# ucsdarclab/diffco

Measured on AMD Instinct MI355X. Metric: million collision-score+grad evals/sec, 7-DoF FK-kernel, 2k supports, higher is better.
Workload: dtype f32

## Files before the change

### diffco_amd/csrc/dcx_api.hip

```cpp
#include <algorithm>
#include <atomic>
#include <cmath>
#include <cstdio>
#include <cstdlib>
#include <cstring>
#include <mutex>
#include <new>
#include <string>
#include <vector>

#include "dcx_internal.h"
#include "motion_cost_kernel.h"
#include "motion_kernel.h"
#include "motion_worst_kernel.h"
#include "pack_kernels.h"
#include "solve_kernels.h"
#include "traj_dense.h"

using namespace dcx;

struct dcx_model {
    int device = 0;
    dcx_fk_desc fk{};
    FkProg* fk_dev = nullptr;
    DhProg* dh_dev = nullptr;
    DhArgs dh{};
    int32_t fk_dwords = 0;
    float* rows_dev = nullptr;
    float* rows_p2_dev = nullptr;
    float* rows_xf_dev = nullptr;
    float* centre_dev = nullptr;
    int64_t S_in = 0;
    int32_t S_active = 0;
    int64_t cap = 0;
    float fold = 1.0f;
    int32_t* info_dev = nullptr;
    int32_t* info_host = nullptr;
    int32_t D = 0, Dt = 0, C = 0, RS = 0;
    int32_t Cc = 0;
    int32_t kind = 0, kf = 0;
    float kp0 = 0, kp1 = 0;
    float kp0_sweep = 0;
    int32_t xf_rq_ok = 0;
    int32_t frame_floats = 0;
    int32_t prog_floats = 0;
    launch_fn launch = nullptr;
    int32_t max_threads = 0;
    int32_t n_cu = 256;
    struct Scratch {
        hipStream_t stream;
        float* ptr;
        size_t rows_bytes;
        uint32_t epoch;
    };
    int32_t* giveup_host = nullptr;
    int32_t* giveup_dev = nullptr;
    mutable std::mutex mu;
    mutable std::vector<Scratch> scratch;
    struct TrajExch {
        hipStream_t stream;
        unsigned long long* ptr;
        size_t bytes;
        uint32_t epoch;
    };
    mutable std::vector<TrajExch> traj_exch;
    struct HessMom {
        hipStream_t stream;
        float* ptr;
        size_t bytes;
    };
    mutable std::vector<HessMom> hess_mom;
};

#ifdef DCX_TIMING
static unsigned long long* g_ts_dev = nullptr;
constexpr size_t kTsWords = 32 * 16 + 4096 * 4;
#endif

namespace {

thread_local std::string g_err;

int fail(int code, const std::string& msg) {
// ... 125 lines not shown
}

int set_device(int device) {
    int n = 0;
    hipError_t e = hipGetDeviceCount(&n);
    if (e != hipSuccess || n == 0) return fail(DCX_ERR_NO_DEVICE, "no HIP device visible (libdcx has no CPU path)");
    if (device < 0 || device >= n) return fail(DCX_ERR_INVALID, "device index out of range");
    DCX_HIP(hipSetDevice(device));
    return DCX_OK;
}

struct FkCacheEntry {
    int device;
    dcx_fk_desc host;
    FkProg* dev;
};
thread_local std::vector<FkCacheEntry> g_fk_cache;

int upload_fk_prog(const dcx_fk_desc& fk, FkProg** out) {
    FkProg prog;
    build_fk_prog(fk, prog);
    FkProg* d = nullptr;
    DCX_HIP(hipMalloc((void**)&d, sizeof(FkProg)));
    hipError_t e = hipMemcpy(d, &prog, sizeof(FkProg), hipMemcpyHostToDevice);
    if (e != hipSuccess) {
        (void)hipFree(d);
        return fail_hip(e, "upload of the FK program");
    }
    *out = d;
    return DCX_OK;
}

int fk_device_copy(int device, const dcx_fk_desc& fk, FkProg** out) {
    for (auto& e : g_fk_cache)
        if (e.device == device && std::memcmp(&e.host, &fk, sizeof(fk)) == 0) {
            *out = e.dev;
            return DCX_OK;
        }
    FkProg* d = nullptr;
    if (int rc = upload_fk_prog(fk, &d)) return rc;
    if (g_fk_cache.size() >= 64) {
        (void)hipFree(g_fk_cache.front().dev);
        g_fk_cache.erase(g_fk_cache.begin());
    }
    g_fk_cache.push_back({device, fk, d});
    *out = d;
    return DCX_OK;
}

struct Knobs {
    std::atomic<int64_t> ys{-1}, nw{-1}, min_rows{-1}, split_finish_kernel{-1}, inlaunch_tiles{-1}, jac_per_class{-1},
        traj_fused{-1}, xf{-1}, jac_one_sweep{-1}, train_grid{-1}, fkk{-1}, jt_waves{-1}, hess_ys{-1}, hess_form{-1},
        traj_ys{-1}, traj_across{-1}, owner_poll{-1}, solve_threads{-1}, qt{-1}, giveup_inject{-1}, skew{-1}, skew8{-1},
        motion_early_exit{-1};
    Knobs() {
        auto rd = [](const char* name, std::atomic<int64_t>& dst, bool flag) {
            if (const char* e = std::getenv(name)) dst = flag ? 1 : std::atoll(e);
        };
        rd("DCX_YS", ys, false);
        rd("DCX_NW", nw, false);
        rd("DCX_MIN_ROWS", min_rows, false);
        rd("DCX_SPLIT_FINISH_KERNEL", split_finish_kernel, true);
        rd("DCX_INLAUNCH_TILES", inlaunch_tiles, false);
        rd("DCX_JAC_PER_CLASS", jac_per_class, true);
        rd("DCX_TRAJ_FUSED", traj_fused, false);
        rd("DCX_XF", xf, false);
        rd("DCX_JAC_ONE_SWEEP", jac_one_sweep, false);
        rd("DCX_TRAIN_GRID", train_grid, false);
        rd("DCX_FKK", fkk, false);
        rd("DCX_JT_WAVES", jt_waves, false);
        rd("DCX_HESS_YS", hess_ys, false);
        rd("DCX_HESS_FORM", hess_form, false);
        rd("DCX_TRAJ_YS", traj_ys, false);
        rd("DCX_TRAJ_ACROSS", traj_across, false);
        rd("DCX_OWNER_POLL", owner_poll, false);
        rd("DCX_SOLVE_THREADS", solve_threads, false);
        rd("DCX_QT", qt, false);
        rd("DCX_SKEW", skew, false);
        rd("DCX_SKEW8", skew8, false);
    }
};
Knobs& knobs() {
    static Knobs k;
    return k;
}

struct Geometry {
    int nw, ys;
    int red_slots;
};
Geometry pick_geometry(const dcx_model* m, int64_t B, int acc_floats, bool allow_split) {
    const int cap = m->max_threads / 64;
    const int64_t tiles = (B + 63) / 64;
    Geometry g;
    g.ys = 1;
    if (allow_split && 2 * tiles <= m->n_cu) {
        const int64_t want = std::min<int64_t>((int64_t)m->n_cu / tiles, m->S_active / 250);
        while (2 * g.ys <= want && g.ys < 32) g.ys *= 2;
        g.nw = std::min(16, cap);
    } else if (allow_split && 3 * tiles <= 2 * (int64_t)m->n_cu && (int64_t)m->S_active * m->Dt >= 18000) {
        g.ys = 3;
        g.nw = std::min(16, cap);
    } else {
        g.nw = std::min((tiles <= 4 * (int64_t)m->n_cu) ? 16 : 8, cap);
    }
    const Knobs& kn = knobs();
    if (const int64_t v = kn.ys; v >= 1 && allow_split) g.ys = (int)std::min<int64_t>(v, 64);
    if (const int64_t v = kn.nw; v >= 1) g.nw = (int)std::min<int64_t>(v, cap);
    int min_rows = 15;
    if (const int64_t v = kn.min_rows; v >= 1) min_rows = (int)v;
    while (g.ys > 1 && m->S_active / (g.ys * g.nw) < min_rows) g.ys /= 2;
    while (g.nw > 1 && m->S_active / (g.ys * g.nw) < min_rows) g.nw /= 2;
    const int d_fk = m->fk.n_points * m->fk.point_dim;
    auto lds_bytes = [&](int nw, int slots) {
        return (size_t)(lds_plan(m->fk.dof, d_fk, m->frame_floats, nw > 1 ? slots : 0, acc_floats, true).total + m->prog_floats) * sizeof(float);
    };
    g.red_slots = g.nw;
    const size_t lds_cap = (g.ys > 1 ? 150 : 64) * 1024;
    if (lds_bytes(g.nw, g.nw) > lds_cap && g.nw >= 8 && lds_bytes(g.nw / 2, g.nw / 2) <= lds_cap && kn.nw < 1) {
        g.nw /= 2;
        g.red_slots = g.nw;
    }
    if (lds_bytes(g.nw, g.nw) > lds_cap) {
        const int wps = sweep_min_waves(m->Dt, m->Cc, m->kf);
        int best_nw = 1, best_waves = 0;
        for (int nw = g.nw; nw >= 1; nw /= 2) {
            const size_t lds = lds_bytes(nw, 1);
            if (lds > 64 * 1024) continue;
            const int by_lds = (int)((160 * 1024) / lds), by_regs = std::max(1, (4 * wps) / nw);
            const int waves = std::min(by_lds, by_regs) * nw;
            if (waves > best_waves) {
                best_waves = waves;
                best_nw = nw;
            }
        }
        g.nw = best_nw;
        g.red_slots = 1;
// ... 195 lines not shown
    a.upstream = upstream;
    a.score = score;
    a.grad = grad;
    a.B = B;
    a.S = m->S_active;
    a.ys = g.ys;
    a.s_super = (m->S_active + g.ys - 1) / g.ys;
    a.s_chunk = (a.s_super + g.nw - 1) / g.nw;
    const bool p2 = !qt && !xf_able && m->rows_p2_dev != nullptr && p2_applies(m->Dt, m->Cc, m->kf);
    if (p2) {
        a.rows = m->rows_p2_dev;
        a.s_super = (a.s_super + 1) & ~1;
        a.s_chunk = ((a.s_super + g.nw - 1) / g.nw + 1) & ~1;
    }
    const bool so = mode == MODE_SCORE && !hinge.traj_slices;
    a.s_skew = (g.nw == 16 && !qt && (a.s_chunk >= 24 || knobs().skew > 0)) ? skew_rule(m->Cc, so, hinge.traj_slices != 0) : (g.nw == 8 && !qt && (a.s_chunk >= 24 || knobs().skew8 > 0)) ? skew8_rule(so) : 0;
    a.red_slots = g.red_slots;
    a.dof = m->fk.dof;
    a.d_fk = d_fk;
    a.frame_floats = m->frame_floats;
    a.kind = m->kind;
    a.c_out = m->C;
    a.one_hot = one_hot;
    a.nz = nz;
    a.grad_stride = grad_stride;
    a.kp0 = m->kp0_sweep;
    a.kp1 = m->kp1;
    a.hinge = hinge.on;
    a.hinge_margin = hinge.margin;
    a.hinge_weight = hinge.weight;
    for (int c = 0; c < DCX_MAX_C; ++c) a.hinge_margin_c[c] = hinge.margin_c[c];
    a.xf = xf_able ? 1 : 0;
    if (qt) {
        a.xf = 0;
        a.qt = 1;
        a.qt_per = qt_per;
        for (int gq = 0; gq < 4; ++gq) a.qt_per_g[gq] = qt_per;
        if (g.nw == 16 && skew_rule() > 0) {
            const int32_t sk = skew_rule();
            const int w3[3] = {sk & 1023, (sk >> 10) & 1023, (sk >> 20) & 1023};
            int left = 4 * qt_per;
            for (int gq = 0; gq < 3; ++gq) {
                a.qt_per_g[gq] = std::min(left, (int)((int64_t)4 * qt_per * w3[gq] / 1000));
                left -= a.qt_per_g[gq];
            }
            a.qt_per_g[3] = left;
        }
        a.qt_off = (int32_t)((lds_plan(a.dof, d_fk, m->frame_floats, g.nw, acc, true).total + m->prog_floats + 3) & ~3);
        a.qt_scr = a.qt_off + QT_SLICES * g.nw * (qt_per * row_stride(m->Dt, m->Cc) + 4);
        const int64_t kq = knobs().qt;
        a.qt_front = (int32_t)((int64_t)QT_SLICES * g.nw * qt_per * (kq >= 100 ? std::min<int64_t>(kq - 100, 100) : 45) / 100);
        nblk = (B + 15) / 16;
    }
    if (a.xf) {
        a.rows = m->rows_xf_dev;
        a.centre = m->centre_dev;
    }
    a.jt_rows = (a.fkk == 2 && g.nw >= 2 * m->dh.n_chains && m->dh.n_chains <= 2 && m->dh.end0 <= kDhUnroll &&
                 m->dh.n_steps - m->dh.end0 <= kDhUnroll && knobs().jt_waves != 0) ? 1 : 0;
    a.jt_waves = (a.jt_rows && mode != MODE_SCORE && g.red_slots == g.nw && (g.nw - 1) * acc >= 12 * m->dh.n_pt + 1 &&
                  (g.ys == 1 || counters != nullptr)) ? 1 : 0;
#ifdef DCX_TIMING
    if (!g_ts_dev && hipMalloc((void**)&g_ts_dev, sizeof(unsigned long long) * kTsWords) == hipSuccess)
        (void)hipMemset(g_ts_dev, 0, sizeof(unsigned long long) * kTsWords);
    a.ts = g_ts_dev;
    a.ts_block = std::getenv("DCX_TS_BLOCK") ? (unsigned)std::atoi(std::getenv("DCX_TS_BLOCK")) : 0u;
#endif
    size_t lds = sizeof(float) * (lds_plan(a.dof, d_fk, m->frame_floats, g.nw > 1 ? g.red_slots : 0, acc, true).total + m->prog_floats);
    if (qt) lds = qt_lds;
    if (g.ys == 1) {
        hipError_t e = m->launch(m->kf, m->Cc, mode, g.nw, lds, nblk, a, st);
        if (e != hipSuccess) return fail_hip(e, "score kernel launch");
        return DCX_OK;
    }
    if (nz > 1 && counters == nullptr) return DCX_ERR_UNSUPPORTED;
    a.partial = part;
    a.tile_done = counters;
    if (counters != nullptr && g.red_slots == g.nw && g.nw > 1 && knobs().owner_poll != 0 && (acc <= 2 * g.nw || knobs().owner_poll > 0) &&
        nblk * nz * g.ys <= (int64_t)m->n_cu && 2 * nblk * nz <= (int64_t)m->n_cu && m->giveup_dev != nullptr &&
        (knobs().owner_poll > 0 || opoll_stream_ok(m->device, st))) {
        a.pwords = reinterpret_cast<unsigned long long*>(reinterpret_cast<char*>(part) + (size_t)2 * m->n_cu * (m->Dt + m->Cc) * 64 * sizeof(float));
        a.ptag = ptag;
        a.giveup = m->giveup_dev;
    }
    hipError_t e = m->launch(m->kf, m->Cc, mode, g.nw, lds, nblk, a, st);
    if (e == hipSuccess && counters == nullptr) {
        FinishArgs f{};
        f.partial = part;
        f.fk = m->fk_dev;
        f.q = q;
        f.upstream = (m->C == 1) ? upstream : nullptr;
        f.score = score;
        f.grad = grad;
        f.B = B;
        f.grad_stride = grad_stride;
        f.ys = g.ys;
        f.acc = acc;
        f.C = m->Cc;
        f.c_out = m->C;
        f.Dt = m->Dt;
        f.dof = m->fk.dof;
        f.d_fk = d_fk;
        f.frame_floats = m->frame_floats;
        f.want_grad = (mode != MODE_SCORE);
        f.hinge = hinge.on;
        f.hinge_margin = hinge.margin;
        f.hinge_weight = hinge.weight;
        e = launch_score_finish(f, nblk, sizeof(float) * (lds_plan(a.dof, d_fk, m->frame_floats, 0, 0).total + m->prog_floats), st);
    }
    if (e != hipSuccess) return fail_hip(e, "split score launch");
    return DCX_OK;
}

}

extern "C" {

#ifdef DCX_TIMING
int dcx_debug_ts_words(void) { return (int)kTsWords; }
int dcx_debug_read_ts(unsigned long long* out) {
    if (!g_ts_dev) return 1;
    (void)hipDeviceSynchronize();
    return hipMemcpy(out, g_ts_dev, sizeof(unsigned long long) * kTsWords, hipMemcpyDeviceToHost) == hipSuccess ? 0 : 3;
}
#endif

int dcx_version(void) { return DCX_VERSION; }

int dcx_debug_set(const char* name, int64_t value) {
    if (!name) return fail(DCX_ERR_INVALID, "knob name is NULL");
    Knobs& k = knobs();
    const std::string n(name);
    if (n == "mfma" || n == "xm")
        return value > 0 ? fail(DCX_ERR_UNSUPPORTED, "the matrix-core forms of the sweep were removed (measured slower, profiles/r03_mfma_ab.txt)")
                         : DCX_OK;
    std::atomic<int64_t>* dst = n == "ys" ? &k.ys : n == "nw" ? &k.nw : n == "min_rows" ? &k.min_rows
        : n == "split_finish_kernel" ? &k.split_finish_kernel : n == "inlaunch_tiles" ? &k.inlaunch_tiles
        : n == "jac_per_class" ? &k.jac_per_class : n == "traj_fused" ? &k.traj_fused : n == "xf" ? &k.xf : n == "jac_one_sweep" ? &k.jac_one_sweep : n == "train_grid" ? &k.train_grid : n == "fkk" ? &k.fkk : n == "jt_waves" ? &k.jt_waves : n == "hess_ys" ? &k.hess_ys : n == "hess_form" ? &k.hess_form : n == "traj_ys" ? &k.traj_ys : n == "traj_across" ? &k.traj_across : n == "owner_poll" ? &k.owner_poll : n == "solve_threads" ? &k.solve_threads : n == "qt" ? &k.qt : n == "giveup_inject" ? &k.giveup_inject : n == "skew" ? &k.skew : n == "skew8" ? &k.skew8 : n == "motion_early_exit" ? &k.motion_early_exit : nullptr;
    if (!dst) return fail(DCX_ERR_INVALID, "unknown knob: " + n);
    *dst = value;
    return DCX_OK;
}

const char* dcx_last_error(void) { return g_err.c_str(); }

int dcx_device_count(void) {
    int n = 0;
    if (hipGetDeviceCount(&n) != hipSuccess) return 0;
    return n;
}

static constexpr double kXfRqRule = 32.0;
static size_t rows_tail_floats(const dcx_model* m) { return 8 * (size_t)m->RS + 16; }

static void model_free_rows(dcx_model* m) {
    if (m->rows_dev) (void)hipFree(m->rows_dev);
    if (m->rows_xf_dev) (void)hipFree(m->rows_xf_dev);
    if (m->rows_p2_dev) (void)hipFree(m->rows_p2_dev);
    m->rows_dev = m->rows_xf_dev = m->rows_p2_dev = nullptr;
    m->cap = 0;
}

static int model_alloc_rows(dcx_model* m, int64_t cap) {
    if (cap < 1) cap = 1;
    if (cap <= m->cap && m->rows_dev) return DCX_OK;
    const size_t floats = (size_t)cap * m->RS + rows_tail_floats(m);
    float *rows = nullptr, *rows_xf = nullptr, *rows_p2 = nullptr;
    hipError_t e = hipMalloc((void**)&rows, floats * sizeof(float));
    if (e == hipSuccess) e = hipMalloc((void**)&rows_xf, floats * sizeof(float));
    if (e == hipSuccess && p2_applies(m->Dt, m->Cc, m->kf)) e = hipMalloc((void**)&rows_p2, (floats + m->RS) * sizeof(float));
    if (e == hipSuccess && !m->centre_dev) e = hipMalloc((void**)&m->centre_dev, (size_t)m->Dt * sizeof(float));
    if (e == hipSuccess && !m->info_dev) e = hipMalloc((void**)&m->info_dev, 16);
    if (e == hipSuccess && !m->info_host) e = hipHostMalloc((void**)&m->info_host, 16, hipHostMallocDefault);
    if (e == hipSuccess && !m->giveup_host) {
        e = hipHostMalloc((void**)&m->giveup_host, sizeof(int32_t), hipHostMallocMapped);
        if (e == hipSuccess) {
            *m->giveup_host = 0;
            e = hipHostGetDevicePointer((void**)&m->giveup_dev, m->giveup_host, 0);
        }
    }
    if (e != hipSuccess) {
        if (rows) (void)hipFree(rows);
        if (rows_xf) (void)hipFree(rows_xf);
        if (rows_p2) (void)hipFree(rows_p2);
        return fail_hip(e, "device allocation of the model");
    }
    model_free_rows(m);
    m->rows_dev = rows;
    m->rows_xf_dev = rows_xf;
    m->rows_p2_dev = rows_p2;
    m->cap = cap;
    return DCX_OK;
}

static int model_fill_device(dcx_model* m, const float* feat_dev, const float* w_dev, int64_t S, hipStream_t stream) {
    PackArgs a{};
    a.feat = feat_dev;
    a.w = w_dev;
    a.rows = m->rows_dev;
    a.rows_xf = m->rows_xf_dev;
    a.centre = m->centre_dev;
    a.info = m->info_dev;
    a.S = S;
    a.D = m->D;
    a.Dt = m->Dt;
    a.C = m->C;
    a.Cl = m->Cc;
    a.RS = m->RS;
    a.tail_floats = (int32_t)rows_tail_floats(m);
    a.centred = (m->fk.kind != DCX_FK_NONE) ? 1 : 0;
    a.rq2 = (m->kf == KF_RQ2) ? 1 : 0;
    a.fold = m->fold;
    a.seed = m->kp0_sweep;
    hipError_t e = launch_pack_rows(a, stream);
    if (e == hipSuccess) e = hipMemcpyAsync(m->info_host, m->info_dev, 16, hipMemcpyDeviceToHost, stream);
    if (e == hipSuccess) e = hipStreamSynchronize(stream);
    if (e != hipSuccess) return fail_hip(e, "packing of the support rows");
    double ss_max;
    std::memcpy(&ss_max, reinterpret_cast<const char*>(m->info_host) + 8, sizeof(double));
    m->S_in = S;
    m->S_active = m->info_host[0];
    m->xf_rq_ok = (m->kf == KF_RQ2 && m->fk.kind != DCX_FK_NONE && (double)m->kp0 * ss_max <= kXfRqRule) ? 1 : 0;
    return DCX_OK;
}

static int model_fill_host(dcx_model* m, const float* support_feat, const float* weights, int64_t S, hipStream_t stream) {
    const int32_t D = m->D, C = m->C, Cl = m->Cc;
    std::vector<float> feat((size_t)S * D), w((size_t)S * C);
    if (S > 0) {
        hipError_t e = hipStreamSynchronize(stream);
        if (e == hipSuccess) e = hipMemcpy(feat.data(), support_feat, feat.size() * sizeof(float), hipMemcpyDefault);
        if (e == hipSuccess) e = hipMemcpy(w.data(), weights, w.size() * sizeof(float), hipMemcpyDefault);
        if (e != hipSuccess) return fail_hip(e, "copy of supports/weights");
    }
    const float fold = m->fold;
    std::vector<float> rows;
    rows.reserve((size_t)S * m->RS + rows_tail_floats(m));
    int32_t kept = 0;
    for (int64_t j = 0; j < S; ++j) {
        bool any = false;
        for (int c = 0; c < C; ++c) any |= (w[j * C + c] != 0.0f);
        if (!any) continue;
        const size_t base = rows.size();
        rows.resize(base + m->RS, 0.0f);
        for (int k = 0; k < D; ++k) rows[base + k] = feat[j * D + k];
        float sum = 0.0f;
        for (int c = 0; c < C; ++c) {
            const float v = w[j * C + c] * fold;
            rows[base + m->Dt + c] = v;
            sum += v;
        }
        if (Cl > 1) rows[base + m->Dt + Cl] = sum;
        double ss = 0.0;
        for (int k = 0; k < D; ++k) ss += (double)feat[j * D + k] * (double)feat[j * D + k];
        rows[base + m->Dt + Cl + (Cl > 1 ? 1 : 0)] = (float)ss;
        ++kept;
    }
    m->S_in = S;
    m->S_active = kept;
    m->xf_rq_ok = 0;
    std::vector<float> centre(m->Dt, 0.0f), rows_xf(rows);
    const int ss_off = m->Dt + Cl + (Cl > 1 ? 1 : 0);
    if (m->fk.kind != DCX_FK_NONE && kept > 0) {
        for (int k = 0; k < D; ++k) {
            double acc = 0.0;
            for (int32_t j = 0; j < kept; ++j) acc += (double)rows[(size_t)j * m->RS + k];
            centre[k] = (float)(acc / (double)kept);
        }
    }
    double ss_max = 0.0;
    for (int32_t j = 0; j < kept; ++j) {
        float* cen = &rows_xf[(size_t)j * m->RS];
        double ss = 0.0;
        for (int k = 0; k < D; ++k) {
            cen[k] = cen[k] - centre[k];
            ss += (double)cen[k] * (double)cen[k];
        }
        ss_max = std::max(ss_max, ss);
        cen[ss_off] = (m->kf == KF_RQ2) ? (float)(ss + (double)m->kp0_sweep) : (float)ss;
    }
    m->xf_rq_ok = (m->kf == KF_RQ2 && m->fk.kind != DCX_FK_NONE && (double)m->kp0 * ss_max <= kXfRqRule) ? 1 : 0;
    rows.resize(rows.size() + rows_tail_floats(m), 0.0f);
    rows_xf.resize(rows.size(), 0.0f);
    hipError_t e = hipMemcpy(m->rows_dev, rows.data(), rows.size() * sizeof(float), hipMemcpyHostToDevice);
    if (e == hipSuccess) e = hipMemcpy(m->rows_xf_dev, rows_xf.data(), rows_xf.size() * sizeof(float), hipMemcpyHostToDevice);
    if (e == hipSuccess) e = hipMemcpy(m->centre_dev, centre.data(), centre.size() * sizeof(float), hipMemcpyHostToDevice);
    if (e != hipSuccess) return fail_hip(e, "upload of the model's rows");
    return DCX_OK;
}

static bool is_device_ptr(const void* p) {
    hipPointerAttribute_t at;
    if (hipPointerGetAttributes(&at, p) != hipSuccess) {
        (void)hipGetLastError();
        return false;
    }
    return at.type == hipMemoryTypeDevice;
}

static int refuse_capture(hipStream_t stream) {
    hipStreamCaptureStatus cap = hipStreamCaptureStatusNone;
    if (hipStreamIsCapturing(stream, &cap) != hipSuccess || cap != hipStreamCaptureStatusNone) {
        (void)hipGetLastError();
        return fail(DCX_ERR_UNSUPPORTED, "a model cannot be built or refilled on a stream that is being captured (the kept row count is read back)");
    }
    return DCX_OK;
}

static int model_fill(dcx_model* m, const float* support_feat, const float* weights, int64_t S, hipStream_t stream) {
    const bool on_device = S > 0 && is_device_ptr(support_feat) && is_device_ptr(weights);
    int rc = on_device ? model_fill_device(m, support_feat, weights, S, stream) : model_fill_host(m, support_feat, weights, S, stream);
    if (rc == DCX_OK && m->rows_p2_dev) {
        hipError_t e = launch_interleave_rows(m->rows_dev, m->rows_p2_dev, (int32_t)m->S_active, m->RS, (int32_t)rows_tail_floats(m), stream);
        if (e != hipSuccess) return fail_hip(e, "interleaving of the support rows");
    }
    return rc;
}

int dcx_model_create(dcx_model** out, int device, const dcx_fk_desc* fk, int kernel_kind, const float* kparams,
                     const float* support_feat, const float* weights, int64_t S, int32_t D, int32_t C) {
    return dcx_model_create_ex(out, device, fk, kernel_kind, kparams, support_feat, weights, S, D, C, 0, nullptr);
}

int dcx_model_create_ex(dcx_model** out, int device, const dcx_fk_desc* fk, int kernel_kind, const float* kparams,
                        const float* support_feat, const float* weights, int64_t S, int32_t D, int32_t C,
                        int64_t capacity, void* stream) {
    if (!out) return fail(DCX_ERR_INVALID, "out is NULL");
    *out = nullptr;
    if (S < 0 || S > 0x7fffffffLL) return fail(DCX_ERR_INVALID, "S out of range");
    if (S > 0 && (!support_feat || !weights)) return fail(DCX_ERR_INVALID, "support_feat / weights is NULL");
    if (D < 1 || D > DCX_MAX_D) return fail(DCX_ERR_UNSUPPORTED, "D must be in [1, DCX_MAX_D]");
    if (C < 1 || C > DCX_MAX_C) return fail(DCX_ERR_UNSUPPORTED, "C must be in [1, DCX_MAX_C]");
    if (int rc = check_kernel(kernel_kind, kparams)) return rc;
    dcx_fk_desc desc;
    std::memset(&desc, 0, sizeof(desc));
    if (fk && fk->kind != DCX_FK_NONE) {
        desc = *fk;
    } else {
// ... 41 lines not shown
        return rc;
    }
    {
        FkProg prog;
        build_fk_prog(m->fk, prog);
        m->fk_dwords = prog.n_dwords;
        DhProg dh;
        if (build_dh_prog(m->fk, dh)) {
            hipError_t de = hipMalloc((void**)&m->dh_dev, sizeof(DhProg));
            if (de == hipSuccess) de = hipMemcpy(m->dh_dev, &dh, sizeof(DhProg), hipMemcpyHostToDevice);
            if (de != hipSuccess) {
                dcx_model_destroy(m);
                return fail_hip(de, "upload of the DH step table");
            }
            m->dh = dh_args_of(dh, m->dh_dev);
        }
    }
    if (capacity > 0x7fffffffLL) capacity = 0x7fffffffLL;
    int rc = model_alloc_rows(m, std::max<int64_t>(S, capacity));
    if (rc == DCX_OK) rc = model_fill(m, support_feat, weights, S, (hipStream_t)stream);
    if (rc != DCX_OK) {
        const std::string msg = g_err;
        dcx_model_destroy(m);
        g_err = msg;
        return rc;
    }
    *out = m;
    return DCX_OK;
}

int dcx_model_update(dcx_model* m, const float* support_feat, const float* weights, int64_t S, void* stream) {
    if (!m) return fail(DCX_ERR_INVALID, "model is NULL");
    if (S < 0 || S > 0x7fffffffLL) return fail(DCX_ERR_INVALID, "S out of range");
    if (S > 0 && (!support_feat || !weights)) return fail(DCX_ERR_INVALID, "support_feat / weights is NULL");
    if (int rc = set_device(m->device)) return rc;
    if (int rc = refuse_capture((hipStream_t)stream)) return rc;
    std::lock_guard<std::mutex> lock(m->mu);
    if (S > m->cap) {
        hipError_t e = hipDeviceSynchronize();
        if (e != hipSuccess) return fail_hip(e, "dcx_model_update");
        if (int rc = model_alloc_rows(m, S)) return rc;
    }
    return model_fill(m, support_feat, weights, S, (hipStream_t)stream);
}

void dcx_model_destroy(dcx_model* m) {
    if (!m) return;
    (void)hipSetDevice(m->device);
    if (m->fk_dev) (void)hipFree(m->fk_dev);
    if (m->dh_dev) (void)hipFree(m->dh_dev);
    if (m->rows_dev) (void)hipFree(m->rows_dev);
    if (m->rows_xf_dev) (void)hipFree(m->rows_xf_dev);
    if (m->rows_p2_dev) (void)hipFree(m->rows_p2_dev);
    if (m->centre_dev) (void)hipFree(m->centre_dev);
    if (m->info_dev) (void)hipFree(m->info_dev);
    if (m->info_host) (void)hipHostFree(m->info_host);
    if (m->giveup_host) (void)hipHostFree(m->giveup_host);
    for (auto& sc : m->scratch)
        if (sc.ptr) (void)hipFree(sc.ptr);
    for (auto& hm : m->hess_mom)
        if (hm.ptr) (void)hipFree(hm.ptr);
    for (auto& ex : m->traj_exch)
        if (ex.ptr) (void)hipFree(ex.ptr);
    delete m;
}

int dcx_model_info(const dcx_model* m, int64_t* S_active, int32_t* D, int32_t* C, int32_t* dof, int32_t* device) {
    if (!m) return fail(DCX_ERR_INVALID, "model is NULL");
    if (S_active) *S_active = m->S_active;
    if (D) *D = m->D;
    if (C) *C = m->C;
    if (dof) *dof = m->fk.dof;
    if (device) *device = m->device;
    return DCX_OK;
}

int dcx_score(const dcx_model* m, const float* q, int64_t B, float* score, void* stream) {
    if (!m) return fail(DCX_ERR_INVALID, "model is NULL");
    if (B < 0 || (B > 0 && (!q || !score))) return fail(DCX_ERR_INVALID, "q / score is NULL or B < 0");
    if (int rc = set_device(m->device)) return rc;
    return run_score(m, q, B, nullptr, score, nullptr, MODE_SCORE, -1, m->fk.dof, (hipStream_t)stream);
}

int dcx_score_grad(const dcx_model* m, const float* q, int64_t B, const float* upstream, float* score, float* grad,
                   void* stream) {
    if (!m) return fail(DCX_ERR_INVALID, "model is NULL");
    if (B < 0 || (B > 0 && (!q || !grad))) return fail(DCX_ERR_INVALID, "q / grad is NULL or B < 0");
    if (int rc = set_device(m->device)) return rc;
    const int mode = (m->C > 1 && upstream) ? MODE_GRAD_UP : MODE_GRAD_ROW;
    return run_score(m, q, B, upstream, score, grad, mode, -1, m->fk.dof, (hipStream_t)stream);
}

static int run_hinge(const dcx_model* m, const float* q, int64_t B, const float* margin , float weight, float* score,
                     float* grad, hipStream_t st, bool traj_slices = false) {
    Hinge h;
    h.weight = weight;
    h.traj_slices = traj_slices ? 1 : 0;
    if (m->C == 1) {
        h.on = 1;
        h.margin = margin[0];
        return run_score(m, q, B, nullptr, score, grad, MODE_GRAD_ROW, -1, m->fk.dof, st, h);
    }
    h.on = 2;
    for (int c = 0; c < m->C; ++c) h.margin_c[c] = margin[c];
    Hinge hs;
    hs.traj_slices = traj_slices ? 1 : 0;
// ... 207 lines not shown
        const int d_fk = m->fk.n_points * m->fk.point_dim;
        int nw = std::min(16, m->max_threads / 64);
        if (const int64_t v = knobs().nw; v >= 1) nw = (int)std::min<int64_t>(v, m->max_threads / 64);
        int ys = 1;
        {
            int64_t want = std::min<int64_t>(8, (int64_t)m->n_cu / std::max(1, st->n_paths));
            if (const int64_t v = knobs().traj_ys; v >= 1) want = std::min<int64_t>(v, 32);
            while (2 * ys <= want) ys *= 2;
            int min_rows = 15;
            if (const int64_t v = knobs().min_rows; v >= 1) min_rows = (int)v;
            while (ys > 1 && (m->S_active / (ys * nw) < min_rows || (int64_t)ys * st->n_paths > m->n_cu)) ys /= 2;
        }
        while (nw > 1 && m->S_active / (ys * nw) < 15) nw /= 2;
        const bool dh_ok = m->fk.kind == DCX_FK_DH && m->dh_dev && knobs().fkk != 0 && knobs().fkk != 1 && knobs().jt_waves != 0 &&
                           m->dh.n_chains <= 2 && m->dh.end0 <= kDhUnroll && m->dh.n_steps - m->dh.end0 <= kDhUnroll;
        const int jt_min_waves = 2 + 2 * m->dh.n_chains;
        auto lds_of = [&](int w) {
            return sizeof(float) * (size_t)(traj_fused_plan(m->fk.dof, d_fk, m->frame_floats, w, m->Dt, (dh_ok && w >= jt_min_waves) ? m->dh.n_pt : 0, m->Cc).total + m->prog_floats);
        };
        while (nw > 1 && lds_of(nw) > 150 * 1024) nw /= 2;
        traj_fused_fn fn = traj_fused_for(m->Dt);
        bool fused_ok = fn && lds_of(nw) <= 150 * 1024;
        if (fused_ok) {
            TrajFusedArgs a{};
            for (int c = 0; c < DCX_MAX_C; ++c) a.margin_c[c] = margin[c];
            a.sc.rows = m->rows_dev;
            set_fk_walk(m, a.sc);
            a.sc.jt_rows = a.sc.jt_waves = (dh_ok && nw >= jt_min_waves && a.sc.fkk == 2) ? 1 : 0;
#ifdef DCX_TIMING
            if (!g_ts_dev && hipMalloc((void**)&g_ts_dev, sizeof(unsigned long long) * kTsWords) == hipSuccess)
                (void)hipMemset(g_ts_dev, 0, sizeof(unsigned long long) * kTsWords);
            a.sc.ts = g_ts_dev;
#endif
            a.sc.S = m->S_active;
            bool traj_p2 = false;
            auto slice = [&](int ys_) {
                a.s_super = (m->S_active + ys_ - 1) / ys_;
                a.sc.s_chunk = (a.s_super + nw - 1) / nw;
                if (traj_p2) {
                    a.s_super = (a.s_super + 1) & ~1;
                    a.sc.s_chunk = ((a.s_super + nw - 1) / nw + 1) & ~1;
                }
                a.sc.s_skew = (nw == 16 && (a.sc.s_chunk >= 24 || knobs().skew > 0)) ? skew_rule(m->Cc, false, true) : (nw == 8 && (a.sc.s_chunk >= 24 || knobs().skew8 > 0)) ? skew8_rule() : 0;
            };
            a.sc.dof = m->fk.dof;
            a.sc.d_fk = d_fk;
            a.sc.frame_floats = m->frame_floats;
            a.sc.kind = m->kind;
            a.sc.c_out = m->C;
            a.sc.kp0 = m->kp0_sweep;
            a.sc.kp1 = m->kp1;
            a.sc.xf = (knobs().xf != 0 && m->kf == KF_POLY1 && xf_applies(m->Dt, m->Cc, KF_POLY1) && m->rows_xf_dev) ? 1 : 0;
            if (a.sc.xf) {
                a.sc.rows = m->rows_xf_dev;
                a.sc.centre = m->centre_dev;
            } else if (m->rows_p2_dev && p2_applies(m->Dt, m->Cc, m->kf)) {
                a.sc.rows = m->rows_p2_dev;
                traj_p2 = true;
            }
            slice(ys);
            a.st = *st;
            a.opt = *opt;
            a.n_points = m->fk.n_points;
            a.point_dim = m->fk.point_dim;
            a.coord_major = (m->fk.kind == DCX_FK_TREE && m->fk.t_coord_major) ? 1 : 0;
            for (int done = 0; done < n_iters; done += kTrajFusedMaxIters) {
                a.n_iters = std::min(kTrajFusedMaxIters, n_iters - done);
                for (int i = 0; i < a.n_iters; ++i) {
                    const double t = (double)(first_step + done + i);
                    a.bias1[i] = (float)(1.0 - std::pow((double)opt->beta1, t));
                    a.bias2_sqrt[i] = (float)std::sqrt(1.0 - std::pow((double)opt->beta2, t));
                }
                a.ys = 1;
                if (ys > 1) {
                    a.exch = traj_exchange_rows(m, (hipStream_t)stream, (size_t)st->n_paths * 2 * ys * traj_exchange_words(m->Dt, m->Cc) * 64 * sizeof(unsigned long long),
                                                &a.tag_base);
                    if (a.exch) a.ys = ys;
                    a.cl_across = knobs().traj_across > 0 ? 1 : 0;
                }
                if (a.ys != ys) {
                    ys = 1;
                    slice(1);
                }
                hipError_t e = fn(m->kf, m->Cc, nw, lds_of(nw), st->n_paths, a, (hipStream_t)stream);
                if (e == hipErrorNotSupported && done == 0) {
                    (void)hipGetLastError();
                    fused_ok = false;
                    break;
                }
                if (e != hipSuccess && a.ys > 1) {
                    (void)hipGetLastError();
                    ys = a.ys = 1;
                    slice(1);
                    e = fn(m->kf, m->Cc, nw, lds_of(nw), st->n_paths, a, (hipStream_t)stream);
                }
                if (e != hipSuccess) return fail_hip(e, "fused trajectory launch");
            }
            if (fused_ok) return DCX_OK;
        }
    }
    for (int it = 0; it < n_iters; ++it) {
        int rc = run_hinge(m, st->path, B, margin, opt->w_collision, const_cast<float*>(st->col_score), const_cast<float*>(st->col_grad),
                           (hipStream_t)stream, true);
        if (rc) return rc;
        hipError_t e = launch_traj_adam_step(m->fk_dev, m->fk, *st, *opt, first_step + it, (hipStream_t)stream, m->C, margin);
        if (e != hipSuccess) return fail_hip(e, "trajectory step launch");
    }
    return DCX_OK;
// ... 113 lines not shown
    w.frac = up((size_t)(E + 1) * sizeof(int64_t));
    w.counters = w.frac + up((size_t)E * sizeof(float));
    w.partial = w.counters + (size_t)kMotionSplitTiles * kCounterStride * sizeof(unsigned int);
    w.total = w.partial + (size_t)kMotionSplitRows * DCX_MAX_C * 64 * sizeof(float);
    return w;
}
motion_fn motion_for(int Dt) {
    switch (Dt) {
#define DCX_CASE(D) case D: return launch_motion_D##D;
        DCX_CASE(2) DCX_CASE(4) DCX_CASE(6) DCX_CASE(8) DCX_CASE(12) DCX_CASE(16) DCX_CASE(18) DCX_CASE(21)
        DCX_CASE(24) DCX_CASE(27) DCX_CASE(30) DCX_CASE(32) DCX_CASE(36) DCX_CASE(42) DCX_CASE(48) DCX_CASE(54)
        DCX_CASE(60) DCX_CASE(64) DCX_CASE(72) DCX_CASE(84) DCX_CASE(96)
#undef DCX_CASE
    default: return nullptr;
    }
}
struct MotionSweepPlan {
    Geometry g;
    size_t lds;
};
MotionSweepPlan motion_sweep_plan(const dcx_model* m, int64_t tiles_max, char* base, const MotionWork& w, ScoreArgs& sa) {
    const int d_fk = m->fk.n_points * m->fk.point_dim;
    const int acc = m->Cc;
    Geometry g = pick_geometry(m, std::min<int64_t>(tiles_max, (int64_t)1 << 30) * 64, acc, true);
    if (g.ys > 1 && (tiles_max > kMotionSplitTiles || tiles_max * g.ys > kMotionSplitRows))
        g = pick_geometry(m, std::min<int64_t>(tiles_max, (int64_t)1 << 30) * 64, acc, false);
    sa.rows = m->rows_dev;
    set_fk_walk(m, sa);
    sa.B = 0;
    sa.S = m->S_active;
    sa.ys = g.ys;
    sa.s_super = (m->S_active + g.ys - 1) / g.ys;
    sa.s_chunk = (sa.s_super + g.nw - 1) / g.nw;
    const bool xf_able = knobs().xf != 0 && xf_applies(m->Dt, m->Cc, m->kf) && m->rows_xf_dev != nullptr &&
                         (m->kf != KF_RQ2 || m->xf_rq_ok || knobs().xf >= 2);
    if (!xf_able && m->rows_p2_dev != nullptr && p2_applies(m->Dt, m->Cc, m->kf)) {
        sa.rows = m->rows_p2_dev;
        sa.s_super = (sa.s_super + 1) & ~1;
        sa.s_chunk = ((sa.s_super + g.nw - 1) / g.nw + 1) & ~1;
    }
    sa.s_skew = (g.nw == 16 && (sa.s_chunk >= 24 || knobs().skew > 0)) ? skew_rule(m->Cc, true)
              : (g.nw == 8 && (sa.s_chunk >= 24 || knobs().skew8 > 0)) ? skew8_rule(true) : 0;
    sa.red_slots = g.red_slots;
    sa.dof = m->fk.dof;
    sa.d_fk = d_fk;
    sa.frame_floats = m->frame_floats;
    sa.kind = m->kind;
    sa.c_out = m->C;
    sa.one_hot = -1;
    sa.nz = 1;
    sa.kp0 = m->kp0_sweep;
    sa.kp1 = m->kp1;
    sa.xf = xf_able ? 1 : 0;
    if (sa.xf) {
        sa.rows = m->rows_xf_dev;
        sa.centre = m->centre_dev;
    }
    sa.jt_rows = (sa.fkk == 2 && g.nw >= 2 * m->dh.n_chains && m->dh.n_chains <= 2 && m->dh.end0 <= kDhUnroll &&
                  m->dh.n_steps - m->dh.end0 <= kDhUnroll && knobs().jt_waves != 0) ? 1 : 0;
    if (g.ys > 1) {
        sa.partial = (float*)(base + w.partial);
        sa.tile_done = (unsigned int*)(base + w.counters);
    }
    const size_t lds = sizeof(float) * (((size_t)lds_plan(sa.dof, d_fk, m->frame_floats, g.nw > 1 ? g.red_slots : 0, acc, true).total +
                                         m->prog_floats + 3) & ~(size_t)3) + sizeof(float) * kMotionLdsFloats;
    return MotionSweepPlan{g, lds};
}
}

size_t dcx_motion_work_bytes(const dcx_model* m, int64_t E) {
    if (!m || E < 0) return 0;
    return motion_work(E).total;
}

int dcx_check_motions(const dcx_model* m, const float* qa, const float* qb, int64_t E, const dcx_motion_opts* opt,
                      const float* margin, int32_t* first_hit, int32_t* n_samples, void* work, size_t work_bytes, void* stream) {
    return dcx_check_motions_ex(m, qa, qb, E, opt, margin, first_hit, n_samples, work, work_bytes, 0, stream);
}

int dcx_check_motions_ex(const dcx_model* m, const float* qa, const float* qb, int64_t E, const dcx_motion_opts* opt,
                         const float* margin, int32_t* first_hit, int32_t* n_samples, void* work, size_t work_bytes,
                         uint64_t wrap_mask, void* stream) {
    if (!m) return fail(DCX_ERR_INVALID, "model is NULL");
    if (!opt) return fail(DCX_ERR_INVALID, "motion options are NULL");
    if (E < 0) return fail(DCX_ERR_INVALID, "E < 0");
    if (E > 0 && (!qa || !qb || !first_hit || !work)) return fail(DCX_ERR_INVALID, "qa / qb / first_hit / work is NULL");
    const bool by_res = opt->res > 0, by_step = opt->max_step > 0.f;
    if (opt->res < 0 || !(opt->max_step >= 0.f) || by_res == by_step)
        return fail(DCX_ERR_INVALID, "motion check needs exactly one sampling rule: res > 0 or max_step > 0 (the other 0)");
    if (opt->max_samples < 1) return fail(DCX_ERR_INVALID, "motion check needs max_samples >= 1");
    if (wrap_mask != 0 && m->fk.dof < 64 && (wrap_mask >> m->fk.dof) != 0)
        return fail(DCX_ERR_INVALID, "motion check: wrap_mask has a bit at or above dof");
    const MotionWork w = motion_work(E);
    if (E > 0 && work_bytes < w.total) return fail(DCX_ERR_INVALID, "motion workspace is smaller than dcx_motion_work_bytes");
    if (E > INT32_MAX) return fail(DCX_ERR_UNSUPPORTED, "motion check: more than 2^31 - 1 edges");
    if (E == 0) return DCX_OK;
    const int64_t tiles_max = (E * (int64_t)opt->max_samples + 63) / 64;
    if (tiles_max > 0x7fffffffLL) return fail(DCX_ERR_UNSUPPORTED, "motion check: E * max_samples too large for one launch");
    if (int rc = set_device(m->device)) return rc;
    hipStream_t st = (hipStream_t)stream;
    char* base = (char*)work;
    MotionArgs a{};
    const MotionSweepPlan plan = motion_sweep_plan(m, tiles_max, base, w, a.sc);
    const Geometry& g = plan.g;
    MotionPrepArgs p{};
    p.qa = qa;
    p.qb = qb;
    p.E = E;
    p.dof = m->fk.dof;
    p.res = opt->res;
// ... 230 lines not shown
    const MotionCostWork w = motion_cost_work(m, E, opt->max_samples);
    char* base = (char*)work;
    const int d_fk = m->fk.n_points * m->fk.point_dim;
    const int acc = m->Dt + m->Cc;
    const int64_t b_max = std::min<int64_t>(tiles_max, (int64_t)1 << 30) * 64;
    Geometry g = pick_geometry(m, b_max, acc, true);
    if (g.ys > 1 && (tiles_max > kMotionSplitTiles || tiles_max * g.ys > kMotionSplitRows)) g = pick_geometry(m, b_max, acc, false);
    MotionPrepArgs p{};
    p.qa = qa;
    p.qb = qb;
    p.E = E;
    p.dof = m->fk.dof;
    p.res = opt->res;
    p.max_samples = opt->max_samples;
    p.max_step = opt->max_step;
    p.offs = (int64_t*)(base + w.offs);
    p.frac = (float*)(base + w.frac);
    p.first_hit = (int32_t*)(base + w.status);
    p.n_samples = n_samples;
    p.counters = g.ys > 1 ? (unsigned int*)(base + w.counters) : nullptr;
    p.n_counters = g.ys > 1 ? (int32_t)tiles_max : 0;
    p.open_end = opt->max_step > 0.f ? opt->open_end : 0;
    p.wrap_mask = wrap_mask;
    hipError_t e = launch_motion_prep(p, st);
    if (e != hipSuccess) return fail_hip(e, "motion cost prep launch");

    MotionCostArgs a{};
    ScoreArgs& sa = a.sc;
    sa.rows = m->rows_dev;
    set_fk_walk(m, sa);
    sa.B = 0;
    sa.S = m->S_active;
    sa.ys = g.ys;
    sa.s_super = (m->S_active + g.ys - 1) / g.ys;
    sa.s_chunk = (sa.s_super + g.nw - 1) / g.nw;
    const bool xf_able = knobs().xf != 0 && xf_applies(m->Dt, m->Cc, m->kf) && m->rows_xf_dev != nullptr &&
                         (m->kf != KF_RQ2 || m->xf_rq_ok || knobs().xf >= 2);
    if (!xf_able && m->rows_p2_dev != nullptr && p2_applies(m->Dt, m->Cc, m->kf)) {
        sa.rows = m->rows_p2_dev;
        sa.s_super = (sa.s_super + 1) & ~1;
        sa.s_chunk = ((sa.s_super + g.nw - 1) / g.nw + 1) & ~1;
    }
    sa.red_slots = g.red_slots;
    sa.dof = m->fk.dof;
    sa.d_fk = d_fk;
    sa.frame_floats = m->frame_floats;
    sa.kind = m->kind;
    sa.c_out = m->C;
    sa.one_hot = -1;
    sa.nz = 1;
    sa.kp0 = m->kp0_sweep;
    sa.kp1 = m->kp1;
    sa.xf = xf_able ? 1 : 0;
    if (sa.xf) {
        sa.rows = m->rows_xf_dev;
        sa.centre = m->centre_dev;
    }
    sa.jt_rows = (sa.fkk == 2 && g.nw >= 2 * m->dh.n_chains && m->dh.n_chains <= 2 && m->dh.end0 <= kDhUnroll &&
                  m->dh.n_steps - m->dh.end0 <= kDhUnroll && knobs().jt_waves != 0) ? 1 : 0;
    sa.jt_waves = 0;
    if (g.ys > 1) {
        sa.partial = (float*)(base + w.partial);
        sa.tile_done = (unsigned int*)(base + w.counters);
    }
    a.qa = qa;
    a.qb = qb;
    a.offs = p.offs;
    a.frac = p.frac;
    a.margin = margin;
    a.h = (float*)(base + w.h);
    a.dq = (float*)(base + w.dq);
    a.scores = m->C > 1 ? (float*)(base + w.scores) : nullptr;
    a.tile_on = m->C > 1 ? (int32_t*)(base + w.tile_on) : nullptr;
    a.E = E;
    a.weight = weight;
    a.res = opt->res;
    a.open_end = p.open_end;
    a.wrap_mask = wrap_mask;
    auto skew_for = [&](bool score_only) {
        return (g.nw == 16 && (sa.s_chunk >= 24 || knobs().skew > 0)) ? skew_rule(m->Cc, score_only)
             : (g.nw == 8 && (sa.s_chunk >= 24 || knobs().skew8 > 0)) ? skew8_rule(score_only) : 0;
    };
    auto lds_for = [&](int acc_floats) {
        return sizeof(float) * (((size_t)lds_plan(sa.dof, d_fk, m->frame_floats, g.nw > 1 ? g.red_slots : 0, acc_floats, true).total +
                                 m->prog_floats + 3) & ~(size_t)3) + sizeof(float) * kMotionCostLdsFloats;
    };
    if (m->C == 1) {
        sa.s_skew = skew_for(false);
        e = launch(m->kf, m->Cc, MODE_GRAD_ROW, g.nw, lds_for(acc), tiles_max, a, st);
    } else {
        sa.s_skew = skew_for(true);
        e = launch(m->kf, m->Cc, MODE_SCORE, g.nw, lds_for(m->Cc), tiles_max, a, st);
        if (e == hipSuccess) {
            sa.s_skew = skew_for(false);
            e = launch(m->kf, m->Cc, MODE_GRAD_UP, g.nw, lds_for(acc), tiles_max, a, st);
        }
    }
    if (e != hipSuccess) return fail_hip(e, "motion cost kernel launch");
    MotionReduceArgs r{};
    r.qa = qa;
    r.qb = qb;
    r.offs = p.offs;
    r.frac = p.frac;
    r.status = p.first_hit;
    r.h = a.h;
    r.dq = a.dq;
    r.cost = cost;
    r.grad_a = grad_a;
    r.grad_b = grad_b;
    r.E = E;
// ... 294 lines not shown
```

### diffco_amd/csrc/motion_cost_inst.hip

```cpp
#include "dcx_internal.h"
#include "motion_cost_kernel.h"

#ifndef DCX_INST_D
#error "compile with -DDCX_INST_D=<feature width>"
#endif

namespace dcx {
#define DCX_CAT_(a, b) a##b
#define DCX_CAT(a, b) DCX_CAT_(a, b)
#ifdef DCX_STUB
hipError_t DCX_CAT(launch_motion_cost_D, DCX_INST_D)(int, int, int, int, size_t, int64_t, const MotionCostArgs&, hipStream_t) {
    return hipErrorNotSupported;
}
#else
namespace {
constexpr int kD = DCX_INST_D;
constexpr int kMaxT = kD <= 16 ? 1024 : (kD <= 48 ? 512 : 256);

template <int KF, int CC, int MODE>
hipError_t go(int nw, size_t lds, int64_t nblk, const MotionCostArgs& a, hipStream_t st) {
    const dim3 grid((unsigned)nblk, (unsigned)(a.sc.ys > 1 ? a.sc.ys : 1));
    const int32_t mc_off = (int32_t)(lds / sizeof(float)) - kMotionCostLdsFloats;
    auto launch = [&](auto kern) {
        if (lds > 64 * 1024) {
            hipError_t e = hipFuncSetAttribute((const void*)kern, hipFuncAttributeMaxDynamicSharedMemorySize, (int)lds);
            if (e != hipSuccess) return e;
        }
        kern<<<grid, dim3(64 * nw), lds, st>>>(a, mc_off);
        return hipGetLastError();
    };
    if constexpr (xf_applies(kD, CC, KF)) {
        if (a.sc.xf) return launch(motion_cost_kernel<kD, KF, CC, MODE, kMaxT, true>);
    }
    return launch(motion_cost_kernel<kD, KF, CC, MODE, kMaxT>);
}

template <int KF, int CC>
hipError_t passes(int mode, int nw, size_t lds, int64_t nblk, const MotionCostArgs& a, hipStream_t st) {
    if (mode == MODE_SCORE) return go<KF, CC, MODE_SCORE>(nw, lds, nblk, a, st);
    if (mode == MODE_GRAD_UP) return go<KF, CC, MODE_GRAD_UP>(nw, lds, nblk, a, st);
    return hipErrorInvalidValue;
}

template <int KF>
hipError_t by_cc(int cc, int mode, int nw, size_t lds, int64_t nblk, const MotionCostArgs& a, hipStream_t st) {
    switch (cc) {
    case 1: return mode == MODE_GRAD_ROW ? go<KF, 1, MODE_GRAD_ROW>(nw, lds, nblk, a, st) : hipErrorInvalidValue;
    case 5: return passes<KF, 5>(mode, nw, lds, nblk, a, st);
#ifndef DCX_DEV_FAST
    case 4: return passes<KF, 4>(mode, nw, lds, nblk, a, st);
    case 8: return passes<KF, 8>(mode, nw, lds, nblk, a, st);
#endif
    default: return hipErrorInvalidValue;
    }
}
}

hipError_t DCX_CAT(launch_motion_cost_D, DCX_INST_D)(int kf, int cc, int mode, int nw, size_t lds, int64_t nblk,
                                                     const MotionCostArgs& a, hipStream_t st) {
    switch (kf) {
    case KF_RQ2: return by_cc<KF_RQ2>(cc, mode, nw, lds, nblk, a, st);
    case KF_POLY1: return by_cc<KF_POLY1>(cc, mode, nw, lds, nblk, a, st);
    case KF_GEN: return by_cc<KF_GEN>(cc, mode, nw, lds, nblk, a, st);
    default: return hipErrorInvalidValue;
    }
}
#endif
}
```

### diffco_amd/csrc/motion_cost_kernel.h

```cpp
#pragma once
#include <hip/hip_runtime.h>
#include <stdint.h>
#include "motion_kernel.h"

namespace dcx {

struct MotionCostArgs {
    ScoreArgs sc;
    const float* qa;
    const float* qb;
    const int64_t* offs;
    const float* frac;
    const float* margin;
    float* h;
    float* dq;
    float* scores;
    int32_t* tile_on;
    int64_t E;
    float weight;
    int32_t res;
    int32_t open_end;
    uint64_t wrap_mask;
};

// ... 20 lines not shown
    float* cost;
    float* grad_a;
    float* grad_b;
    int64_t E;
    int32_t dof, res, open_end;
    float weight;
    uint64_t wrap_mask;
};
hipError_t launch_motion_cost_reduce(const MotionReduceArgs& r, hipStream_t stream);

#ifdef __HIPCC__
constexpr int kMotionCostLdsFloats = kMotionLdsFloats;

__device__ __forceinline__ void motion_tile_lookup(const int64_t* offs, int64_t E, int64_t base, int nb, int64_t* sEnd,
                                                   int32_t* sEdge, int32_t* sK, int32_t* sN) {
    const int lane = threadIdx.x & 63;
    int64_t lo = 0, hi = E;
    while (hi - lo > 1) {
        const int64_t step = (hi - lo + 63) / 64;
        const int64_t idx = lo + (int64_t)lane * step;
        const bool le = idx < hi && offs[idx] <= base;
        const int p = __popcll(__builtin_amdgcn_ballot_w64(le));
        const int64_t nlo = lo + (int64_t)(p - 1) * step;
        hi = (lo + (int64_t)p * step < hi) ? lo + (int64_t)p * step : hi;
        lo = nlo;
    }
    const int64_t e0 = lo;
    sEnd[lane] = (e0 + 1 + lane <= E) ? offs[e0 + 1 + lane] : INT64_MAX;
    __builtin_amdgcn_wave_barrier();
    __builtin_amdgcn_fence(__ATOMIC_ACQ_REL, "workgroup");
    const int64_t s = base + (lane < nb ? lane : nb - 1);
    int64_t e, start;
    if (sEnd[63] > s) {
        int j = 0;
#pragma unroll
        for (int hh = 32; hh >= 1; hh >>= 1)
            if (sEnd[j + hh - 1] <= s) j += hh;
        e = e0 + j;
        start = j ? sEnd[j - 1] : offs[e0];
    } else {
        int64_t l2 = e0 + 64, h2 = E;
        while (h2 - l2 > 1) {
            const int64_t md = (l2 + h2) / 2;
            if (offs[md] <= s) l2 = md; else h2 = md;
        }
        e = l2;
        start = offs[l2];
    }
    sEdge[lane] = (int32_t)e;
    sK[lane] = (int32_t)(s - start);
    sN[lane] = (int32_t)(offs[e + 1] - start);
}

template <int D, int KF, int CC, int MODE, int MAXT, bool XF = false>
__global__ __launch_bounds__(MAXT, sweep_min_waves(D, CC, KF)) void motion_cost_kernel(const MotionCostArgs m, int32_t mc_off) {
    static_assert((CC == 1) == (MODE == MODE_GRAD_ROW), "one class: the hinge sweep; several: the score and gradient passes");
    extern __shared__ __attribute__((aligned(16))) float smem[];
    constexpr bool GRAD = MODE != MODE_SCORE;
    constexpr int ACC = (GRAD ? D : 0) + CC;
    const ScoreArgs& a = m.sc;
    const int wave = __builtin_amdgcn_readfirstlane(threadIdx.x >> 6);
    const int nw = blockDim.x >> 6;
    const int dof = a.dof;
    const LdsPlan lp = lds_plan(dof, a.d_fk, a.frame_floats, nw > 1 ? a.red_slots : 0, ACC, true);
    float* sQ = smem + lp.q;
    float* sX = smem + lp.x;
    float* sF = smem + lp.f;
    int64_t* sEnd = reinterpret_cast<int64_t*>(smem + mc_off);
    int32_t* sEdge = reinterpret_cast<int32_t*>(smem + mc_off + 128);
    int32_t* sK = sEdge + 64;
    int32_t* sN = sEdge + 128;

    const int64_t E = m.E;
    const int64_t total = m.offs[E];
    const int64_t tile = blockIdx.x;
    if (tile * 64 >= total) return;
    if constexpr (MODE == MODE_GRAD_UP) {
        if (m.tile_on[tile] == 0) return;
    }
    const FkWalk fw = fk_stage_sel(a.fkk, a.fk, a.fk_dwords, a.dh, smem + lp.fk, threadIdx.x, blockDim.x);
    const int64_t base = tile * 64;
    const int nb = (int)((total - base) < 64 ? (total - base) : 64);
    if (wave == 0) motion_tile_lookup(m.offs, E, base, nb, sEnd, sEdge, sK, sN);
    __syncthreads();
    for (int i = threadIdx.x; i < 64 * dof; i += blockDim.x) {
        const int l = i / dof, j = i - l * dof;
        const int64_t e = sEdge[l];
        const int k = sK[l];
        const float qa = m.qa[e * dof + j], qb = m.qb[e * dof + j];
        sQ[i] = motion_coord(qa, qb, k, m.res, !m.open_end && k == sN[l] - 1, m.frac + e, (m.wrap_mask >> j) & 1ull);
    }
    __syncthreads();
    {
        const int lane = threadIdx.x & 63;
        fk_trig_sel(fw, a.dh, sQ + lane * dof, sF + lane, wave, nw);
        __syncthreads();
        if (a.fkk == 2 && a.jt_rows) dh2_chain_rows_sel(fw.dh, a.dh, sX + lane, sF + lane, wave);
        else if (wave == 0) fk_chain_sel(fw, a.dh, sQ + lane * dof, sX + lane, sF + lane);
        __syncthreads();
    }
    const int lane0 = threadIdx.x & 63;
    float x[D];
    if (a.d_fk == D) {
#pragma unroll
        for (int k = 0; k < D; ++k) x[k] = sX[k * 64 + lane0];
    } else {
#pragma unroll
        for (int k = 0; k < D; ++k) x[k] = (k < a.d_fk) ? sX[k * 64 + lane0] : 0.0f;
    }
    if constexpr (XF) {
        cfloat_ptr cen = (cfloat_ptr)(uintptr_t)a.centre;
#pragma unroll
        for (int k = 0; k < D; ++k) x[k] -= cen[k];
    }
    if (nw > 1) __syncthreads();
    float up[CC];
#pragma unroll
    for (int c = 0; c < CC; ++c) up[c] = 0.0f;
    if constexpr (MODE == MODE_GRAD_UP) {
        const int64_t s = base + (lane0 < nb ? lane0 : nb - 1);
#pragma unroll
        for (int c = 0; c < CC; ++c)
            if (c < a.c_out) up[c] = (m.scores[s * a.c_out + c] - (m.margin ? m.margin[c] : 0.0f) > 0.0f) ? m.weight : 0.0f;
    }
    float sc[CC];
    float gx[D];
#pragma unroll
    for (int c = 0; c < CC; ++c) sc[c] = 0.0f;
#pragma unroll
    for (int k = 0; k < D; ++k) gx[k] = 0.0f;
    const int ybase = blockIdx.y * a.s_super;
    const int yend = (ybase + a.s_super < a.S) ? (ybase + a.s_super) : a.S;
    int j0, j1;
    wave_slice(wave, nw, a.s_chunk, a.s_skew, ybase, yend, j0, j1);
    sweep_rows<D, KF, CC, MODE, XF>(a, x, up, j0, j1, sc, gx);

    const auto& b = reload_kernargs<MotionCostArgs>();
    const int lane = fresh_lane();
    const LdsPlan lq = lds_plan(b.sc.dof, b.sc.d_fk, b.sc.frame_floats, nw > 1 ? b.sc.red_slots : 0, ACC, true);
    float* sRed = smem + lq.red;
    if (nw > 1 && b.sc.red_slots == nw) {
        float* mine = sRed + (size_t)wave * ACC * 64 + lane;
#pragma unroll
        for (int c = 0; c < CC; ++c) mine[c * 64] = sc[c];
        if constexpr (GRAD) {
#pragma unroll
            for (int k = 0; k < D; ++k) mine[(CC + k) * 64] = gx[k];
        }
        __syncthreads();
        fold_partial_rows<ACC>(sRed, wave, lane, nw);
        __syncthreads();
        if (wave != 0) return;
#pragma unroll
        for (int c = 0; c < CC; ++c) sc[c] = sRed[c * 64 + lane];
        if constexpr (GRAD) {
#pragma unroll
            for (int k = 0; k < D; ++k) gx[k] = sRed[(CC + k) * 64 + lane];
        }
    } else if (nw > 1) {
        for (int w = 1; w < nw; ++w) {
            if (wave == w) {
#pragma unroll
                for (int c = 0; c < CC; ++c) sRed[c * 64 + lane] = sc[c];
                if constexpr (GRAD) {
#pragma unroll
                    for (int k = 0; k < D; ++k) sRed[(CC + k) * 64 + lane] = gx[k];
                }
            }
            __syncthreads();
            if (wave == 0) {
#pragma unroll
                for (int c = 0; c < CC; ++c) sc[c] += sRed[c * 64 + lane];
                if constexpr (GRAD) {
#pragma unroll
                    for (int k = 0; k < D; ++k) gx[k] += sRed[(CC + k) * 64 + lane];
                }
            }
            __syncthreads();
        }
        if (wave != 0) return;
    }
    const int64_t t = blockIdx.x;
    if (b.sc.partial != nullptr) {
        float* out = b.sc.partial + (t * b.sc.ys + blockIdx.y) * ACC * 64 + lane;
#pragma unroll
        for (int c = 0; c < CC; ++c) __hip_atomic_store(out + c * 64, sc[c], __ATOMIC_RELAXED, __HIP_MEMORY_SCOPE_AGENT);
        if constexpr (GRAD) {
#pragma unroll
// ... 83 lines not shown
```

### diffco_amd/csrc/motion_inst.hip

```cpp
#include "dcx_internal.h"
#include "motion_kernel.h"

#ifndef DCX_INST_D
#error "compile with -DDCX_INST_D=<feature width>"
#endif

namespace dcx {
#define DCX_CAT_(a, b) a##b
#define DCX_CAT(a, b) DCX_CAT_(a, b)
#ifdef DCX_STUB
hipError_t DCX_CAT(launch_motion_D, DCX_INST_D)(int, int, int, size_t, int64_t, const MotionArgs&, hipStream_t) { return hipErrorNotSupported; }
#else
namespace {
constexpr int kD = DCX_INST_D;
constexpr int kMaxT = kD <= 16 ? 1024 : (kD <= 48 ? 512 : 256);

template <int KF, int CC>
hipError_t go(int nw, size_t lds, int64_t nblk, const MotionArgs& a, hipStream_t st) {
    const dim3 grid((unsigned)nblk, (unsigned)(a.sc.ys > 1 ? a.sc.ys : 1));
    const int32_t mo_off = (int32_t)(lds / sizeof(float)) - kMotionLdsFloats;
    auto launch = [&](auto kern) {
        if (lds > 64 * 1024) {
            hipError_t e = hipFuncSetAttribute((const void*)kern, hipFuncAttributeMaxDynamicSharedMemorySize, (int)lds);
            if (e != hipSuccess) return e;
        }
        kern<<<grid, dim3(64 * nw), lds, st>>>(a, mo_off);
        return hipGetLastError();
    };
    if constexpr (xf_applies(kD, CC, KF)) {
        if (a.sc.xf) return launch(motion_kernel<kD, KF, CC, kMaxT, true>);
    }
    return launch(motion_kernel<kD, KF, CC, kMaxT>);
}

template <int KF>
hipError_t by_cc(int cc, int nw, size_t lds, int64_t nblk, const MotionArgs& a, hipStream_t st) {
    switch (cc) {
    case 1: return go<KF, 1>(nw, lds, nblk, a, st);
    case 5: return go<KF, 5>(nw, lds, nblk, a, st);
#ifndef DCX_DEV_FAST
    case 4: return go<KF, 4>(nw, lds, nblk, a, st);
    case 8: return go<KF, 8>(nw, lds, nblk, a, st);
#endif
    default: return hipErrorInvalidValue;
    }
}
}

hipError_t DCX_CAT(launch_motion_D, DCX_INST_D)(int kf, int cc, int nw, size_t lds, int64_t nblk, const MotionArgs& a,
                                                hipStream_t st) {
    switch (kf) {
    case KF_RQ2: return by_cc<KF_RQ2>(cc, nw, lds, nblk, a, st);
    case KF_POLY1: return by_cc<KF_POLY1>(cc, nw, lds, nblk, a, st);
    case KF_GEN: return by_cc<KF_GEN>(cc, nw, lds, nblk, a, st);
    default: return hipErrorInvalidValue;
    }
}
#endif
}
```

### diffco_amd/csrc/motion_kernel.h

```cpp
#pragma once
#include <hip/hip_runtime.h>
#include <stdint.h>
#include "score_kernel.h"
#ifdef __HIPCC__
#include "wrap_device.h"
#endif

namespace dcx {

struct MotionArgs {
    ScoreArgs sc;
    const float* qa;
    const float* qb;
    const int64_t* offs;
    const float* frac;
    unsigned int* first_hit;
    const float* margin;
    int64_t E;
    int32_t res;
    int32_t early_exit;
    uint64_t wrap_mask;
};

constexpr int kMotionLdsFloats = 64 * 2 + 64 * 3 + 4;

struct MotionPrepArgs {
    const float* qa;
    const float* qb;
    int64_t E;
    int32_t dof, res, max_samples;
    float max_step;
    int64_t* offs;
    float* frac;
    int32_t* first_hit;
    int32_t* n_samples;
    unsigned int* counters;
    int32_t n_counters;
    int32_t open_end;
    uint64_t wrap_mask;
};
hipError_t launch_motion_prep(const MotionPrepArgs& p, hipStream_t stream);

typedef hipError_t (*motion_fn)(int kf, int cc, int nw, size_t lds, int64_t n_blocks, const MotionArgs& a, hipStream_t stream);
#define DCX_DECLARE_MOTION(D) hipError_t launch_motion_D##D(int, int, int, size_t, int64_t, const MotionArgs&, hipStream_t);
DCX_DECLARE_MOTION(2)  DCX_DECLARE_MOTION(4)  DCX_DECLARE_MOTION(6)  DCX_DECLARE_MOTION(8)
DCX_DECLARE_MOTION(12) DCX_DECLARE_MOTION(16) DCX_DECLARE_MOTION(18) DCX_DECLARE_MOTION(21)
DCX_DECLARE_MOTION(24) DCX_DECLARE_MOTION(27) DCX_DECLARE_MOTION(30) DCX_DECLARE_MOTION(32)
DCX_DECLARE_MOTION(36) DCX_DECLARE_MOTION(42) DCX_DECLARE_MOTION(48) DCX_DECLARE_MOTION(54)
DCX_DECLARE_MOTION(60) DCX_DECLARE_MOTION(64) DCX_DECLARE_MOTION(72) DCX_DECLARE_MOTION(84)
DCX_DECLARE_MOTION(96)
#undef DCX_DECLARE_MOTION

#ifdef __HIPCC__
__device__ __forceinline__ float motion_coord(float qa, float qb, int k, int res, bool target, const float* frac_e, bool masked) {
    if (masked) {
#pragma clang fp contract(off)
        const float d = wrap2pi_f32(__fsub_rn(qb, qa));
        if (res > 0) {
            const float p = d * __fdiv_rn((float)k, (float)res);
            return wrap2pi_f32(qa + p);
        }
        if (target) return qb;
        const float s = d * *frac_e;
        const float p = (float)k * s;
        return wrap2pi_f32(qa + p);
    }
    const float d = __fsub_rn(qb, qa);
    if (res > 0) return __fadd_rn(qa, __fmul_rn(d, __fdiv_rn((float)k, (float)res)));
    if (target) return qb;
    return __fadd_rn(qa, __fmul_rn((float)k, __fmul_rn(d, *frac_e)));
}

template <int D, int KF, int CC, int MAXT, bool XF = false>
__global__ __launch_bounds__(MAXT, sweep_min_waves(D, CC, KF)) void motion_kernel(const MotionArgs m, int32_t mo_off) {
    extern __shared__ __attribute__((aligned(16))) float smem[];
    const ScoreArgs& a = m.sc;
    constexpr int ACC = CC;
    const int wave = __builtin_amdgcn_readfirstlane(threadIdx.x >> 6);
    const int nw = blockDim.x >> 6;
    const int dof = a.dof;
    const LdsPlan lp = lds_plan(dof, a.d_fk, a.frame_floats, nw > 1 ? a.red_slots : 0, ACC, true);
    float* sQ = smem + lp.q;
    float* sX = smem + lp.x;
    float* sF = smem + lp.f;
    float* sRed = smem + lp.red;
    int64_t* sEnd = reinterpret_cast<int64_t*>(smem + mo_off);
    int32_t* sEdge = reinterpret_cast<int32_t*>(smem + mo_off + 128);
    int32_t* sK = sEdge + 64;
    int32_t* sN = sEdge + 128;
    int32_t* sFlag = sEdge + 192;

    const int64_t E = m.E;
    const int64_t total = m.offs[E];
    const int64_t tile = blockIdx.x;
    if (tile * 64 >= total) return;
    const FkWalk fw = fk_stage_sel(a.fkk, a.fk, a.fk_dwords, a.dh, smem + lp.fk, threadIdx.x, blockDim.x);
    const bool split = a.partial != nullptr;
    do {
        const int64_t base = tile * 64;
        const int nb = (int)((total - base) < 64 ? (total - base) : 64);
        if (wave == 0) {
            const int lane = threadIdx.x & 63;
            int64_t lo = 0, hi = E;
            while (hi - lo > 1) {
                const int64_t step = (hi - lo + 63) / 64;
                const int64_t idx = lo + (int64_t)lane * step;
                const bool le = idx < hi && m.offs[idx] <= base;
                const int p = __popcll(__builtin_amdgcn_ballot_w64(le));
                const int64_t nlo = lo + (int64_t)(p - 1) * step;
                hi = (lo + (int64_t)p * step < hi) ? lo + (int64_t)p * step : hi;
                lo = nlo;
            }
            const int64_t e0 = lo;
            sEnd[lane] = (e0 + 1 + lane <= E) ? m.offs[e0 + 1 + lane] : INT64_MAX;
            __builtin_amdgcn_wave_barrier();
            __builtin_amdgcn_fence(__ATOMIC_ACQ_REL, "workgroup");
            const int64_t s = base + (lane < nb ? lane : nb - 1);
            int64_t e, start;
            if (sEnd[63] > s) {
                int j = 0;
#pragma unroll
                for (int h = 32; h >= 1; h >>= 1)
                    if (sEnd[j + h - 1] <= s) j += h;
                e = e0 + j;
                start = j ? sEnd[j - 1] : m.offs[e0];
            } else {
                int64_t l2 = e0 + 64, h2 = E;
                while (h2 - l2 > 1) {
                    const int64_t md = (l2 + h2) / 2;
                    if (m.offs[md] <= s) l2 = md; else h2 = md;
                }
                e = l2;
                start = m.offs[l2];
            }
            const int k = (int)(s - start);
            sEdge[lane] = (int32_t)e;
            sK[lane] = k;
            sN[lane] = (int32_t)(m.offs[e + 1] - start);
            const unsigned int fh = m.early_exit ? __hip_atomic_load(m.first_hit + e, __ATOMIC_RELAXED, __HIP_MEMORY_SCOPE_AGENT) : 0xffffffffu;
            const bool any_live = __builtin_amdgcn_ballot_w64(lane < nb && (unsigned int)k < fh) != 0;
            if (lane == 0) *sFlag = any_live ? 1 : 0;
        }
        __syncthreads();
        const bool live = *sFlag != 0;
        if (!live && !split) continue;
        float sc[CC];
#pragma unroll
        for (int c = 0; c < CC; ++c) sc[c] = 0.0f;
        if (live) {
            for (int i = threadIdx.x; i < 64 * dof; i += blockDim.x) {
                const int l = i / dof, j = i - l * dof;
                const int64_t e = sEdge[l];
                const int k = sK[l];
                const float qa = m.qa[e * dof + j], qb = m.qb[e * dof + j];
                sQ[i] = motion_coord(qa, qb, k, m.res, k == sN[l] - 1, m.frac + e, (m.wrap_mask >> j) & 1ull);
            }
            __syncthreads();
            const int lane = threadIdx.x & 63;
            fk_trig_sel(fw, a.dh, sQ + lane * dof, sF + lane, wave, nw);
            __syncthreads();
            if (a.fkk == 2 && a.jt_rows) dh2_chain_rows_sel(fw.dh, a.dh, sX + lane, sF + lane, wave);
            else if (wave == 0) fk_chain_sel(fw, a.dh, sQ + lane * dof, sX + lane, sF + lane);
            __syncthreads();
            float x[D];
            if (a.d_fk == D) {
#pragma unroll
                for (int k = 0; k < D; ++k) x[k] = sX[k * 64 + lane];
            } else {
#pragma unroll
                for (int k = 0; k < D; ++k) x[k] = (k < a.d_fk) ? sX[k * 64 + lane] : 0.0f;
            }
            if constexpr (XF) {
                cfloat_ptr cen = (cfloat_ptr)(uintptr_t)a.centre;
#pragma unroll
                for (int k = 0; k < D; ++k) x[k] -= cen[k];
            }
            if (nw > 1) __syncthreads();
            const int ybase = blockIdx.y * a.s_super;
            const int yend = (ybase + a.s_super < a.S) ? (ybase + a.s_super) : a.S;
            int j0, j1;
            wave_slice(wave, nw, a.s_chunk, a.s_skew, ybase, yend, j0, j1);
            float up[CC];
            float gx[D];
#pragma unroll
            for (int c = 0; c < CC; ++c) up[c] = 0.0f;
            sweep_rows<D, KF, CC, MODE_SCORE, XF>(a, x, up, j0, j1, sc, gx);
        }
        const auto& b = reload_kernargs<MotionArgs>();
        const int lane = fresh_lane();
        if (nw > 1 && b.sc.red_slots == nw) {
            float* mine = sRed + (size_t)wave * ACC * 64 + lane;
#pragma unroll
            for (int c = 0; c < CC; ++c) mine[c * 64] = sc[c];
            __syncthreads();
            if (wave == 0) {
                for (int w = 1; w < nw; ++w)
#pragma unroll
                    for (int c = 0; c < CC; ++c) sc[c] += sRed[((size_t)w * ACC + c) * 64 + lane];
            }
        } else if (nw > 1) {
            for (int w = 1; w < nw; ++w) {
                if (wave == w) {
#pragma unroll
                    for (int c = 0; c < CC; ++c) sRed[c * 64 + lane] = sc[c];
                }
                __syncthreads();
                if (wave == 0) {
#pragma unroll
                    for (int c = 0; c < CC; ++c) sc[c] += sRed[c * 64 + lane];
                }
                __syncthreads();
            }
        }
        if (wave != 0) continue;
        if (split) {
            float* out = b.sc.partial + (tile * b.sc.ys + blockIdx.y) * ACC * 64 + lane;
#pragma unroll
            for (int c = 0; c < CC; ++c) __hip_atomic_store(out + c * 64, sc[c], __ATOMIC_RELAXED, __HIP_MEMORY_SCOPE_AGENT);
            asm volatile("s_waitcnt vmcnt(0)" ::: "memory");
            unsigned int arrived = 0;
            if (lane == 0) arrived = __hip_atomic_fetch_add(b.sc.tile_done + tile * kCounterStride, 1u, __ATOMIC_RELAXED, __HIP_MEMORY_SCOPE_AGENT);
            arrived = __builtin_amdgcn_readfirstlane(arrived);
            if (arrived != (unsigned int)b.sc.ys - 1u) continue;
            if (lane == 0) b.sc.tile_done[tile * kCounterStride] = 0u;
            asm volatile("" ::: "memory");
            const float* part = b.sc.partial + tile * b.sc.ys * ACC * 64 + lane;
#pragma unroll
            for (int c = 0; c < CC; ++c) sc[c] = 0.0f;
            for (int y = 0; y < b.sc.ys; ++y)
#pragma unroll
                for (int c = 0; c < CC; ++c) sc[c] += __hip_atomic_load(part + ((size_t)y * ACC + c) * 64, __ATOMIC_RELAXED, __HIP_MEMORY_SCOPE_AGENT);
        }
        bool hit = false;
#pragma unroll
        for (int c = 0; c < CC; ++c)
            if (c < b.sc.c_out) hit = hit || (sc[c] - (b.margin ? b.margin[c] : 0.0f) > 0.0f);
        hit = hit && lane < nb;
        const int k = sK[lane];
        const uint64_t hits = __builtin_amdgcn_ballot_w64(hit);
// ... 11 lines not shown
```

### diffco_amd/csrc/motion_worst_inst.hip

```cpp
#include "dcx_internal.h"
#include "motion_worst_kernel.h"

#ifndef DCX_INST_D
#error "compile with -DDCX_INST_D=<feature width>"
#endif

namespace dcx {
#define DCX_CAT_(a, b) a##b
#define DCX_CAT(a, b) DCX_CAT_(a, b)
#ifdef DCX_STUB
hipError_t DCX_CAT(launch_motion_worst_D, DCX_INST_D)(int, int, int, size_t, int64_t, const MotionWorstArgs&, hipStream_t) { return hipErrorNotSupported; }
#else
namespace {
constexpr int kD = DCX_INST_D;
constexpr int kMaxT = kD <= 16 ? 1024 : (kD <= 48 ? 512 : 256);

template <int KF, int CC>
hipError_t go(int nw, size_t lds, int64_t nblk, const MotionWorstArgs& a, hipStream_t st) {
    const dim3 grid((unsigned)nblk, (unsigned)(a.sc.ys > 1 ? a.sc.ys : 1));
    const int32_t mo_off = (int32_t)(lds / sizeof(float)) - kMotionLdsFloats;
    auto launch = [&](auto kern) {
        if (lds > 64 * 1024) {
            hipError_t e = hipFuncSetAttribute((const void*)kern, hipFuncAttributeMaxDynamicSharedMemorySize, (int)lds);
            if (e != hipSuccess) return e;
        }
        kern<<<grid, dim3(64 * nw), lds, st>>>(a, mo_off);
        return hipGetLastError();
    };
    if constexpr (xf_applies(kD, CC, KF)) {
        if (a.sc.xf) return launch(motion_worst_kernel<kD, KF, CC, kMaxT, true>);
    }
    return launch(motion_worst_kernel<kD, KF, CC, kMaxT>);
}

template <int KF>
hipError_t by_cc(int cc, int nw, size_t lds, int64_t nblk, const MotionWorstArgs& a, hipStream_t st) {
    switch (cc) {
    case 1: return go<KF, 1>(nw, lds, nblk, a, st);
    case 5: return go<KF, 5>(nw, lds, nblk, a, st);
#ifndef DCX_DEV_FAST
    case 4: return go<KF, 4>(nw, lds, nblk, a, st);
    case 8: return go<KF, 8>(nw, lds, nblk, a, st);
#endif
    default: return hipErrorInvalidValue;
    }
}
}

hipError_t DCX_CAT(launch_motion_worst_D, DCX_INST_D)(int kf, int cc, int nw, size_t lds, int64_t nblk, const MotionWorstArgs& a,
                                                hipStream_t st) {
    switch (kf) {
    case KF_RQ2: return by_cc<KF_RQ2>(cc, nw, lds, nblk, a, st);
    case KF_POLY1: return by_cc<KF_POLY1>(cc, nw, lds, nblk, a, st);
    case KF_GEN: return by_cc<KF_GEN>(cc, nw, lds, nblk, a, st);
    default: return hipErrorInvalidValue;
    }
}
#endif
}
```

### diffco_amd/csrc/motion_worst_kernel.h

```cpp
#pragma once
#include <hip/hip_runtime.h>
#include <stdint.h>
#include "motion_cost_kernel.h"

namespace dcx {

constexpr int kMotionWorstSampleLimit = (1 << 24) - 1;
static_assert(10000 <= kMotionWorstSampleLimit, "documentation only: the Python layer's default max_samples fits the sample field");
static_assert(DCX_MAX_C <= 256, "the key holds the class in 8 bits");

struct MotionWorstArgs {
    ScoreArgs sc;
    const float* qa;
    const float* qb;
    const int64_t* offs;
    const float* frac;
    unsigned long long* keys;
    const float* margin;
    int64_t E;
    int32_t res;
    uint64_t wrap_mask;
};

typedef hipError_t (*motion_worst_fn)(int kf, int cc, int nw, size_t lds, int64_t n_blocks, const MotionWorstArgs& a, hipStream_t stream);
#define DCX_DECLARE_MOTION_WORST(D) \
    hipError_t launch_motion_worst_D##D(int, int, int, size_t, int64_t, const MotionWorstArgs&, hipStream_t);
DCX_DECLARE_MOTION_WORST(2)  DCX_DECLARE_MOTION_WORST(4)  DCX_DECLARE_MOTION_WORST(6)  DCX_DECLARE_MOTION_WORST(8)
DCX_DECLARE_MOTION_WORST(12) DCX_DECLARE_MOTION_WORST(16) DCX_DECLARE_MOTION_WORST(18) DCX_DECLARE_MOTION_WORST(21)
DCX_DECLARE_MOTION_WORST(24) DCX_DECLARE_MOTION_WORST(27) DCX_DECLARE_MOTION_WORST(30) DCX_DECLARE_MOTION_WORST(32)
DCX_DECLARE_MOTION_WORST(36) DCX_DECLARE_MOTION_WORST(42) DCX_DECLARE_MOTION_WORST(48) DCX_DECLARE_MOTION_WORST(54)
DCX_DECLARE_MOTION_WORST(60) DCX_DECLARE_MOTION_WORST(64) DCX_DECLARE_MOTION_WORST(72) DCX_DECLARE_MOTION_WORST(84)
DCX_DECLARE_MOTION_WORST(96)
#undef DCX_DECLARE_MOTION_WORST

struct MotionWorstFinishArgs {
    const float* qa;
    const float* qb;
    const int64_t* offs;
    const float* frac;
    const int32_t* status;
    const unsigned long long* keys;
    float* worst;
    int32_t* worst_idx;
    int32_t* worst_class;
    float* xstar;
    float* up;
    const float* g;
    float* grad_a;
    float* grad_b;
    int64_t E;
    int32_t dof, res, C;
    uint64_t wrap_mask;
};
hipError_t launch_motion_worst_finish(const MotionWorstFinishArgs& f, hipStream_t stream);
hipError_t launch_motion_worst_chain(const MotionWorstFinishArgs& f, hipStream_t stream);

__host__ __device__ inline uint32_t motion_worst_orderable(uint32_t bits) { return (bits & 0x80000000u) ? ~bits : (bits | 0x80000000u); }
__host__ __device__ inline uint32_t motion_worst_unorder(uint32_t o) { return (o & 0x80000000u) ? (o & 0x7fffffffu) : ~o; }

#ifdef __HIPCC__
template <int D, int KF, int CC, int MAXT, bool XF = false>
__global__ __launch_bounds__(MAXT, sweep_min_waves(D, CC, KF)) void motion_worst_kernel(const MotionWorstArgs m, int32_t mo_off) {
    extern __shared__ __attribute__((aligned(16))) float smem[];
    const ScoreArgs& a = m.sc;
    constexpr int ACC = CC;
    const int wave = __builtin_amdgcn_readfirstlane(threadIdx.x >> 6);
    const int nw = blockDim.x >> 6;
    const int dof = a.dof;
    const LdsPlan lp = lds_plan(dof, a.d_fk, a.frame_floats, nw > 1 ? a.red_slots : 0, ACC, true);
    float* sQ = smem + lp.q;
    float* sX = smem + lp.x;
    float* sF = smem + lp.f;
    float* sRed = smem + lp.red;
    int64_t* sEnd = reinterpret_cast<int64_t*>(smem + mo_off);
    int32_t* sEdge = reinterpret_cast<int32_t*>(smem + mo_off + 128);
    int32_t* sK = sEdge + 64;
    int32_t* sN = sEdge + 128;

    const int64_t E = m.E;
    const int64_t total = m.offs[E];
    const int64_t tile = blockIdx.x;
    if (tile * 64 >= total) return;
    const FkWalk fw = fk_stage_sel(a.fkk, a.fk, a.fk_dwords, a.dh, smem + lp.fk, threadIdx.x, blockDim.x);
    const bool split = a.partial != nullptr;
    const int64_t base = tile * 64;
    const int nb = (int)((total - base) < 64 ? (total - base) : 64);
    if (wave == 0) motion_tile_lookup(m.offs, E, base, nb, sEnd, sEdge, sK, sN);
    __syncthreads();
    float sc[CC];
#pragma unroll
    for (int c = 0; c < CC; ++c) sc[c] = 0.0f;
    {
        for (int i = threadIdx.x; i < 64 * dof; i += blockDim.x) {
            const int l = i / dof, j = i - l * dof;
            const int64_t e = sEdge[l];
            const int k = sK[l];
            const float qa = m.qa[e * dof + j], qb = m.qb[e * dof + j];
            sQ[i] = motion_coord(qa, qb, k, m.res, k == sN[l] - 1, m.frac + e, (m.wrap_mask >> j) & 1ull);
        }
        __syncthreads();
        const int lane = threadIdx.x & 63;
        fk_trig_sel(fw, a.dh, sQ + lane * dof, sF + lane, wave, nw);
        __syncthreads();
        if (a.fkk == 2 && a.jt_rows) dh2_chain_rows_sel(fw.dh, a.dh, sX + lane, sF + lane, wave);
        else if (wave == 0) fk_chain_sel(fw, a.dh, sQ + lane * dof, sX + lane, sF + lane);
        __syncthreads();
        float x[D];
        if (a.d_fk == D) {
#pragma unroll
            for (int k = 0; k < D; ++k) x[k] = sX[k * 64 + lane];
        } else {
#pragma unroll
            for (int k = 0; k < D; ++k) x[k] = (k < a.d_fk) ? sX[k * 64 + lane] : 0.0f;
        }
        if constexpr (XF) {
            cfloat_ptr cen = (cfloat_ptr)(uintptr_t)a.centre;
#pragma unroll
            for (int k = 0; k < D; ++k) x[k] -= cen[k];
        }
        if (nw > 1) __syncthreads();
        const int ybase = blockIdx.y * a.s_super;
        const int yend = (ybase + a.s_super < a.S) ? (ybase + a.s_super) : a.S;
        int j0, j1;
        wave_slice(wave, nw, a.s_chunk, a.s_skew, ybase, yend, j0, j1);
        float up[CC];
        float gx[D];
#pragma unroll
        for (int c = 0; c < CC; ++c) up[c] = 0.0f;
        sweep_rows<D, KF, CC, MODE_SCORE, XF>(a, x, up, j0, j1, sc, gx);
    }
    const auto& b = reload_kernargs<MotionWorstArgs>();
    const int lane = fresh_lane();
    if (nw > 1 && b.sc.red_slots == nw) {
        float* mine = sRed + (size_t)wave * ACC * 64 + lane;
#pragma unroll
        for (int c = 0; c < CC; ++c) mine[c * 64] = sc[c];
        __syncthreads();
        if (wave == 0) {
            for (int w = 1; w < nw; ++w)
#pragma unroll
                for (int c = 0; c < CC; ++c) sc[c] += sRed[((size_t)w * ACC + c) * 64 + lane];
        }
    } else if (nw > 1) {
        for (int w = 1; w < nw; ++w) {
            if (wave == w) {
#pragma unroll
                for (int c = 0; c < CC; ++c) sRed[c * 64 + lane] = sc[c];
            }
            __syncthreads();
            if (wave == 0) {
#pragma unroll
                for (int c = 0; c < CC; ++c) sc[c] += sRed[c * 64 + lane];
            }
            __syncthreads();
        }
    }
    if (wave != 0) return;
    if (split) {
        float* out = b.sc.partial + (tile * b.sc.ys + blockIdx.y) * ACC * 64 + lane;
#pragma unroll
        for (int c = 0; c < CC; ++c) __hip_atomic_store(out + c * 64, sc[c], __ATOMIC_RELAXED, __HIP_MEMORY_SCOPE_AGENT);
        asm volatile("s_waitcnt vmcnt(0)" ::: "memory");
        unsigned int arrived = 0;
        if (lane == 0) arrived = __hip_atomic_fetch_add(b.sc.tile_done + tile * kCounterStride, 1u, __ATOMIC_RELAXED, __HIP_MEMORY_SCOPE_AGENT);
        arrived = __builtin_amdgcn_readfirstlane(arrived);
        if (arrived != (unsigned int)b.sc.ys - 1u) return;
        if (lane == 0) b.sc.tile_done[tile * kCounterStride] = 0u;
        asm volatile("" ::: "memory");
        const float* part = b.sc.partial + tile * b.sc.ys * ACC * 64 + lane;
#pragma unroll
        for (int c = 0; c < CC; ++c) sc[c] = 0.0f;
        for (int y = 0; y < b.sc.ys; ++y)
#pragma unroll
            for (int c = 0; c < CC; ++c) sc[c] += __hip_atomic_load(part + ((size_t)y * ACC + c) * 64, __ATOMIC_RELAXED, __HIP_MEMORY_SCOPE_AGENT);
    }
    float v = -__builtin_inff();
    int cbest = 0;
#pragma unroll
    for (int c = 0; c < CC; ++c) {
        const float d = sc[c] - (b.margin ? b.margin[c] : 0.0f);
        if (c < b.sc.c_out && d > v) {
            v = d;
// ... 25 lines not shown
```

### diffco_amd/csrc/pack_kernels.h

```cpp
#pragma once
#include <hip/hip_runtime.h>
#include <stdint.h>

namespace dcx {

struct PackArgs {
    const float* feat;
    const float* w;
    float* rows;
    float* rows_xf;
    float* centre;
    int32_t* info;
    int64_t S;
    int32_t D, Dt, C, RS;
    int32_t Cl;
    int32_t tail_floats;
    int32_t centred;
    int32_t rq2;
    float fold, seed;
};
hipError_t launch_pack_rows(const PackArgs& a, hipStream_t stream);
hipError_t launch_interleave_rows(const float* rows, float* rows_il, int32_t kept, int32_t RS, int32_t tail, hipStream_t stream);

}
```

### diffco_amd/csrc/pack_kernels.hip

```cpp
#include <algorithm>

#include "pack_kernels.h"

namespace dcx {
namespace {

constexpr int kPackThreads = 1024;

__global__ __launch_bounds__(kPackThreads) void pack_rows_kernel(const PackArgs a) {
    __shared__ int s_wave_cnt[kPackThreads / 64];
    __shared__ int s_base;
    __shared__ double s_max[kPackThreads / 64];
    const int tid = threadIdx.x, lane = tid & 63, wave = tid >> 6;
    const int ss_off = a.Dt + a.Cl + (a.Cl > 1 ? 1 : 0);
    if (tid == 0) s_base = 0;
    __syncthreads();
    for (int64_t j0 = 0; j0 < a.S; j0 += kPackThreads) {
        const int64_t j = j0 + tid;
        bool keep = false;
        if (j < a.S)
            for (int c = 0; c < a.C; ++c) keep |= (a.w[j * a.C + c] != 0.0f);
        const unsigned long long m = __builtin_amdgcn_ballot_w64(keep);
        if (lane == 0) s_wave_cnt[wave] = __builtin_popcountll(m);
        __syncthreads();
        int before = s_base;
        for (int w = 0; w < wave; ++w) before += s_wave_cnt[w];
        const int dst = before + __builtin_popcountll(m & ((1ull << lane) - 1ull));
        if (keep) {
            float* r = a.rows + (size_t)dst * a.RS;
            const float* f = a.feat + j * a.D;
            double ss = 0.0;
            for (int k = 0; k < a.D; ++k) {
                const float v = f[k];
                r[k] = v;
                ss += (double)v * (double)v;
            }
            for (int k = a.D; k < a.RS; ++k) r[k] = 0.0f;
            float sum = 0.0f;
            for (int c = 0; c < a.C; ++c) {
                const float v = a.w[j * a.C + c] * a.fold;
                r[a.Dt + c] = v;
                sum += v;
            }
            if (a.Cl > 1) r[a.Dt + a.Cl] = sum;
            r[ss_off] = (float)ss;
        }
        __syncthreads();
        if (tid == 0) {
            int tot = 0;
            for (int w = 0; w < kPackThreads / 64; ++w) tot += s_wave_cnt[w];
            s_base += tot;
        }
        __syncthreads();
    }
    const int kept = s_base;
    for (int i = tid; i < a.tail_floats; i += kPackThreads) {
        a.rows[(size_t)kept * a.RS + i] = 0.0f;
        a.rows_xf[(size_t)kept * a.RS + i] = 0.0f;
    }
    __syncthreads();
    if (tid < a.Dt) {
        float c = 0.0f;
        if (a.centred && tid < a.D && kept > 0) {
            double acc = 0.0;
            const float* col = a.rows + tid;
            int j = 0;
            for (; j + 32 <= kept; j += 32) {
                float v[32];
#pragma unroll
                for (int u = 0; u < 32; ++u) v[u] = col[(size_t)(j + u) * a.RS];
#pragma unroll
                for (int u = 0; u < 32; ++u) acc += (double)v[u];
            }
            for (; j < kept; ++j) acc += (double)col[(size_t)j * a.RS];
            c = (float)(acc / (double)kept);
        }
        a.centre[tid] = c;
    }
    __syncthreads();
    double mx = 0.0;
    for (int j = tid; j < kept; j += kPackThreads) {
        const float* r = a.rows + (size_t)j * a.RS;
        float* x = a.rows_xf + (size_t)j * a.RS;
        double ss = 0.0;
        for (int k = 0; k < a.D; ++k) {
            const float v = r[k] - a.centre[k];
            x[k] = v;
            ss += (double)v * (double)v;
        }
        for (int k = a.D; k < a.RS; ++k) x[k] = r[k];
        x[ss_off] = a.rq2 ? (float)(ss + (double)a.seed) : (float)ss;
        mx = ss > mx ? ss : mx;
    }
#pragma unroll
    for (int o = 32; o > 0; o >>= 1) {
        const double other = __shfl_xor(mx, o, 64);
        mx = other > mx ? other : mx;
    }
    if (lane == 0) s_max[wave] = mx;
    __syncthreads();
    if (tid == 0) {
        double t = 0.0;
        for (int w = 0; w < kPackThreads / 64; ++w) t = s_max[w] > t ? s_max[w] : t;
        a.info[0] = kept;
        a.info[1] = 0;
        reinterpret_cast<double*>(a.info)[1] = t;
    }
}

__global__ __launch_bounds__(256) void interleave_rows_kernel(const float* rows, float* il, int32_t kept, int32_t RS, int32_t tail) {
    const int32_t even = (kept + 1) & ~1;
    const int64_t n = (int64_t)even * RS + tail;
    for (int64_t i = (int64_t)blockIdx.x * blockDim.x + threadIdx.x; i < n; i += (int64_t)gridDim.x * blockDim.x) {
        if (i >= (int64_t)even * RS) {
            il[i] = 0.0f;
            continue;
        }
        const int32_t j = (int32_t)(i / RS), e = (int32_t)(i % RS);
        il[(size_t)(j >> 1) * 2 * RS + 2 * e + (j & 1)] = j < kept ? rows[i] : 0.0f;
    }
}

}

hipError_t launch_interleave_rows(const float* rows, float* rows_il, int32_t kept, int32_t RS, int32_t tail, hipStream_t stream) {
    const int64_t n = (int64_t)((kept + 1) & ~1) * RS + tail;
    const unsigned blocks = (unsigned)std::min<int64_t>((n + 255) / 256, 1024);
    interleave_rows_kernel<<<dim3(blocks ? blocks : 1), 256, 0, stream>>>(rows, rows_il, kept, RS, tail);
    return hipGetLastError();
}

hipError_t launch_pack_rows(const PackArgs& a, hipStream_t stream) {
    pack_rows_kernel<<<dim3(1), dim3(kPackThreads), 0, stream>>>(a);
    return hipGetLastError();
}

}
```

### diffco_amd/csrc/score_inst.hip

```cpp
#include "dcx_internal.h"
#include "traj_fused.h"
#include "jac_kernel.h"

#ifndef DCX_INST_D
#error "compile with -DDCX_INST_D=<feature width>"
#endif

#if (defined(DCX_STUB) && DCX_INST_PART != 0) || (DCX_INST_PART == 2 && DCX_INST_D > 24)
#elif defined(DCX_STUB)
namespace dcx {
#define DCX_CAT_(a, b) a##b
#define DCX_CAT(a, b) DCX_CAT_(a, b)
hipError_t DCX_CAT(launch_score_D, DCX_INST_D)(int, int, int, int, size_t, int64_t, const ScoreArgs&, hipStream_t) { return hipErrorNotSupported; }
hipError_t DCX_CAT(launch_jac_D, DCX_INST_D)(int, int, int, size_t, int64_t, const ScoreArgs&, hipStream_t) { return hipErrorNotSupported; }
hipError_t DCX_CAT(launch_traj_fused_D, DCX_INST_D)(int, int, int, size_t, int, const TrajFusedArgs&, hipStream_t) { return hipErrorNotSupported; }
}
#else
namespace dcx {
namespace {

constexpr int kD = DCX_INST_D;
constexpr int kMaxT = kD <= 16 ? 1024 : (kD <= 48 ? 512 : 256);


template <int KF, int CC, int MODE>
hipError_t go(int nw, size_t lds, int64_t nblk, const ScoreArgs& a, hipStream_t st) {
    const dim3 grid((unsigned)nblk, (unsigned)(a.ys > 1 ? a.ys : 1), (unsigned)(a.nz > 1 ? a.nz : 1));
    auto launch = [&](auto kern) {
        if (lds > 64 * 1024) {
            hipError_t e = hipFuncSetAttribute((const void*)kern, hipFuncAttributeMaxDynamicSharedMemorySize, (int)lds);
            if (e != hipSuccess) return e;
        }
        kern<<<grid, dim3(64 * nw), lds, st>>>(a);
        return hipGetLastError();
    };
    if constexpr (qt_applies(kD, CC, KF, MODE)) {
        if (a.qt) return launch(score_kernel<kD, KF, CC, MODE, kMaxT, false, true>);
    }
    if constexpr (xf_applies(kD, CC, KF)) {
        if (a.xf) return launch(score_kernel<kD, KF, CC, MODE, kMaxT, true>);
    }
    return launch(score_kernel<kD, KF, CC, MODE, kMaxT>);
}

template <int KF, int CC>
hipError_t by_mode(int mode, int nw, size_t lds, int64_t nblk, const ScoreArgs& a, hipStream_t st) {
    switch (mode) {
    case MODE_SCORE: return go<KF, CC, MODE_SCORE>(nw, lds, nblk, a, st);
    case MODE_GRAD_ROW: return go<KF, CC, MODE_GRAD_ROW>(nw, lds, nblk, a, st);
    case MODE_GRAD_UP:
        if constexpr (CC > 1) return go<KF, CC, MODE_GRAD_UP>(nw, lds, nblk, a, st);
    default: return hipErrorInvalidValue;
    }
}

template <int KF>
hipError_t by_cc(int cc, int mode, int nw, size_t lds, int64_t nblk, const ScoreArgs& a, hipStream_t st) {
    switch (cc) {
    case 1: return by_mode<KF, 1>(mode, nw, lds, nblk, a, st);
    case 5: return by_mode<KF, 5>(mode, nw, lds, nblk, a, st);
#ifndef DCX_DEV_FAST
    case 4: return by_mode<KF, 4>(mode, nw, lds, nblk, a, st);
    case 8: return by_mode<KF, 8>(mode, nw, lds, nblk, a, st);
#endif
    default: return hipErrorInvalidValue;
    }
}

}

#define DCX_CAT_(a, b) a##b
#define DCX_CAT(a, b) DCX_CAT_(a, b)
#ifndef DCX_INST_PART
#error "compile with -DDCX_INST_PART=0, 1 and (D <= 24) 2"
#endif
hipError_t DCX_CAT(launch_score_gen_D, DCX_INST_D)(int cc, int mode, int nw, size_t lds, int64_t nblk, const ScoreArgs& a, hipStream_t st);
namespace {
template <class K>
hipError_t traj_go(K kern, int nw, size_t lds, int n_paths, const TrajFusedArgs& a, hipStream_t st) {
    if (lds > 64 * 1024) {
        hipError_t e = hipFuncSetAttribute((const void*)kern, hipFuncAttributeMaxDynamicSharedMemorySize, (int)lds);
        if (e != hipSuccess) return e;
    }
    if (a.ys > 1) {
        TrajFusedArgs copy = a;
        void* params[] = {&copy};
        const dim3 grid = a.cl_across ? dim3((unsigned)a.ys, (unsigned)n_paths) : dim3((unsigned)n_paths, (unsigned)a.ys);
        return hipLaunchCooperativeKernel((const void*)kern, grid, dim3(64 * nw), params, (unsigned int)lds, st);
    }
    kern<<<dim3((unsigned)n_paths), dim3(64 * nw), lds, st>>>(a);
    return hipGetLastError();
// ... 18 lines not shown
namespace {
template <int KF, int CC>
hipError_t jac_go(int nw, size_t lds, int64_t nblk, const ScoreArgs& a, hipStream_t st) {
    if constexpr (jac_applies(kD, CC)) {
        auto kern = score_jac_kernel<kD, KF, CC, kMaxT>;
        if (lds > 64 * 1024) {
            hipError_t e = hipFuncSetAttribute((const void*)kern, hipFuncAttributeMaxDynamicSharedMemorySize, (int)lds);
            if (e != hipSuccess) return e;
        }
        kern<<<dim3((unsigned)nblk), dim3(64 * nw), lds, st>>>(a);
        return hipGetLastError();
    } else {
        return hipErrorNotSupported;
    }
}
template <int KF>
hipError_t jac_by_cc(int cc, int nw, size_t lds, int64_t nblk, const ScoreArgs& a, hipStream_t st) {
    switch (cc) {
    case 5: return jac_go<KF, 5>(nw, lds, nblk, a, st);
#ifndef DCX_DEV_FAST
    case 4: return jac_go<KF, 4>(nw, lds, nblk, a, st);
    case 8: return jac_go<KF, 8>(nw, lds, nblk, a, st);
#endif
    default: return hipErrorNotSupported;
    }
}
}

hipError_t DCX_CAT(launch_jac_D, DCX_INST_D)(int kf, int cc, int nw, size_t lds, int64_t nblk, const ScoreArgs& a,
                                             hipStream_t st) {
    switch (kf) {
    case KF_RQ2: return jac_by_cc<KF_RQ2>(cc, nw, lds, nblk, a, st);
    case KF_POLY1: return jac_by_cc<KF_POLY1>(cc, nw, lds, nblk, a, st);
    case KF_GEN: return jac_by_cc<KF_GEN>(cc, nw, lds, nblk, a, st);
    default: return hipErrorInvalidValue;
    }
}

#if DCX_INST_PART == 1
#if DCX_INST_D <= 24
hipError_t DCX_CAT(launch_traj_fused_mc_D, DCX_INST_D)(int kf, int cc, int nw, size_t lds, int n_paths, const TrajFusedArgs& a, hipStream_t st);
#endif
hipError_t DCX_CAT(launch_traj_fused_D, DCX_INST_D)(int kf, int cc, int nw, size_t lds, int n_paths, const TrajFusedArgs& a,
                                                    hipStream_t st) {
    if (cc > 1) {
#if DCX_INST_D <= 24
        return DCX_CAT(launch_traj_fused_mc_D, DCX_INST_D)(kf, cc, nw, lds, n_paths, a, st);
#else
        return hipErrorNotSupported;
#endif
    }
    auto go_t = [&](auto kern) { return traj_go(kern, nw, lds, n_paths, a, st); };
    if (a.ys > 1) {
        if constexpr (xf_applies(kD, 1, KF_POLY1)) {
            if (kf == KF_POLY1 && a.sc.xf) return go_t(traj_fused_kernel<kD, KF_POLY1, kMaxT, true, true>);
        }
        switch (kf) {
        case KF_RQ2: return go_t(traj_fused_kernel<kD, KF_RQ2, kMaxT, false, true>);
        case KF_POLY1: return go_t(traj_fused_kernel<kD, KF_POLY1, kMaxT, false, true>);
        case KF_GEN: return go_t(traj_fused_kernel<kD, KF_GEN, kMaxT, false, true>);
        default: return hipErrorInvalidValue;
        }
    }
    if constexpr (xf_applies(kD, 1, KF_POLY1)) {
        if (kf == KF_POLY1 && a.sc.xf) return go_t(traj_fused_kernel<kD, KF_POLY1, kMaxT, true>);
    }
    switch (kf) {
    case KF_RQ2: return go_t(traj_fused_kernel<kD, KF_RQ2, kMaxT>);
    case KF_POLY1: return go_t(traj_fused_kernel<kD, KF_POLY1, kMaxT>);
    case KF_GEN: return go_t(traj_fused_kernel<kD, KF_GEN, kMaxT>);
    default: return hipErrorInvalidValue;
    }
}
#endif

#else
namespace {
template <int CC>
hipError_t traj_mc(int kf, int nw, size_t lds, int n_paths, const TrajFusedArgs& a, hipStream_t st) {
    auto go_t = [&](auto kern) { return traj_go(kern, nw, lds, n_paths, a, st); };
    if (a.ys > 1) {
        if constexpr (xf_applies(kD, CC, KF_POLY1)) {
            if (kf == KF_POLY1 && a.sc.xf) return go_t(traj_fused_kernel<kD, KF_POLY1, kMaxT, true, true, CC>);
        }
        switch (kf) {
        case KF_RQ2: return go_t(traj_fused_kernel<kD, KF_RQ2, kMaxT, false, true, CC>);
        case KF_POLY1: return go_t(traj_fused_kernel<kD, KF_POLY1, kMaxT, false, true, CC>);
        default: return hipErrorNotSupported;
        }
    }
    if constexpr (xf_applies(kD, CC, KF_POLY1)) {
        if (kf == KF_POLY1 && a.sc.xf) return go_t(traj_fused_kernel<kD, KF_POLY1, kMaxT, true, false, CC>);
    }
    switch (kf) {
    case KF_RQ2: return go_t(traj_fused_kernel<kD, KF_RQ2, kMaxT, false, false, CC>);
    case KF_POLY1: return go_t(traj_fused_kernel<kD, KF_POLY1, kMaxT, false, false, CC>);
    default: return hipErrorNotSupported;
    }
}
}
hipError_t DCX_CAT(launch_traj_fused_mc_D, DCX_INST_D)(int kf, int cc, int nw, size_t lds, int n_paths, const TrajFusedArgs& a, hipStream_t st) {
    switch (cc) {
    case 5: return traj_mc<5>(kf, nw, lds, n_paths, a, st);
#ifndef DCX_DEV_FAST
    case 4: return traj_mc<4>(kf, nw, lds, n_paths, a, st);
    case 8: return traj_mc<8>(kf, nw, lds, n_paths, a, st);
#endif
    default: return hipErrorNotSupported;
    }
}
#endif
}
#endif
```

### diffco_amd/csrc/score_kernel.h

```cpp
#pragma once
#include <hip/hip_runtime.h>
#include <type_traits>
#include <stdint.h>
#include "fk_device.h"

namespace dcx {

enum { KF_RQ2 = 0,
       KF_POLY1 = 1,
       KF_GEN = 2 };

enum { MODE_SCORE = 0,
       MODE_GRAD_ROW = 1,
       MODE_GRAD_UP = 2 };

struct ScoreArgs {
    const float* rows;
    const float* centre;
    const FkProg* fk;
    const float* q;
    const float* upstream;
    float* score;
    float* grad;
    int64_t B;
    int32_t S;
    int32_t s_chunk;
    int32_t dof;
    int32_t d_fk;
    int32_t frame_floats;
    int32_t kind;
    int32_t c_out;
    int32_t one_hot;
    int32_t nz;
    int64_t grad_stride;
    float* partial;
    unsigned int* tile_done;
    unsigned long long* pwords;
    uint32_t ptag;
    int32_t* giveup;
    int32_t ys;
    int32_t s_super;
    int32_t red_slots;
#ifdef DCX_TIMING
    unsigned long long* ts;
    unsigned int ts_block;
#endif
    float kp0, kp1;
    int32_t xf;
    int32_t fkk;
    int32_t fk_dwords;
    DhArgs dh;
    int32_t jt_rows;
    int32_t jt_waves;
    int32_t hinge;
    float hinge_margin, hinge_weight;
    float hinge_margin_c[8];
    int32_t s_skew;
    int32_t qt;
    int32_t qt_off;
    int32_t qt_per;
    int32_t qt_per_g[4];
    int32_t qt_scr;
    int32_t qt_front;
};

#ifndef DCX_ROW_ALIGN_MULTI
#define DCX_ROW_ALIGN_MULTI 4
#endif
template <int D, int CC>
struct RowLayout {
    static constexpr int W_OFF = D;
    static constexpr int WSUM_OFF = D + CC;
    static constexpr int SS_OFF = D + CC + (CC > 1 ? 1 : 0);
    static constexpr int AL = CC > 1 ? DCX_ROW_ALIGN_MULTI : 4;
    static constexpr int RS = (SS_OFF + 1 + AL - 1) / AL * AL;
};

__device__ __forceinline__ void wave_slice(int wave, int nw, int s_chunk, int skew, int ybase, int yend, int& j0, int& j1) {
    int start = wave * s_chunk, len = s_chunk;
    if (skew > 0 && nw == 16) {
        const int w0 = skew & 1023, w1 = (skew >> 10) & 1023, w2 = (skew >> 20) & 1023;
        const int l0 = (s_chunk * w0 / 250) & ~1, l1 = (s_chunk * w1 / 250) & ~1, l2 = (s_chunk * w2 / 250) & ~1;
        int l3 = 4 * s_chunk - l0 - l1 - l2;
        l3 = l3 > 0 ? l3 : 0;
        const int g = wave >> 2, q = wave & 3;
        len = (g == 0) ? l0 : (g == 1) ? l1 : (g == 2) ? l2 : l3;
        start = 4 * ((g > 0 ? l0 : 0) + (g > 1 ? l1 : 0) + (g > 2 ? l2 : 0)) + q * len;
    } else if (skew < 0 && nw == 8) {
        int l0 = (s_chunk * (-skew) / 500) & ~1;
        l0 = l0 < 2 * s_chunk ? l0 : 2 * s_chunk;
        const int g = wave >> 2, q = wave & 3;
        len = g ? 2 * s_chunk - l0 : l0;
        start = (g ? 4 * l0 : 0) + q * len;
    }
    j0 = (ybase + start < yend) ? ybase + start : yend;
    j1 = (j0 + len < yend) ? j0 + len : yend;
}

constexpr int kCounterStride = 32;

typedef const __attribute__((address_space(4))) float* cfloat_ptr;
// ... 131 lines not shown
    return p;
}

#ifndef DCX_MINW_SLACK
#define DCX_MINW_SLACK 0
#endif
constexpr int sweep_min_waves(int D, int CC, int KF, bool QT = false) {
    if (QT) return 4;
    const int need = 3 * D + 2 * CC + 16 + DCX_MINW_SLACK + (KF == 2 ? 40 : 0);
    return need <= 64 ? 8 : need <= 72 ? 7 : need <= 80 ? 6 : need <= 96 ? 5 : need <= 128 ? 4 : need <= 168 ? 3 : need <= 256 ? 2 : 1;
}

__device__ __forceinline__ int fresh_lane() {
    int l = (int)__builtin_amdgcn_mbcnt_hi(~0u, __builtin_amdgcn_mbcnt_lo(~0u, 0u));
    asm volatile("" : "+v"(l));
    return l;
}

template <class Args>
__device__ __forceinline__ const __attribute__((address_space(4))) Args& reload_kernargs() {
    auto p = (const __attribute__((address_space(4))) Args*)__builtin_amdgcn_kernarg_segment_ptr();
    asm volatile("" : "+s"(p));
    return *p;
}
__device__ __forceinline__ const __attribute__((address_space(4))) ScoreArgs& reload_args() { return reload_kernargs<ScoreArgs>(); }
#define DCX_COPY_DH(dst, src)          \
    do {                               \
        (dst).prog = (src).prog;       \
        (dst).n_dwords = (src).n_dwords; \
        (dst).n_steps = (src).n_steps; \
        (dst).end0 = (src).end0;       \
        (dst).n_chains = (src).n_chains; \
        (dst).pt = (src).pt;           \
        (dst).bare = (src).bare;       \
        (dst).real = (src).real;       \
        (dst).n_pt = (src).n_pt;       \
        (dst).shared_q = (src).shared_q; \
    } while (0)

__device__ __forceinline__ void row_opaque(float& u, float& v) { asm volatile("" : "+v"(u), "+v"(v)); }

#ifndef DCX_XF_TAU
#define DCX_XF_TAU 0.01f
#endif
#ifndef DCX_XF_FLUSH
#define DCX_XF_FLUSH 64
#endif

constexpr bool xf_applies(int D, int CC, int KF) {
    const int used = D + CC + (CC > 1 ? 1 : 0);
    const int parts = (4 * used <= (CC > 1 ? DCX_P0_MAX_MULTI : DCX_P0_MAX_SINGLE)) ? 0 : (used + 37) / 38;
    return (KF == KF_POLY1 || KF == KF_RQ2) && used + 1 <= 38 && parts <= 1;
}
constexpr bool p2_applies(int D, int CC, int KF) {
    return DCX_PAIR2 && DCX_PAIR2_LOADS && CC == 1 && (D % 2) == 0 && D <= DCX_PAIR2_MAX_D && 4 * (D + 1) <= DCX_P0_MAX_SINGLE &&
           (KF == KF_RQ2 || KF == KF_POLY1);
}

template <int D, int KF, int CC, int MODE, bool XF = false, int NACC = 0, bool NS = false>
__device__ __forceinline__ void sweep_rows(const ScoreArgs& a, const float (&x)[D], const float (&up)[CC], int j0, int j1,
                                           float (&sc)[CC], float (&gx)[D]) {
    static_assert(!NS || (CC > 1 && MODE == MODE_GRAD_UP), "NS: the gradient sweep of a multi-class model");
    using L = RowLayout<D, CC>;
    constexpr bool GRAD = (MODE != MODE_SCORE);
    v2f gx2[D / 2 + 1];
#pragma unroll
    for (int k = 0; k < D / 2 + 1; ++k) gx2[k] = v2f{0.0f, 0.0f};
    cfloat_ptr rows = (cfloat_ptr)(uintptr_t)a.rows;
    constexpr int USED_DIRECT = D + CC + (CC > 1 ? 1 : 0);
    constexpr bool XFA = XF && xf_applies(D, CC, KF);
    constexpr int USED = USED_DIRECT + (XFA ? 1 : 0);
    constexpr int RSTRIDE = L::RS;
    constexpr int PARTS = (4 * USED <= (CC > 1 ? DCX_P0_MAX_MULTI : DCX_P0_MAX_SINGLE)) ? 0 : (USED + 37) / 38;
    constexpr bool SC2 = (CC > 1 && PARTS == 1);
    v2f sc2[CC / 2 + 1];
#pragma unroll
    for (int i = 0; i < CC / 2 + 1; ++i) sc2[i] = v2f{0.0f, 0.0f};
    auto add_scores = [&](auto weight_of, float val) __attribute__((always_inline)) {
        if constexpr (NS) {
            (void)val;
        } else if constexpr (SC2) {
            const v2f v2 = {val, val};
#pragma unroll
            for (int c = 0; c + 1 < CC; c += 2) sc2[c / 2] = __builtin_elementwise_fma(v2f{weight_of(c), weight_of(c + 1)}, v2, sc2[c / 2]);
            if constexpr (CC & 1) sc[CC - 1] = fmaf(weight_of(CC - 1), val, sc[CC - 1]);
#pragma unroll
            for (int c = 0; c + 1 < CC; c += 2) asm volatile("" : "+v"(sc2[c / 2]));
            if constexpr (CC & 1) asm volatile("" : "+v"(sc[CC - 1]));
        } else {
#pragma unroll
            for (int c = 0; c < CC; ++c) sc[c] = fmaf(weight_of(c), val, sc[c]);
        }
    };

    v2f xm[D / 2 + 1], ga[D / 2 + 1];
    float xm_tail = 0.0f, ga_tail = 0.0f, xx = 0.0f, thr = 1e-30f, asum = 0.0f;
    if constexpr (XFA) {
#pragma unroll
        for (int k = 0; k < D; ++k) xx = fmaf(x[k], x[k], xx);
        thr = fmaxf(DCX_XF_TAU * xx, 1e-30f);
#pragma unroll
        for (int k = 0; k + 1 < D; k += 2) {
            xm[k / 2] = v2f{-2.0f * x[k], -2.0f * x[k + 1]};
            ga[k / 2] = v2f{0.0f, 0.0f};
        }
        if constexpr (D & 1) xm_tail = -2.0f * x[D - 1];
    }
    auto d2_x = [&](const auto& r) __attribute__((always_inline)) -> float {
        constexpr int NA = NACC > 0 ? NACC : DCX_D2_ACCS(D);
        v2f acc[NA];
        acc[0] = v2f{xx + r[L::SS_OFF], 0.0f};
#pragma unroll
        for (int i = 1; i < NA; ++i) acc[i] = v2f{0.0f, 0.0f};
#pragma unroll
        for (int k = 0; k + 1 < D; k += 2) {
            const v2f rv = {r[k], r[k + 1]};
            acc[(k / 2) % NA] = __builtin_elementwise_fma(xm[k / 2], rv, acc[(k / 2) % NA]);
        }
#pragma unroll
        for (int i = 1; i < NA; ++i) acc[0] += acc[i];
        float d2 = acc[0].x + acc[0].y;
        if constexpr (D & 1) d2 = fmaf(xm_tail, r[D - 1], d2);
        if constexpr (KF == KF_POLY1) return fmaxf(d2, thr);
        else return d2;
    };
    auto coef_of = [&](const auto& r, float g) __attribute__((always_inline)) -> float {
        if constexpr (MODE == MODE_GRAD_ROW) {
            return g * r[CC > 1 ? L::WSUM_OFF : L::W_OFF];
        } else {
            float wb = 0.0f;
#pragma unroll
            for (int c = 0; c < CC; ++c) wb = fmaf(up[c], r[L::W_OFF + c], wb);
            return g * wb;
        }
    };
    auto apply_x = [&](const auto& r, float d2c, auto sign, bool keep) __attribute__((always_inline)) {
        constexpr int SIGN = decltype(sign)::value;
        float val, g;
        sweep_eval<KF, true>(d2c, a, val, g);
        if constexpr (PARTS == 1) row_opaque(val, g);
        constexpr bool SCORE_BY_COEF = (KF == KF_POLY1 && CC == 1 && MODE == MODE_GRAD_ROW);
        if constexpr (!SCORE_BY_COEF) {
            if constexpr (SIGN < 0) val = keep ? -val : 0.0f;
            add_scores([&](int c) __attribute__((always_inline)) { return r[L::W_OFF + c]; }, val);
        }
        if constexpr (GRAD) {
            float coef = coef_of(r, g);
            if constexpr (PARTS == 1) asm volatile("" : "+v"(coef));
            if constexpr (SIGN < 0) coef = keep ? -coef : 0.0f;
            if constexpr (SCORE_BY_COEF) sc[0] = fmaf(coef, d2c, sc[0]);
            const v2f c2 = {coef, coef};
#pragma unroll
            for (int k = 0; k + 1 < D; k += 2) {
                const v2f rv = {r[k], r[k + 1]};
                ga[k / 2] = __builtin_elementwise_fma(c2, rv, ga[k / 2]);
            }
            if constexpr (D & 1) ga_tail = fmaf(coef, r[D - 1], ga_tail);
            asum += coef;
        }
    };
    auto pair_x = [&](const auto& r) __attribute__((always_inline)) -> float {
        const float d2 = d2_x(r);
        apply_x(r, d2, std::integral_constant<int, 1>{}, true);
        return d2;
    };
    auto fix_near = [&](const auto& r, float d2c) __attribute__((always_inline)) {
        const bool nr = d2c <= thr;
        apply_x(r, d2c, std::integral_constant<int, -1>{}, nr);
        const v2f mh = {-0.5f, -0.5f};
        v2f dacc = {0.0f, 0.0f};
#pragma unroll
        for (int k = 0; k + 1 < D; k += 2) {
            const v2f rv = {r[k], r[k + 1]};
            const v2f dk = xm[k / 2] * mh - rv;
            dacc = __builtin_elementwise_fma(dk, dk, dacc);
        }
        float d2d = dacc.x + dacc.y;
        if constexpr (D & 1) {
            const float dl_tail = -0.5f * xm_tail - r[D - 1];
            d2d = fmaf(dl_tail, dl_tail, d2d);
        }
        float val, g;
        kernel_eval<KF>(d2d, a, val, g);
        val = nr ? val : 0.0f;
        if constexpr (!NS) {
#pragma unroll
            for (int c = 0; c < CC; ++c) sc[c] = fmaf(r[L::W_OFF + c], val, sc[c]);
        }
        if constexpr (GRAD) {
            const float cd = nr ? -coef_of(r, g) : 0.0f;
            const v2f cd2 = {cd, cd};
#pragma unroll
            for (int k = 0; k + 1 < D; k += 2) {
                const v2f rv = {r[k], r[k + 1]};
                ga[k / 2] = __builtin_elementwise_fma(cd2, xm[k / 2] * mh - rv, ga[k / 2]);
            }
            if constexpr (D & 1) ga_tail = fmaf(cd, -0.5f * xm_tail - r[D - 1], ga_tail);
        }
    };
    auto stage_x = [&](const auto& r0, const auto& r1) __attribute__((always_inline)) {
        if constexpr (KF != KF_POLY1) {
            (void)pair_x(r0);
            (void)pair_x(r1);
            return;
        }
        const auto m0 = __builtin_amdgcn_ballot_w64(pair_x(r0) <= thr);
        const auto m1 = __builtin_amdgcn_ballot_w64(pair_x(r1) <= thr);
        if (__builtin_expect((m0 | m1) != 0, 0)) {
            fix_near(r0, d2_x(r0));
            fix_near(r1, d2_x(r1));
        }
    };
    auto single_x = [&](const auto& r0) __attribute__((always_inline)) {
        if constexpr (KF != KF_POLY1) {
            (void)pair_x(r0);
            return;
        }
        if (__builtin_expect(__builtin_amdgcn_ballot_w64(pair_x(r0) <= thr) != 0, 0)) fix_near(r0, d2_x(r0));
    };
    auto flush_x = [&]() __attribute__((always_inline)) {
        if constexpr (XFA && GRAD) {
            const v2f ah = {0.5f * asum, 0.5f * asum};
#pragma unroll
            for (int k = 0; k + 1 < D; k += 2) ga[k / 2] = __builtin_elementwise_fma(xm[k / 2], ah, ga[k / 2]);
            if constexpr (D & 1) ga_tail = fmaf(xm_tail, 0.5f * asum, ga_tail);
            asum = 0.0f;
        }
    };
    auto pair = [&](const float (&r)[L::RS]) __attribute__((always_inline)) {
        float dl[D];
        float d2;
        v2f dp[D / 2 + 1];
        {
            constexpr int NA = DCX_D2_ACCS(D);
            v2f acc[NA];
            acc[0] = v2f{d2_seed<KF>(a), 0.0f};
#pragma unroll
            for (int i = 1; i < NA; ++i) acc[i] = v2f{0.0f, 0.0f};
#pragma unroll
            for (int k = 0; k + 1 < D; k += 2) {
                const v2f xv = {x[k], x[k + 1]};
                const v2f rv = {r[k], r[k + 1]};
                dp[k / 2] = xv - rv;
                acc[(k / 2) % NA] = __builtin_elementwise_fma(dp[k / 2], dp[k / 2], acc[(k / 2) % NA]);
            }
#pragma unroll
            for (int i = 1; i < NA; ++i) acc[0] += acc[i];
            d2 = acc[0].x + acc[0].y;
            if constexpr (D & 1) {
                dl[D - 1] = x[D - 1] - r[D - 1];
                d2 = fmaf(dl[D - 1], dl[D - 1], d2);
            }
        }
        float val, g;
        sweep_eval<KF>(d2, a, val, g);
        if constexpr (!NS) {
#pragma unroll
            for (int c = 0; c < CC; ++c) sc[c] = fmaf(r[L::W_OFF + c], val, sc[c]);
        }
        if constexpr (GRAD) {
            float coef;
            if constexpr (MODE == MODE_GRAD_ROW) {
                coef = g * r[CC > 1 ? L::WSUM_OFF : L::W_OFF];
            } else {
                float wb = 0.0f;
#pragma unroll
                for (int c = 0; c < CC; ++c) wb = fmaf(up[c], r[L::W_OFF + c], wb);
                coef = g * wb;
            }
            const v2f c2 = {coef, coef};
#pragma unroll
            for (int k = 0; k + 1 < D; k += 2) gx2[k / 2] = __builtin_elementwise_fma(c2, dp[k / 2], gx2[k / 2]);
            if constexpr (D & 1) gx[D - 1] = fmaf(coef, dl[D - 1], gx[D - 1]);
        }
    };
    constexpr bool P2 = !XF && p2_applies(D, CC, KF);
    static_assert(!P2 || PARTS == 0, "pair2: whole rows in the four-row budget");
    v2f gp[P2 ? D : 1];
    v2f scp = {0.0f, 0.0f};
    if constexpr (P2) {
#pragma unroll
        for (int k = 0; k < D; ++k) gp[k] = v2f{0.0f, 0.0f};
    }
    auto pair2 = [&](const float (&b)[2 * L::RS]) __attribute__((always_inline)) {
        v2f dk[D];
        v2f acc = {d2_seed<KF>(a), d2_seed<KF>(a)};
#pragma unroll
        for (int k = 0; k < D; ++k) {
            const v2f xv = {x[k], x[k]};
            const v2f rv = {b[2 * k], b[2 * k + 1]};
            dk[k] = xv - rv;
            acc = __builtin_elementwise_fma(dk[k], dk[k], acc);
        }
        v2f val, g;
        if constexpr (KF == KF_RQ2) {
            const v2f u = {__builtin_amdgcn_rcpf(acc.x), __builtin_amdgcn_rcpf(acc.y)};
            val = u * u;
            g = val * u;
        } else {
            const v2f d2c = {fmaxf(acc.x, 1e-30f), fmaxf(acc.y, 1e-30f)};
            g = v2f{__builtin_amdgcn_rsqf(d2c.x), __builtin_amdgcn_rsqf(d2c.y)};
            val = d2c * g;
        }
        const v2f w2 = {b[2 * L::W_OFF], b[2 * L::W_OFF + 1]};
        scp = __builtin_elementwise_fma(w2, val, scp);
        if constexpr (GRAD) {
            v2f coef = g * w2;
            if constexpr (MODE != MODE_GRAD_ROW) coef = coef * v2f{up[0], up[0]};
#pragma unroll
            for (int k = 0; k < D; ++k) gp[k] = __builtin_elementwise_fma(coef, dk[k], gp[k]);
        }
    };
    constexpr int USED4 = (USED + 3) / 4 * 4;
    static_assert(USED4 <= L::RS, "the row stride covers whole groups of four");
    constexpr int NLOAD = DCX_LOAD_GROUPS ? USED4 : USED;
#ifdef DCX_EXP_NO_LOADS
    int exp_real_loads = 4;
#endif
    auto load_row = [&](float (&dst)[L::RS], int j) __attribute__((always_inline)) {
        cfloat_ptr r = rows + (size_t)j * RSTRIDE;
#ifdef DCX_EXP_NO_LOADS
        if (exp_real_loads <= 0) {
#pragma unroll
            for (int e = 0; e < NLOAD; ++e) asm volatile("" : "+s"(dst[e]));
            return;
        }
        --exp_real_loads;
#endif
#pragma unroll
        for (int e = 0; e < NLOAD; ++e) dst[e] = r[e];
    };

    static_assert(!XFA || PARTS <= 1, "expanded form: whole rows only");
    if constexpr (P2 && DCX_PAIR2_LOADS) {
    if (j0 < j1) {
        constexpr int R2 = 2 * L::RS;
        float ab[R2], cd[R2];
        auto load2 = [&](float (&dst)[R2], int j) __attribute__((always_inline)) {
            cfloat_ptr r = rows + (size_t)j * RSTRIDE;
#pragma unroll
            for (int e = 0; e < R2; ++e) dst[e] = r[e];
        };
        auto body2 = [&](const float (&b)[R2]) __attribute__((always_inline)) {
#pragma unroll
            for (int e = 2 * USED; e < R2; ++e) asm volatile("" ::"s"(b[e]));
            pair2(b);
        };
        const int j1e = (j1 + 1) & ~1;
        const int jl = j1e - 2;
        load2(ab, j0);
        int j = j0;
        for (; j + 3 < j1e; j += 4) {
            __builtin_amdgcn_s_waitcnt(0xC07F);
            __builtin_amdgcn_sched_barrier(0);
            load2(cd, j + 2);
            __builtin_amdgcn_sched_barrier(0);
            body2(ab);
            __builtin_amdgcn_sched_barrier(0);
            __builtin_amdgcn_s_waitcnt(0xC07F);
            __builtin_amdgcn_sched_barrier(0);
            load2(ab, (j + 4 < j1e) ? j + 4 : jl);
            __builtin_amdgcn_sched_barrier(0);
            body2(cd);
            __builtin_amdgcn_sched_barrier(0);
        }
        if (j < j1e) body2(ab);
    }
    } else if constexpr (PARTS == 0) {
    if (j0 < j1) {
        float rowA[L::RS], rowB[L::RS], rowC[L::RS], rowD[L::RS];
        const int jl = j1 - 1;
        load_row(rowA, j0);
        load_row(rowB, (j0 + 1 < j1) ? j0 + 1 : jl);
        int j = j0;
        for (; j + 3 < j1; j += 4) {
            __builtin_amdgcn_s_waitcnt(0xC07F);
            __builtin_amdgcn_sched_barrier(0);
            load_row(rowC, j + 2);
            load_row(rowD, j + 3);
            __builtin_amdgcn_sched_barrier(0);
            if constexpr (XFA) {
                stage_x(rowA, rowB);
            } else {
// ... 143 lines not shown
                    consume(bufA, P0c{});
                    __builtin_amdgcn_sched_barrier(0);
                    __builtin_amdgcn_s_waitcnt(0xC07F);
                    __builtin_amdgcn_sched_barrier(0);
                    load_part(bufA, (j + 1 < j1) ? j + 1 : jl, P0c{});
                    __builtin_amdgcn_sched_barrier(0);
                    consume(bufB, P1c{});
                    __builtin_amdgcn_sched_barrier(0);
                }
            } else {
                auto step = [&](auto self, auto uc, int j) __attribute__((always_inline)) -> void {
                    constexpr int U = decltype(uc)::value;
                    constexpr int NU = U + 1;
                    __builtin_amdgcn_s_waitcnt(0xC07F);
                    __builtin_amdgcn_sched_barrier(0);
                    {
                        const int jr = j + NU / PARTS;
                        const int row = jr < j1 ? jr : jl;
                        if constexpr (NU % 2 == 0) load_part(bufA, row, std::integral_constant<int, NU % PARTS>{});
                        else load_part(bufB, row, std::integral_constant<int, NU % PARTS>{});
                    }
                    __builtin_amdgcn_sched_barrier(0);
                    if constexpr (U % 2 == 0) consume(bufA, std::integral_constant<int, U % PARTS>{});
                    else consume(bufB, std::integral_constant<int, U % PARTS>{});
                    __builtin_amdgcn_sched_barrier(0);
                    if constexpr (U + 1 < 2 * PARTS) self(self, std::integral_constant<int, U + 1>{}, j);
                };
                load_part(bufA, j0, P0c{});
                int j = j0;
                for (; j + 1 < j1; j += 2) step(step, P0c{}, j);
                if (j < j1) {
                    auto tail = [&](auto self, auto pc) __attribute__((always_inline)) -> void {
                        constexpr int P = decltype(pc)::value;
                        __builtin_amdgcn_s_waitcnt(0xC07F);
                        __builtin_amdgcn_sched_barrier(0);
                        if constexpr (P + 1 < PARTS) {
                            if constexpr ((P + 1) % 2 == 0) load_part(bufA, j, std::integral_constant<int, P + 1>{});
                            else load_part(bufB, j, std::integral_constant<int, P + 1>{});
                        }
                        __builtin_amdgcn_sched_barrier(0);
                        if constexpr (P % 2 == 0) consume(bufA, pc);
                        else consume(bufB, pc);
                        __builtin_amdgcn_sched_barrier(0);
                        if constexpr (P + 1 < PARTS) self(self, std::integral_constant<int, P + 1>{});
                    };
                    tail(tail, P0c{});
                }
            }
        }
    }

    if constexpr (XFA && GRAD) {
        flush_x();
#pragma unroll
        for (int k = 0; k + 1 < D; k += 2) {
            gx[k] -= ga[k / 2].x;
            gx[k + 1] -= ga[k / 2].y;
        }
        if constexpr (D & 1) gx[D - 1] -= ga_tail;
    } else {
#pragma unroll
        for (int k = 0; k + 1 < D; k += 2) {
            gx[k] += gx2[k / 2].x;
            gx[k + 1] += gx2[k / 2].y;
        }
        if constexpr (P2) {
            sc[0] += scp.x + scp.y;
            if constexpr (GRAD) {
#pragma unroll
                for (int k = 0; k < D; ++k) gx[k] += gp[k].x + gp[k].y;
            }
        }
    }
    if constexpr (SC2) {
#pragma unroll
        for (int c = 0; c + 1 < CC; c += 2) {
            sc[c] += sc2[c / 2].x;
            sc[c + 1] += sc2[c / 2].y;
        }
    }
    if constexpr (GRAD && kGradScale<KF> != 1.0f) {
#pragma unroll
        for (int k = 0; k < D; ++k) gx[k] *= kGradScale<KF>;
    }
}

constexpr int kQtSlices = 4;
constexpr bool qt_applies(int D, int CC, int KF, int MODE) {
    return (D == 12 || D == 24) && CC == 1 && (MODE == 1  || MODE == 0 ) && KF != 2 ;
}
template <int D, int KF, bool GRAD>
__device__ __forceinline__ void sweep_rows_lds(const ScoreArgs& a, const float (&x)[D], const float* slice, int per, float& sc0,
                                               float (&gx)[D]) {
    static_assert(D % 4 == 0, "rows are read as whole float4s");
    using L = RowLayout<D, 1>;
    v2f g2[D / 2];
#pragma unroll
    for (int k = 0; k < D / 2; ++k) g2[k] = v2f{0.0f, 0.0f};
    typedef float v4f_t __attribute__((ext_vector_type(4)));
    auto load_row = [&](float (&r)[D + 1], int jj) __attribute__((always_inline)) {
        const float* p = slice + (size_t)jj * L::RS;
#pragma unroll
        for (int q = 0; q < D / 4; ++q) {
            const v4f_t v = *reinterpret_cast<const v4f_t*>(p + 4 * q);
            r[4 * q] = v.x; r[4 * q + 1] = v.y; r[4 * q + 2] = v.z; r[4 * q + 3] = v.w;
        }
        r[D] = p[L::W_OFF];
    };
    auto pair = [&](const float (&r)[D + 1]) __attribute__((always_inline)) {
        v2f dp[D / 2];
        constexpr int NA = DCX_D2_ACCS(D);
        v2f acc[NA];
// ... 17 lines not shown
            const float coef = g * r[D];
            const v2f c2 = {coef, coef};
#pragma unroll
            for (int k = 0; k + 1 < D; k += 2) g2[k / 2] = __builtin_elementwise_fma(c2, dp[k / 2], g2[k / 2]);
        }
    };
    float ra[D + 1], rb[D + 1];
    load_row(ra, 0);
    int jj = 0;
    for (; jj + 2 <= per; jj += 2) {
        load_row(rb, jj + 1);
        pair(ra);
        load_row(ra, jj + 2 < per ? jj + 2 : jj + 1);
        pair(rb);
    }
    if (jj < per) pair(ra);
    if constexpr (GRAD) {
#pragma unroll
        for (int k = 0; k + 1 < D; k += 2) {
            gx[k] += g2[k / 2].x * kGradScale<KF>;
            gx[k + 1] += g2[k / 2].y * kGradScale<KF>;
        }
    }
}

template <int ACC, int E0 = 0, int E1 = ACC>
__device__ __forceinline__ void fold_partial_rows(float* sRed, int wave, int lane, int nw) {
    auto fold_rows = [&](auto nwc) __attribute__((always_inline)) {
        constexpr int NWC = decltype(nwc)::value;
        for (int e = E0 + wave; e < E1; e += NWC) {
            float r[NWC];
#pragma unroll
            for (int w = 0; w < NWC; ++w) r[w] = sRed[((size_t)w * ACC + e) * 64 + lane];
            float v = r[0];
#pragma unroll
            for (int w = 1; w < NWC; ++w) v += r[w];
            sRed[e * 64 + lane] = v;
        }
    };
    if (nw == 16) fold_rows(std::integral_constant<int, 16>{});
    else if (nw == 8) fold_rows(std::integral_constant<int, 8>{});
    else if (nw == 4) fold_rows(std::integral_constant<int, 4>{});
    else if (nw == 2) fold_rows(std::integral_constant<int, 2>{});
    else {
        for (int e = E0 + wave; e < E1; e += nw) {
            float v = sRed[e * 64 + lane];
            for (int w = 1; w < nw; ++w) v += sRed[((size_t)w * ACC + e) * 64 + lane];
            sRed[e * 64 + lane] = v;
        }
    }
}


template <int D, int KF, int CC, int MODE, int MAXT, bool XF = false, bool QT = false>
__global__ __launch_bounds__(MAXT, sweep_min_waves(D, CC, KF, QT)) void score_kernel(const ScoreArgs a) {
    extern __shared__ __attribute__((aligned(16))) float smem[];
    constexpr bool GRAD = (MODE != MODE_SCORE);
    constexpr int ACC = (GRAD ? D : 0) + CC;
    constexpr int TILE = QT ? 16 : 64;
    static_assert(!QT || (!XF && qt_applies(D, CC, KF, MODE)), "the quarter tile: direct form, one class, row weights");

    int lane = threadIdx.x & 63;
    const int wave = __builtin_amdgcn_readfirstlane(threadIdx.x >> 6);
    const int nw = blockDim.x >> 6;
    const int64_t b0 = (int64_t)blockIdx.x * TILE;
    const int nb = (int)((a.B - b0) < TILE ? (a.B - b0) : TILE);
    const int dof = a.dof;
    const LdsPlan lp = lds_plan(dof, a.d_fk, a.frame_floats, nw > 1 ? a.red_slots : 0, ACC, true);
    float* sQ = smem + lp.q;
    float* sX = smem + lp.x;
    float* sF = smem + lp.f;

    auto stage_rows = [&](int first_wave, int row0, int row1) __attribute__((always_inline)) {
        if constexpr (QT) {
            constexpr int RS4 = RowLayout<D, CC>::RS / 4;
            typedef float v4f_t __attribute__((ext_vector_type(4)));
            const v4f_t* src = reinterpret_cast<const v4f_t*>(a.rows);
            constexpr int RSQ = RowLayout<D, CC>::RS;
            const int p0 = a.qt_per_g[0], p1 = a.qt_per_g[1], p2 = a.qt_per_g[2], p3 = a.qt_per_g[3];
            const int r1 = 16 * p0, r2 = r1 + 16 * p1, r3 = r2 + 16 * p2;
            const int b1 = 16 * (p0 * RSQ + 4), b2 = b1 + 16 * (p1 * RSQ + 4), b3 = b2 + 16 * (p2 * RSQ + 4);
            float* dst = smem + a.qt_off;
            for (int e = row0 * RS4 + (int)threadIdx.x - 64 * first_wave; e < row1 * RS4; e += (int)blockDim.x - 64 * first_wave) {
                const int row = e / RS4, q4 = e - row * RS4;
                const int g = (row >= r3) ? 3 : (row >= r2) ? 2 : (row >= r1) ? 1 : 0;
                const int per = (g == 3) ? p3 : (g == 2) ? p2 : (g == 1) ? p1 : p0;
                const int rr = row - ((g == 3) ? r3 : (g == 2) ? r2 : (g == 1) ? r1 : 0);
                const int base = (g == 3) ? b3 : (g == 2) ? b2 : (g == 1) ? b1 : 0;
                const int sl = per > 0 ? rr / per : 0, jj = rr - sl * per;
                v4f_t v = {0.0f, 0.0f, 0.0f, 0.0f};
                if (row < a.S) v = src[(size_t)row * RS4 + q4];
                if (per > 0 && sl < 16) *reinterpret_cast<v4f_t*>(dst + base + sl * (per * RSQ + 4) + jj * RSQ + 4 * q4) = v;
            }
        }
    };
    DCX_TS(0);
    DCX_TSB(0);
    const FkWalk fw = fk_stage_sel(a.fkk, a.fk, a.fk_dwords, a.dh, smem + lp.fk, threadIdx.x, blockDim.x);
#ifdef DCX_TIMING
    if (threadIdx.x == 0) dcx_fk_ts = (a.ts && blockIdx.x == a.ts_block && blockIdx.y == 0) ? a.ts : nullptr;
#endif
    {
        const float* qsrc = a.q + b0 * dof;
        const int n = nb * dof;
        if constexpr (QT) {
            for (int i = threadIdx.x; i < 64 * dof; i += blockDim.x) {
                const int c = (i / dof) & 15;
                sQ[i] = qsrc[(c < nb ? c : nb - 1) * dof + (i % dof)];
// ... 17 lines not shown
        stage_rows(1, a.qt_front, kQtSlices * nw * a.qt_per);
    }
    __syncthreads();

    DCX_TS(2);
    float x[D];
    if (a.d_fk == D) {
#pragma unroll
        for (int k = 0; k < D; ++k) x[k] = sX[k * 64 + lane];
    } else {
#pragma unroll
        for (int k = 0; k < D; ++k) x[k] = (k < a.d_fk) ? sX[k * 64 + lane] : 0.0f;
    }
    if constexpr (XF) {
        cfloat_ptr cen = (cfloat_ptr)(uintptr_t)a.centre;
#pragma unroll
        for (int k = 0; k < D; ++k) x[k] -= cen[k];
    }
    if (nw > 1) __syncthreads();

    float up[CC];
    if constexpr (MODE == MODE_GRAD_UP) {
        const int64_t bl = b0 + (lane < nb ? lane : nb - 1);
        const int hot = (a.nz > 1) ? (int)blockIdx.z : a.one_hot;
#pragma unroll
        for (int c = 0; c < CC; ++c) up[c] = (hot >= 0) ? (c == hot ? 1.0f : 0.0f) : (c < a.c_out ? a.upstream[bl * a.c_out + c] : 0.0f);
        if (a.hinge == 2) {
#pragma unroll
            for (int c = 0; c < CC; ++c) up[c] = (c < a.c_out && up[c] - a.hinge_margin_c[c < 8 ? c : 7] > 0.0f) ? a.hinge_weight : 0.0f;
        }
    }

    float sc[CC];
    float gx[D];
#pragma unroll
    for (int c = 0; c < CC; ++c) sc[c] = 0.0f;
#pragma unroll
    for (int k = 0; k < D; ++k) gx[k] = 0.0f;
    const int ybase = blockIdx.y * a.s_super;
    const int yend = (ybase + a.s_super < a.S) ? (ybase + a.s_super) : a.S;
    int j0, j1;
    wave_slice(wave, nw, a.s_chunk, a.s_skew, ybase, yend, j0, j1);

    DCX_TSB(1);
    if constexpr (QT) {
        constexpr int RSQ = RowLayout<D, CC>::RS;
        const int g = wave >> 2;
        const int per = a.qt_per_g[g];
        int base = 0;
        for (int h = 0; h < g; ++h) base += 16 * (a.qt_per_g[h] * RSQ + 4);
        const float* slice = smem + a.qt_off + base + ((wave & 3) * kQtSlices + (lane >> 4)) * (per * RSQ + 4);
        sweep_rows_lds<D, KF, GRAD>(a, x, slice, per, sc[0], gx);
    } else {
        sweep_rows<D, KF, CC, MODE, XF>(a, x, up, j0, j1, sc, gx);
    }
    DCX_TS(3);
    {
    const auto& b = reload_args();
    int lane = fresh_lane();
    const int wave = __builtin_amdgcn_readfirstlane(threadIdx.x >> 6);
    const int nw = blockDim.x >> 6;
    const int64_t b0 = (int64_t)blockIdx.x * TILE;
    const size_t tile = (size_t)blockIdx.x * gridDim.z + blockIdx.z;
    const int nb = (int)((b.B - b0) < TILE ? (b.B - b0) : TILE);
    const int dof = b.dof;
    const LdsPlan lp = lds_plan(dof, b.d_fk, b.frame_floats, nw > 1 ? b.red_slots : 0, ACC, true);
    float* sQ = smem + lp.q;
    float* sG = smem + lp.g;
    float* sF = smem + lp.f;
    float* sRed = smem + lp.red;
    DhArgs dhb;
    DCX_COPY_DH(dhb, b.dh);
    FkWalk fw;
    fw.fkk = b.fkk;
    fw.g = b.fk;
    fw.fk = (fk_cptr)(uintptr_t)(uint32_t)(uintptr_t)(smem + lp.fk);
    fw.dh = (dh_cptr)(uintptr_t)(uint32_t)(uintptr_t)(smem + lp.fk);
    const bool split = b.partial != nullptr;
    const bool par_tail = nw > 1 && b.red_slots != 1 && (!split || b.tile_done != nullptr);
    bool r1_done = false;
    if constexpr (QT && GRAD) {
        if (b.jt_waves && b.qt_scr > 0) {
            r1_done = true;
            dh2_vjp_r1_sel(fw.dh, dhb, sF + lane, smem + b.qt_scr + lane, wave);
        }
    }
    if (par_tail) {
        float* mine = sRed + (size_t)wave * ACC * 64 + lane;
#pragma unroll
        for (int c = 0; c < CC; ++c) mine[c * 64] = sc[c];
        if constexpr (GRAD) {
#pragma unroll
            for (int k = 0; k < D; ++k) mine[(CC + k) * 64] = gx[k];
        }
        __syncthreads();
        DCX_TS(16);
        const bool opoll = split && b.pwords != nullptr;
        const bool publisher = opoll && blockIdx.y != 0;
        unsigned long long* wout = opoll ? b.pwords + ((tile * b.ys + blockIdx.y) * ACC) * 64 + lane : nullptr;
        float* out = (split && !opoll) ? b.partial + (tile * b.ys + blockIdx.y) * ACC * 64 + lane : nullptr;
        auto fold_mine = [&](auto nwc) __attribute__((always_inline)) {
            constexpr int NWC = decltype(nwc)::value;
            const int nwr = NWC > 0 ? NWC : nw;
            for (int e = wave; e < ACC; e += nwr) {
                float v;
                if constexpr (NWC > 0) {
                    float r[NWC];
// ... 246 lines not shown
                }
            }
#pragma unroll
            for (int u = 0; u < 4; ++u)
                if (e0 + u < ACC) sRed[(e0 + u) * 64 + lane] = tot[u];
        }
#pragma unroll
        for (int c = 0; c < CC; ++c) sc[c] = sRed[c * 64 + lane];
        if constexpr (GRAD) {
#pragma unroll
            for (int k = 0; k < D; ++k) gx[k] = sRed[(CC + k) * 64 + lane];
        }
    }

    if (b.score != nullptr && lane < nb && blockIdx.z == 0) {
#pragma unroll
        for (int c = 0; c < CC; ++c)
            if (c < b.c_out) b.score[(b0 + lane) * b.c_out + c] = sc[c];
    }
    }

    if constexpr (GRAD) {
        float scale = 1.0f;
        if constexpr (CC == 1 && MODE == MODE_GRAD_ROW) {
            if (b.upstream != nullptr) scale = b.upstream[b0 + (lane < nb ? lane : nb - 1)];
            if (b.hinge) scale = (sc[0] - b.hinge_margin > 0.0f) ? b.hinge_weight : 0.0f;
        }
        if (b.d_fk == D) {
#pragma unroll
            for (int k = 0; k < D; ++k) sG[k * 64 + lane] = gx[k] * scale;
        } else {
#pragma unroll
            for (int k = 0; k < D; ++k)
                if (k < b.d_fk) sG[k * 64 + lane] = gx[k] * scale;
        }
        DCX_FK_TS(12, 2);
        float* gq = smem + lp.q;
        fk_vjp_sel(fw, dhb, sQ + lane * dof, sF + lane, sG + lane, gq + lane * dof, dof);
        DCX_TS(5);
        __builtin_amdgcn_fence(__ATOMIC_ACQ_REL, "workgroup");
        __builtin_amdgcn_wave_barrier();
        float* gdst = b.grad + b0 * b.grad_stride + (b.nz > 1 ? (size_t)blockIdx.z * dof : 0);
        const int n = nb * dof;
        if (b.grad_stride == dof) {
            for (int i = lane; i < n; i += 64) gdst[i] = gq[i];
        } else {
            for (int i = lane; i < n; i += 64) gdst[(int64_t)(i / dof) * b.grad_stride + (i % dof)] = gq[i];
        }
        DCX_TSB(3);
    }
    }
}

struct FinishArgs {
    const float* partial;
    const FkProg* fk;
    const float* q;
    const float* upstream;
    float* score;
    float* grad;
    int64_t B;
    int64_t grad_stride;
    int32_t ys, acc, C, Dt, dof, d_fk, frame_floats, want_grad;
    int32_t c_out;
    int32_t hinge;
    float hinge_margin, hinge_weight;
};

}
```

### diffco_amd/csrc/traj_fused.h

```cpp
#pragma once
#include "score_kernel.h"

#ifndef DCX_TRAJ_NACC
#define DCX_TRAJ_NACC 0
#endif

namespace dcx {

#ifdef DCX_TIMING
#define DCX_TTS(slot)                                                                             \
    do {                                                                                          \
        if (a.sc.ts && blockIdx.x == 0 && blockIdx.y == 0 && it == 2 && (threadIdx.x & 63) == 0 && (threadIdx.x >> 6) < 16) \
            a.sc.ts[(slot) * 16 + (threadIdx.x >> 6)] = __builtin_readcyclecounter();             \
    } while (0)
#else
#define DCX_TTS(slot) do { } while (0)
#endif

__device__ __forceinline__ float traj_excess(float n2, float max_speed) {
#pragma clang fp contract(off)
    return n2 - max_speed * max_speed;
}
__device__ __forceinline__ float traj_path_grad(float cp, float dp, float cn, float dn) {
#pragma clang fp contract(off)
// ... 131 lines not shown
            }
            __builtin_amdgcn_s_sleep(2);
        }
        sRed[e * 64 + lane] = tot;
    }
    return ok;
}

template <typename A>
__device__ __forceinline__ void traj_path_terms(const A& b, const TrajLds& L, int lane) {
    const int w = lane;
    const int W = b.st.n_waypoints, pd = b.point_dim, n_points = b.n_points;
    const bool live = w < W;
    float obj = 0.f, mmv = 0.f;
        const float ms = b.opt.max_speed;
        const float w_diff = b.opt.w_diff, w_mm = b.opt.w_max_move;
        const bool has_n = live && w + 1 < W, has_p = live && w >= 1;
        const int wn = has_n ? w + 1 : w, wp = has_p ? w - 1 : w;
        auto one = [&](int kx, int ky, int kz, int npd) __attribute__((always_inline)) {
            const int kk[3] = {kx, ky, kz};
            float dn[3] = {0.f, 0.f, 0.f}, dp[3] = {0.f, 0.f, 0.f};
            float n2n = 0.f, n2p = 0.f;
#pragma unroll
            for (int c = 0; c < 3; ++c) {
                if (c < npd) {
                    const float xc = live ? L.sX[kk[c] * 64 + w] : 0.f;
                    if (has_n) { dn[c] = L.sX[kk[c] * 64 + wn] - xc; n2n = fmaf(dn[c], dn[c], n2n); }
                    if (has_p) { dp[c] = xc - L.sX[kk[c] * 64 + wp]; n2p = fmaf(dp[c], dp[c], n2p); }
                }
            }
            const float mn = traj_excess(n2n, ms), mp = traj_excess(n2p, ms);
            if (has_n) {
                obj += n2n;
                if (mn > 0.f) mmv += mn;
            }
            const float cn = 2.f * (w_diff + (mn > 0.f ? w_mm : 0.f));
            const float cp = 2.f * (w_diff + (mp > 0.f ? w_mm : 0.f));
#pragma unroll
            for (int c = 0; c < 3; ++c)
                if (c < npd) L.sGp[kk[c] * 64 + lane] = traj_path_grad(cp, dp[c], cn, dn[c]);
        };
        if (pd == 3 && !b.coord_major) {
            for (int p = 0; p < n_points; ++p) one(3 * p, 3 * p + 1, 3 * p + 2, 3);
        } else {
            for (int p = 0; p < n_points; ++p) {
                const int k0 = b.coord_major ? p : p * pd, st = b.coord_major ? n_points : 1;
                one(k0, k0 + st, k0 + 2 * st, pd);
            }
        }
        const float so = traj_wave_sum(obj), sm = traj_wave_sum(mmv);
        if (lane == 0) { L.sR[0] = so; L.sR[16] = sm; }
}

template <int D, int KF, int MAXT, bool XF = false, bool CL = false, int CC = 1>
__global__ __launch_bounds__(MAXT, (MAXT / 256 > 0 ? MAXT / 256 : 1)) void traj_fused_kernel(const TrajFusedArgs a) {
    extern __shared__ __attribute__((aligned(16))) float smem[];
    constexpr int ACC = D + CC;
    constexpr int XS = CC > 1 ? CC + 2 * D : ACC;
    const int r = (CL && a.cl_across) ? blockIdx.y : blockIdx.x;
    const int ycl = CL ? (a.cl_across ? (int)blockIdx.x : (int)blockIdx.y) : 0;
    if (a.st.done[r]) return;
    const int tid = threadIdx.x, lane = tid & 63;
    const int wave = __builtin_amdgcn_readfirstlane(tid >> 6);
    const int nw = blockDim.x >> 6;
    {
        const int W = a.st.n_waypoints, dof = a.sc.dof;
        const TrajLds L = traj_lds<D, CC>(smem, a, nw);
        (void)fk_stage_sel(a.sc.fkk, a.sc.fk, a.sc.fk_dwords, a.sc.dh, L.sFk, tid, blockDim.x);
        const size_t base = (size_t)r * W * dof;
        const int n = W * dof;
        for (int i = tid; i < 64 * dof; i += blockDim.x) {
            const int ii = i < n ? i : (i % dof) + (W - 1) * dof;
            L.sQ[i] = a.st.path[base + ii];
            L.sM[i] = i < n ? a.st.adam_m[base + i] : 0.f;
            L.sV[i] = i < n ? a.st.adam_v[base + i] : 0.f;
        }
        if (tid < 2 * dof) L.sR[kTrajLim + tid] = a.st.limits[tid];
        if (tid == 0) {
            L.sR[kTrajLowest] = a.st.lowest_loss[r];
            L.sR[kTrajBestValid] = a.st.best_valid_obj[r];
            L.sR[kTrajLowestObj] = a.st.lowest_obj[r];
            L.sR[kTrajSteps] = __int_as_float(a.st.steps[r]);
            L.sR[kTrajAbort] = 0.0f;
        }
        if (tid < 8) L.sR[kTrajStats + tid] = a.st.stats[(size_t)r * 8 + tid];
    }
    __syncthreads();

    const int w = lane;
    float up_prev[CC];
    bool spec = false;
#pragma unroll
    for (int c = 0; c < CC; ++c) up_prev[c] = 0.0f;
    int it = 0, n_iters;
    {
        const auto& b = reload_kernargs<TrajFusedArgs>();
        n_iters = b.n_iters;
    }
    for (; it < n_iters; ++it) {
        float x[D];
        int j0, j1;
        ScoreArgs sa;
        {
            const auto& b = reload_kernargs<TrajFusedArgs>();
            const TrajLds L = traj_lds<D, CC>(smem, b, nw);
            const int dof = b.sc.dof, d_fk = b.sc.d_fk;
            DhArgs dh;
            DCX_COPY_DH(dh, b.sc.dh);
            FkWalk fw;
            fw.fkk = b.sc.fkk;
            fw.g = b.sc.fk;
            fw.fk = (fk_cptr)(uintptr_t)(uint32_t)(uintptr_t)L.sFk;
            fw.dh = (dh_cptr)(uintptr_t)(uint32_t)(uintptr_t)L.sFk;
            DCX_TTS(0);
            fk_trig_sel(fw, dh, L.sQ + lane * dof, L.sF + lane, wave, nw);
            __syncthreads();
            DCX_TTS(1);
            if (b.sc.jt_waves) dh2_chain_rows_sel(fw.dh, dh, L.sX + lane, L.sF + lane, wave);
            else if (wave == 0) fk_chain_sel(fw, dh, L.sQ + lane * dof, L.sX + lane, L.sF + lane);
            __syncthreads();
            DCX_TTS(2);
            if (b.sc.jt_waves && nw > 1) {
                if (wave == 1) traj_path_terms(b, L, lane);
                else if (wave >= 2) dh2_vjp_r1_sel(fw.dh, dh, L.sF + lane, L.sJ + lane, wave - 2, 15);
            }
            if (d_fk == D) {
#pragma unroll
                for (int k = 0; k < D; ++k) x[k] = L.sX[k * 64 + lane];
            } else {
#pragma unroll
                for (int k = 0; k < D; ++k) x[k] = (k < d_fk) ? L.sX[k * 64 + lane] : 0.0f;
            }
            if constexpr (CL) {
                const int ybase = ycl * b.s_super;
                const int yend = (ybase + b.s_super < b.sc.S) ? ybase + b.s_super : b.sc.S;
                wave_slice(wave, nw, b.sc.s_chunk, b.sc.s_skew, ybase, yend, j0, j1);
            } else {
                wave_slice(wave, nw, b.sc.s_chunk, b.sc.s_skew, 0, b.sc.S, j0, j1);
            }
            if constexpr (XF) {
                cfloat_ptr cen = (cfloat_ptr)(uintptr_t)b.sc.centre;
#pragma unroll
                for (int k = 0; k < D; ++k) x[k] -= cen[k];
            }
            sa.rows = b.sc.rows;
            sa.kind = b.sc.kind;
            sa.kp0 = b.sc.kp0;
            sa.kp1 = b.sc.kp1;
        }
        float sc[CC];
        float gx[D];
        bool grad_folded = false, regrad = false, grad_zero = false;
#pragma unroll
        for (int k = 0; k < D; ++k) gx[k] = 0.0f;
#pragma unroll
        for (int c = 0; c < CC; ++c) sc[c] = 0.0f;
        if constexpr (CC == 1) {
            const float up[1] = {1.0f};
            sweep_rows<D, KF, 1, MODE_GRAD_ROW, XF, DCX_TRAJ_NACC>(sa, x, up, j0, j1, sc, gx);
        } else {
            float up[CC];
            bool resweep = true;
            bool moved = false;
            auto totals_to_upstream = [&](const auto& b, const TrajLds& L) __attribute__((always_inline)) {
#pragma unroll
                for (int c = 0; c < CC; ++c) {
                    const float t = L.sRed[c * 64 + lane];
                    up[c] = (c < b.sc.c_out && t - b.margin_c[c < 8 ? c : 7] > 0.0f) ? b.opt.w_collision : 0.0f;
                }
            };
            bool prev_nonzero = false;
#pragma unroll
            for (int c = 0; c < CC; ++c) prev_nonzero = prev_nonzero || (up_prev[c] != 0.0f);
            const bool spec_full = spec && __builtin_amdgcn_ballot_w64(prev_nonzero) != 0;
            if (spec_full) {
#pragma unroll
                for (int c = 0; c < CC; ++c) up[c] = up_prev[c];
                sweep_rows<D, KF, CC, MODE_GRAD_UP, XF, DCX_TRAJ_NACC>(sa, x, up, j0, j1, sc, gx);
                const auto& b = reload_kernargs<TrajFusedArgs>();
                const TrajLds L = traj_lds<D, CC>(smem, b, nw);
                float* mine = L.sRed + (size_t)wave * ACC * 64 + lane;
#pragma unroll
                for (int c = 0; c < CC; ++c) mine[c * 64] = sc[c];
#pragma unroll
                for (int k = 0; k < D; ++k) mine[(CC + k) * 64] = gx[k];
                __syncthreads();
                if constexpr (CL) {
                    unsigned long long* slot = b.exch + ((size_t)(r * 2 + (it & 1)) * b.ys) * XS * 64 + lane;
                    const uint32_t tag = b.tag_base + (uint32_t)it + 1u;
                    traj_exchange_publish<ACC, 0, ACC, XS, 0>(L.sRed, slot, tag, ycl, wave, lane, nw);
                    if (!traj_exchange_collect<ACC, 0, ACC, XS, 0>(L.sRed, slot, tag, b.ys, wave, lane, nw)) L.sR[kTrajAbort] = 1.0f;
                } else {
                    fold_partial_rows<ACC, 0, ACC>(L.sRed, wave, lane, nw);
                }
                __syncthreads();
                totals_to_upstream(b, L);
                bool differs = false;
#pragma unroll
                for (int c = 0; c < CC; ++c) differs = differs || (up[c] != up_prev[c]);
                resweep = __builtin_amdgcn_ballot_w64(differs) != 0;
                moved = resweep;
            } else {
#pragma unroll
                for (int c = 0; c < CC; ++c) up[c] = 0.0f;
                sweep_rows<D, KF, CC, MODE_SCORE, XF, DCX_TRAJ_NACC>(sa, x, up, j0, j1, sc, gx);
                const auto& b = reload_kernargs<TrajFusedArgs>();
                const TrajLds L = traj_lds<D, CC>(smem, b, nw);
                float* mine = L.sRed + (size_t)wave * ACC * 64 + lane;
#pragma unroll
                for (int c = 0; c < CC; ++c) mine[c * 64] = sc[c];
                __syncthreads();
                if constexpr (CL) {
                    unsigned long long* slot = b.exch + ((size_t)(r * 2 + (it & 1)) * b.ys) * XS * 64 + lane;
                    const uint32_t tag = b.tag_base + (uint32_t)it + 1u;
                    traj_exchange_publish<ACC, 0, CC, XS, 0>(L.sRed, slot, tag, ycl, wave, lane, nw);
                    if (!traj_exchange_collect<ACC, 0, CC, XS, 0>(L.sRed, slot, tag, b.ys, wave, lane, nw)) L.sR[kTrajAbort] = 1.0f;
                } else {
                    fold_partial_rows<ACC, 0, CC>(L.sRed, wave, lane, nw);
                }
                __syncthreads();
                totals_to_upstream(b, L);
                bool differs = false;
#pragma unroll
                for (int c = 0; c < CC; ++c) differs = differs || (up[c] != up_prev[c]);
                moved = __builtin_amdgcn_ballot_w64(differs) != 0;
                bool nonzero = false;
#pragma unroll
                for (int c = 0; c < CC; ++c) nonzero = nonzero || (up[c] != 0.0f);
                resweep = __builtin_amdgcn_ballot_w64(nonzero) != 0;
                grad_zero = !resweep;
            }
            if (resweep) {
#pragma unroll
                for (int c = 0; c < CC; ++c) sc[c] = 0.0f;
#pragma unroll
                for (int k = 0; k < D; ++k) gx[k] = 0.0f;
                sweep_rows<D, KF, CC, MODE_GRAD_UP, XF, DCX_TRAJ_NACC, true>(sa, x, up, j0, j1, sc, gx);
            }
            grad_folded = !resweep;
            regrad = spec_full && resweep;
#pragma unroll
            for (int c = 0; c < CC; ++c) up_prev[c] = up[c];
            spec = !moved;
        }
        DCX_TTS(3);
        {
            const auto& b = reload_kernargs<TrajFusedArgs>();
            const TrajLds L = traj_lds<D, CC>(smem, b, nw);
            const int W = b.st.n_waypoints, dof = b.sc.dof, d_fk = b.sc.d_fk;
            const bool live = w < W;
            const bool jt = b.sc.jt_waves != 0;
            DhArgs dh;
            DCX_COPY_DH(dh, b.sc.dh);
            FkWalk fw;
            fw.fkk = b.sc.fkk;
            fw.g = b.sc.fk;
            fw.fk = (fk_cptr)(uintptr_t)(uint32_t)(uintptr_t)L.sFk;
            fw.dh = (dh_cptr)(uintptr_t)(uint32_t)(uintptr_t)L.sFk;
            const bool tree = fk_is_tree(fw);
            float col = 0.f;
            const int pwave = (nw > 1 && !tree) ? 1 : 0;
            auto path_terms = [&]() __attribute__((always_inline)) { traj_path_terms(b, L, lane); };
            constexpr int E0 = CC > 1 ? CC : 0;
            if (CC > 1 && grad_zero) {
                for (int e = wave; e < D; e += nw) L.sRed[(CC + e) * 64 + lane] = 0.0f;
                __syncthreads();
            }
            if ((CL || nw > 1 || CC > 1) && !grad_folded) {
                float* mine = L.sRed + (size_t)wave * ACC * 64 + lane;
                if constexpr (CC == 1) mine[0] = sc[0];
#pragma unroll
                for (int k = 0; k < D; ++k) mine[(CC + k) * 64] = gx[k];
                __syncthreads();
                DCX_TTS(4);
                if constexpr (CL) {
                    unsigned long long* slot = b.exch + ((size_t)(r * 2 + (it & 1)) * b.ys) * XS * 64 + lane;
                    const uint32_t tag = b.tag_base + (uint32_t)it + 1u;
                    if (CC > 1 && regrad) {
                        traj_exchange_publish<ACC, E0, ACC, XS, D>(L.sRed, slot, tag, ycl, wave, lane, nw);
                        if (!traj_exchange_collect<ACC, E0, ACC, XS, D>(L.sRed, slot, tag, b.ys, wave, lane, nw)) L.sR[kTrajAbort] = 1.0f;
                    } else {
                        traj_exchange_publish<ACC, E0, ACC, XS, 0>(L.sRed, slot, tag, ycl, wave, lane, nw);
                        if (!traj_exchange_collect<ACC, E0, ACC, XS, 0>(L.sRed, slot, tag, b.ys, wave, lane, nw)) L.sR[kTrajAbort] = 1.0f;
                    }
                } else {
                fold_partial_rows<ACC, E0, ACC>(L.sRed, wave, lane, nw);
                }
                DCX_TTS(5);
                DCX_TTS(6);
                __syncthreads();
// ... 193 lines not shown
```

Baseline: 783.1.

## Reuse a constant input column as spare slot for squared-norm term in sweep

Detects at pack time a configuration column whose value is the same across all support rows (or an FK-output column) and builds an alternate row buffer that moves the last coordinate into that column and puts the row's squared-norm offset in the freed slot. Sweep kernels gain an SP template path that folds the norm into the vector FMA instead of a separate add, and drops the scalar coefficient accumulation in the gradient, with a fix-up at flush time. The aim is fewer per-row scalar ops and loads in the hot distance/gradient loop, at the cost of an extra device row buffer, more kernel instantiations, and more complex gradient bookkeeping.

```diff
diff --git a/diffco_amd/csrc/dcx_api.hip b/diffco_amd/csrc/dcx_api.hip
--- a/diffco_amd/csrc/dcx_api.hip
+++ b/diffco_amd/csrc/dcx_api.hip
@@ -29,6 +29,8 @@
     float* rows_dev = nullptr;
     float* rows_p2_dev = nullptr;
     float* rows_xf_dev = nullptr;
+    float* rows_sp_dev = nullptr;
+    int32_t spare_col = -1;
     float* centre_dev = nullptr;
     int64_t S_in = 0;
     int32_t S_active = 0;
@@ -260,7 +262,7 @@
     std::atomic<int64_t> ys{-1}, nw{-1}, min_rows{-1}, split_finish_kernel{-1}, inlaunch_tiles{-1}, jac_per_class{-1},
         traj_fused{-1}, xf{-1}, jac_one_sweep{-1}, train_grid{-1}, fkk{-1}, jt_waves{-1}, hess_ys{-1}, hess_form{-1},
         traj_ys{-1}, traj_across{-1}, owner_poll{-1}, solve_threads{-1}, qt{-1}, giveup_inject{-1}, skew{-1}, skew8{-1},
-        motion_early_exit{-1};
+        motion_early_exit{-1}, spare{-1};
     Knobs() {
         auto rd = [](const char* name, std::atomic<int64_t>& dst, bool flag) {
             if (const char* e = std::getenv(name)) dst = flag ? 1 : std::atoll(e);
@@ -273,6 +275,7 @@
         rd("DCX_JAC_PER_CLASS", jac_per_class, true);
         rd("DCX_TRAJ_FUSED", traj_fused, false);
         rd("DCX_XF", xf, false);
+        rd("DCX_SPARE", spare, false);
         rd("DCX_JAC_ONE_SWEEP", jac_one_sweep, false);
         rd("DCX_TRAIN_GRID", train_grid, false);
         rd("DCX_FKK", fkk, false);
@@ -291,6 +294,16 @@
 Knobs& knobs() {
     static Knobs k;
     return k;
+}
+
+bool spare_on(const dcx_model* m) {
+    return knobs().spare != 0 && m->spare_col >= 0 && m->rows_sp_dev != nullptr && spare_applies(m->Dt, m->Cc, m->kf);
+}
+void xf_rows(const dcx_model* m, ScoreArgs& a) {
+    const bool sp = spare_on(m);
+    a.rows = sp ? m->rows_sp_dev : m->rows_xf_dev;
+    a.centre = m->centre_dev;
+    a.spare = sp ? m->spare_col + 1 : 0;
 }
 
 struct Geometry {
@@ -592,10 +605,7 @@
         a.qt_front = (int32_t)((int64_t)QT_SLICES * g.nw * qt_per * (kq >= 100 ? std::min<int64_t>(kq - 100, 100) : 45) / 100);
         nblk = (B + 15) / 16;
     }
-    if (a.xf) {
-        a.rows = m->rows_xf_dev;
-        a.centre = m->centre_dev;
-    }
+    if (a.xf) xf_rows(m, a);
     a.jt_rows = (a.fkk == 2 && g.nw >= 2 * m->dh.n_chains && m->dh.n_chains <= 2 && m->dh.end0 <= kDhUnroll &&
                  m->dh.n_steps - m->dh.end0 <= kDhUnroll && knobs().jt_waves != 0) ? 1 : 0;
     a.jt_waves = (a.jt_rows && mode != MODE_SCORE && g.red_slots == g.nw && (g.nw - 1) * acc >= 12 * m->dh.n_pt + 1 &&
@@ -676,7 +686,7 @@
                          : DCX_OK;
     std::atomic<int64_t>* dst = n == "ys" ? &k.ys : n == "nw" ? &k.nw : n == "min_rows" ? &k.min_rows
         : n == "split_finish_kernel" ? &k.split_finish_kernel : n == "inlaunch_tiles" ? &k.inlaunch_tiles
-        : n == "jac_per_class" ? &k.jac_per_class : n == "traj_fused" ? &k.traj_fused : n == "xf" ? &k.xf : n == "jac_one_sweep" ? &k.jac_one_sweep : n == "train_grid" ? &k.train_grid : n == "fkk" ? &k.fkk : n == "jt_waves" ? &k.jt_waves : n == "hess_ys" ? &k.hess_ys : n == "hess_form" ? &k.hess_form : n == "traj_ys" ? &k.traj_ys : n == "traj_across" ? &k.traj_across : n == "owner_poll" ? &k.owner_poll : n == "solve_threads" ? &k.solve_threads : n == "qt" ? &k.qt : n == "giveup_inject" ? &k.giveup_inject : n == "skew" ? &k.skew : n == "skew8" ? &k.skew8 : n == "motion_early_exit" ? &k.motion_early_exit : nullptr;
+        : n == "jac_per_class" ? &k.jac_per_class : n == "traj_fused" ? &k.traj_fused : n == "xf" ? &k.xf : n == "spare" ? &k.spare : n == "jac_one_sweep" ? &k.jac_one_sweep : n == "train_grid" ? &k.train_grid : n == "fkk" ? &k.fkk : n == "jt_waves" ? &k.jt_waves : n == "hess_ys" ? &k.hess_ys : n == "hess_form" ? &k.hess_form : n == "traj_ys" ? &k.traj_ys : n == "traj_across" ? &k.traj_across : n == "owner_poll" ? &k.owner_poll : n == "solve_threads" ? &k.solve_threads : n == "qt" ? &k.qt : n == "giveup_inject" ? &k.giveup_inject : n == "skew" ? &k.skew : n == "skew8" ? &k.skew8 : n == "motion_early_exit" ? &k.motion_early_exit : nullptr;
     if (!dst) return fail(DCX_ERR_INVALID, "unknown knob: " + n);
     *dst = value;
     return DCX_OK;
@@ -697,7 +707,9 @@
     if (m->rows_dev) (void)hipFree(m->rows_dev);
     if (m->rows_xf_dev) (void)hipFree(m->rows_xf_dev);
     if (m->rows_p2_dev) (void)hipFree(m->rows_p2_dev);
-    m->rows_dev = m->rows_xf_dev = m->rows_p2_dev = nullptr;
+    if (m->rows_sp_dev) (void)hipFree(m->rows_sp_dev);
+    m->rows_dev = m->rows_xf_dev = m->rows_p2_dev = m->rows_sp_dev = nullptr;
+    m->spare_col = -1;
     m->cap = 0;
 }
 
@@ -705,9 +717,10 @@
     if (cap < 1) cap = 1;
     if (cap <= m->cap && m->rows_dev) return DCX_OK;
     const size_t floats = (size_t)cap * m->RS + rows_tail_floats(m);
-    float *rows = nullptr, *rows_xf = nullptr, *rows_p2 = nullptr;
+    float *rows = nullptr, *rows_xf = nullptr, *rows_p2 = nullptr, *rows_sp = nullptr;
     hipError_t e = hipMalloc((void**)&rows, floats * sizeof(float));
     if (e == hipSuccess) e = hipMalloc((void**)&rows_xf, floats * sizeof(float));
+    if (e == hipSuccess && spare_applies(m->Dt, m->Cc, m->kf)) e = hipMalloc((void**)&rows_sp, floats * sizeof(float));
     if (e == hipSuccess && p2_applies(m->Dt, m->Cc, m->kf)) e = hipMalloc((void**)&rows_p2, (floats + m->RS) * sizeof(float));
     if (e == hipSuccess && !m->centre_dev) e = hipMalloc((void**)&m->centre_dev, (size_t)m->Dt * sizeof(float));
     if (e == hipSuccess && !m->info_dev) e = hipMalloc((void**)&m->info_dev, 16);
@@ -723,12 +736,14 @@
         if (rows) (void)hipFree(rows);
         if (rows_xf) (void)hipFree(rows_xf);
         if (rows_p2) (void)hipFree(rows_p2);
+        if (rows_sp) (void)hipFree(rows_sp);
         return fail_hip(e, "device allocation of the model");
     }
     model_free_rows(m);
     m->rows_dev = rows;
     m->rows_xf_dev = rows_xf;
     m->rows_p2_dev = rows_p2;
+    m->rows_sp_dev = rows_sp;
     m->cap = cap;
     return DCX_OK;
 }
@@ -739,6 +754,7 @@
     a.w = w_dev;
     a.rows = m->rows_dev;
     a.rows_xf = m->rows_xf_dev;
+    a.rows_sp = m->rows_sp_dev;
     a.centre = m->centre_dev;
     a.info = m->info_dev;
     a.S = S;
@@ -760,6 +776,7 @@
     std::memcpy(&ss_max, reinterpret_cast<const char*>(m->info_host) + 8, sizeof(double));
     m->S_in = S;
     m->S_active = m->info_host[0];
+    m->spare_col = m->info_host[1] - 1;
     m->xf_rq_ok = (m->kf == KF_RQ2 && m->fk.kind != DCX_FK_NONE && (double)m->kp0 * ss_max <= kXfRqRule) ? 1 : 0;
     return DCX_OK;
 }
@@ -808,6 +825,23 @@
             centre[k] = (float)(acc / (double)kept);
         }
     }
+    int sp = -1;
+    if (m->rows_sp_dev && kept > 0) {
+        for (int k = m->Dt - 1; k >= 0; --k) {
+            bool same = (k >= D || m->fk.kind != DCX_FK_NONE);
+            if (same && k < D) {
+                uint32_t first, v;
+                std::memcpy(&first, &rows[k], 4);
+                for (int32_t j = 0; j < kept && same; ++j) {
+                    std::memcpy(&v, &rows[(size_t)j * m->RS + k], 4);
+                    same = (v == first);
+                }
+                if (same) centre[k] = rows[k];
+            }
+            if (same && sp < 0) sp = k;
+        }
+    }
+    m->spare_col = sp;
     double ss_max = 0.0;
     for (int32_t j = 0; j < kept; ++j) {
         float* cen = &rows_xf[(size_t)j * m->RS];
@@ -824,6 +858,18 @@
     rows_xf.resize(rows.size(), 0.0f);
     hipError_t e = hipMemcpy(m->rows_dev, rows.data(), rows.size() * sizeof(float), hipMemcpyHostToDevice);
     if (e == hipSuccess) e = hipMemcpy(m->rows_xf_dev, rows_xf.data(), rows_xf.size() * sizeof(float), hipMemcpyHostToDevice);
+    if (e == hipSuccess && sp >= 0) {
+        std::vector<float> rows_sp(rows_xf);
+        for (int32_t j = 0; j < kept; ++j) {
+            const float* x = &rows_xf[(size_t)j * m->RS];
+            float* y = &rows_sp[(size_t)j * m->RS];
+            y[sp] = x[m->Dt - 1];
+            y[m->Dt - 1] = x[ss_off];
+            y[m->Dt + 2] = y[m->Dt - 2];
+            y[m->Dt + 3] = 1.0f;
+        }
+        e = hipMemcpy(m->rows_sp_dev, rows_sp.data(), rows_sp.size() * sizeof(float), hipMemcpyHostToDevice);
+    }
     if (e == hipSuccess) e = hipMemcpy(m->centre_dev, centre.data(), centre.size() * sizeof(float), hipMemcpyHostToDevice);
     if (e != hipSuccess) return fail_hip(e, "upload of the model's rows");
     return DCX_OK;
@@ -971,6 +1017,7 @@
     if (m->rows_dev) (void)hipFree(m->rows_dev);
     if (m->rows_xf_dev) (void)hipFree(m->rows_xf_dev);
     if (m->rows_p2_dev) (void)hipFree(m->rows_p2_dev);
+    if (m->rows_sp_dev) (void)hipFree(m->rows_sp_dev);
     if (m->centre_dev) (void)hipFree(m->centre_dev);
     if (m->info_dev) (void)hipFree(m->info_dev);
     if (m->info_host) (void)hipHostFree(m->info_host);
@@ -1284,8 +1331,7 @@
             a.sc.kp1 = m->kp1;
             a.sc.xf = (knobs().xf != 0 && m->kf == KF_POLY1 && xf_applies(m->Dt, m->Cc, KF_POLY1) && m->rows_xf_dev) ? 1 : 0;
             if (a.sc.xf) {
-                a.sc.rows = m->rows_xf_dev;
-                a.sc.centre = m->centre_dev;
+                xf_rows(m, a.sc);
             } else if (m->rows_p2_dev && p2_applies(m->Dt, m->Cc, m->kf)) {
                 a.sc.rows = m->rows_p2_dev;
                 traj_p2 = true;
@@ -1505,10 +1551,7 @@
     sa.kp0 = m->kp0_sweep;
     sa.kp1 = m->kp1;
     sa.xf = xf_able ? 1 : 0;
-    if (sa.xf) {
-        sa.rows = m->rows_xf_dev;
-        sa.centre = m->centre_dev;
-    }
+    if (sa.xf) xf_rows(m, sa);
     sa.jt_rows = (sa.fkk == 2 && g.nw >= 2 * m->dh.n_chains && m->dh.n_chains <= 2 && m->dh.end0 <= kDhUnroll &&
                   m->dh.n_steps - m->dh.end0 <= kDhUnroll && knobs().jt_waves != 0) ? 1 : 0;
     if (g.ys > 1) {
@@ -1845,10 +1888,7 @@
     sa.kp0 = m->kp0_sweep;
     sa.kp1 = m->kp1;
     sa.xf = xf_able ? 1 : 0;
-    if (sa.xf) {
-        sa.rows = m->rows_xf_dev;
-        sa.centre = m->centre_dev;
-    }
+    if (sa.xf) xf_rows(m, sa);
     sa.jt_rows = (sa.fkk == 2 && g.nw >= 2 * m->dh.n_chains && m->dh.n_chains <= 2 && m->dh.end0 <= kDhUnroll &&
                   m->dh.n_steps - m->dh.end0 <= kDhUnroll && knobs().jt_waves != 0) ? 1 : 0;
     sa.jt_waves = 0;
diff --git a/diffco_amd/csrc/motion_cost_inst.hip b/diffco_amd/csrc/motion_cost_inst.hip
--- a/diffco_amd/csrc/motion_cost_inst.hip
+++ b/diffco_amd/csrc/motion_cost_inst.hip
@@ -29,8 +29,11 @@
         kern<<<grid, dim3(64 * nw), lds, st>>>(a, mc_off);
         return hipGetLastError();
     };
+    if constexpr (spare_applies(kD, CC, KF)) {
+        if (a.sc.xf && a.sc.spare > 0) return launch(motion_cost_kernel<kD, KF, CC, MODE, kMaxT, 2>);
+    }
     if constexpr (xf_applies(kD, CC, KF)) {
-        if (a.sc.xf) return launch(motion_cost_kernel<kD, KF, CC, MODE, kMaxT, true>);
+        if (a.sc.xf) return launch(motion_cost_kernel<kD, KF, CC, MODE, kMaxT, 1>);
     }
     return launch(motion_cost_kernel<kD, KF, CC, MODE, kMaxT>);
 }
diff --git a/diffco_amd/csrc/motion_cost_kernel.h b/diffco_amd/csrc/motion_cost_kernel.h
--- a/diffco_amd/csrc/motion_cost_kernel.h
+++ b/diffco_amd/csrc/motion_cost_kernel.h
@@ -96,7 +96,7 @@
     sN[lane] = (int32_t)(offs[e + 1] - start);
 }
 
-template <int D, int KF, int CC, int MODE, int MAXT, bool XF = false>
+template <int D, int KF, int CC, int MODE, int MAXT, int XF = 0 >
 __global__ __launch_bounds__(MAXT, sweep_min_waves(D, CC, KF)) void motion_cost_kernel(const MotionCostArgs m, int32_t mc_off) {
     static_assert((CC == 1) == (MODE == MODE_GRAD_ROW), "one class: the hinge sweep; several: the score and gradient passes");
     extern __shared__ __attribute__((aligned(16))) float smem[];
@@ -152,7 +152,7 @@
 #pragma unroll
         for (int k = 0; k < D; ++k) x[k] = (k < a.d_fk) ? sX[k * 64 + lane0] : 0.0f;
     }
-    if constexpr (XF) {
+    if constexpr (XF != 0) {
         cfloat_ptr cen = (cfloat_ptr)(uintptr_t)a.centre;
 #pragma unroll
         for (int k = 0; k < D; ++k) x[k] -= cen[k];
@@ -177,7 +177,7 @@
     const int yend = (ybase + a.s_super < a.S) ? (ybase + a.s_super) : a.S;
     int j0, j1;
     wave_slice(wave, nw, a.s_chunk, a.s_skew, ybase, yend, j0, j1);
-    sweep_rows<D, KF, CC, MODE, XF>(a, x, up, j0, j1, sc, gx);
+    sweep_rows<D, KF, CC, MODE, XF != 0, 0, false, XF == 2>(a, x, up, j0, j1, sc, gx);
 
     const auto& b = reload_kernargs<MotionCostArgs>();
     const int lane = fresh_lane();
diff --git a/diffco_amd/csrc/motion_inst.hip b/diffco_amd/csrc/motion_inst.hip
--- a/diffco_amd/csrc/motion_inst.hip
+++ b/diffco_amd/csrc/motion_inst.hip
@@ -27,8 +27,11 @@
         kern<<<grid, dim3(64 * nw), lds, st>>>(a, mo_off);
         return hipGetLastError();
     };
+    if constexpr (spare_applies(kD, CC, KF)) {
+        if (a.sc.xf && a.sc.spare > 0) return launch(motion_kernel<kD, KF, CC, kMaxT, 2>);
+    }
     if constexpr (xf_applies(kD, CC, KF)) {
-        if (a.sc.xf) return launch(motion_kernel<kD, KF, CC, kMaxT, true>);
+        if (a.sc.xf) return launch(motion_kernel<kD, KF, CC, kMaxT, 1>);
     }
     return launch(motion_kernel<kD, KF, CC, kMaxT>);
 }
diff --git a/diffco_amd/csrc/motion_kernel.h b/diffco_amd/csrc/motion_kernel.h
--- a/diffco_amd/csrc/motion_kernel.h
+++ b/diffco_amd/csrc/motion_kernel.h
@@ -71,7 +71,7 @@
     return __fadd_rn(qa, __fmul_rn((float)k, __fmul_rn(d, *frac_e)));
 }
 
-template <int D, int KF, int CC, int MAXT, bool XF = false>
+template <int D, int KF, int CC, int MAXT, int XF = 0 >
 __global__ __launch_bounds__(MAXT, sweep_min_waves(D, CC, KF)) void motion_kernel(const MotionArgs m, int32_t mo_off) {
     extern __shared__ __attribute__((aligned(16))) float smem[];
     const ScoreArgs& a = m.sc;
@@ -170,7 +170,7 @@
 #pragma unroll
                 for (int k = 0; k < D; ++k) x[k] = (k < a.d_fk) ? sX[k * 64 + lane] : 0.0f;
             }
-            if constexpr (XF) {
+            if constexpr (XF != 0) {
                 cfloat_ptr cen = (cfloat_ptr)(uintptr_t)a.centre;
 #pragma unroll
                 for (int k = 0; k < D; ++k) x[k] -= cen[k];
@@ -184,7 +184,7 @@
             float gx[D];
 #pragma unroll
             for (int c = 0; c < CC; ++c) up[c] = 0.0f;
-            sweep_rows<D, KF, CC, MODE_SCORE, XF>(a, x, up, j0, j1, sc, gx);
+            sweep_rows<D, KF, CC, MODE_SCORE, XF != 0, 0, false, XF == 2>(a, x, up, j0, j1, sc, gx);
         }
         const auto& b = reload_kernargs<MotionArgs>();
         const int lane = fresh_lane();
diff --git a/diffco_amd/csrc/motion_worst_inst.hip b/diffco_amd/csrc/motion_worst_inst.hip
--- a/diffco_amd/csrc/motion_worst_inst.hip
+++ b/diffco_amd/csrc/motion_worst_inst.hip
@@ -27,8 +27,11 @@
         kern<<<grid, dim3(64 * nw), lds, st>>>(a, mo_off);
         return hipGetLastError();
     };
+    if constexpr (spare_applies(kD, CC, KF)) {
+        if (a.sc.xf && a.sc.spare > 0) return launch(motion_worst_kernel<kD, KF, CC, kMaxT, 2>);
+    }
     if constexpr (xf_applies(kD, CC, KF)) {
-        if (a.sc.xf) return launch(motion_worst_kernel<kD, KF, CC, kMaxT, true>);
+        if (a.sc.xf) return launch(motion_worst_kernel<kD, KF, CC, kMaxT, 1>);
     }
     return launch(motion_worst_kernel<kD, KF, CC, kMaxT>);
 }
diff --git a/diffco_amd/csrc/motion_worst_kernel.h b/diffco_amd/csrc/motion_worst_kernel.h
--- a/diffco_amd/csrc/motion_worst_kernel.h
+++ b/diffco_amd/csrc/motion_worst_kernel.h
@@ -59,7 +59,7 @@
 __host__ __device__ inline uint32_t motion_worst_unorder(uint32_t o) { return (o & 0x80000000u) ? (o & 0x7fffffffu) : ~o; }
 
 #ifdef __HIPCC__
-template <int D, int KF, int CC, int MAXT, bool XF = false>
+template <int D, int KF, int CC, int MAXT, int XF = 0 >
 __global__ __launch_bounds__(MAXT, sweep_min_waves(D, CC, KF)) void motion_worst_kernel(const MotionWorstArgs m, int32_t mo_off) {
     extern __shared__ __attribute__((aligned(16))) float smem[];
     const ScoreArgs& a = m.sc;
@@ -113,7 +113,7 @@
 #pragma unroll
             for (int k = 0; k < D; ++k) x[k] = (k < a.d_fk) ? sX[k * 64 + lane] : 0.0f;
         }
-        if constexpr (XF) {
+        if constexpr (XF != 0) {
             cfloat_ptr cen = (cfloat_ptr)(uintptr_t)a.centre;
 #pragma unroll
             for (int k = 0; k < D; ++k) x[k] -= cen[k];
@@ -127,7 +127,7 @@
         float gx[D];
 #pragma unroll
         for (int c = 0; c < CC; ++c) up[c] = 0.0f;
-        sweep_rows<D, KF, CC, MODE_SCORE, XF>(a, x, up, j0, j1, sc, gx);
+        sweep_rows<D, KF, CC, MODE_SCORE, XF != 0, 0, false, XF == 2>(a, x, up, j0, j1, sc, gx);
     }
     const auto& b = reload_kernargs<MotionWorstArgs>();
     const int lane = fresh_lane();
diff --git a/diffco_amd/csrc/pack_kernels.h b/diffco_amd/csrc/pack_kernels.h
--- a/diffco_amd/csrc/pack_kernels.h
+++ b/diffco_amd/csrc/pack_kernels.h
@@ -9,6 +9,7 @@
     const float* w;
     float* rows;
     float* rows_xf;
+    float* rows_sp;
     float* centre;
     int32_t* info;
     int64_t S;
diff --git a/diffco_amd/csrc/pack_kernels.hip b/diffco_amd/csrc/pack_kernels.hip
--- a/diffco_amd/csrc/pack_kernels.hip
+++ b/diffco_amd/csrc/pack_kernels.hip
@@ -11,6 +11,7 @@
     __shared__ int s_wave_cnt[kPackThreads / 64];
     __shared__ int s_base;
     __shared__ double s_max[kPackThreads / 64];
+    __shared__ int s_same[128];
     const int tid = threadIdx.x, lane = tid & 63, wave = tid >> 6;
     const int ss_off = a.Dt + a.Cl + (a.Cl > 1 ? 1 : 0);
     if (tid == 0) s_base = 0;
@@ -57,40 +58,75 @@
     for (int i = tid; i < a.tail_floats; i += kPackThreads) {
         a.rows[(size_t)kept * a.RS + i] = 0.0f;
         a.rows_xf[(size_t)kept * a.RS + i] = 0.0f;
+        if (a.rows_sp) a.rows_sp[(size_t)kept * a.RS + i] = 0.0f;
     }
     __syncthreads();
     if (tid < a.Dt) {
         float c = 0.0f;
+        bool same = kept > 0 && (tid >= a.D || a.centred);
+        uint32_t differ = 0;
         if (a.centred && tid < a.D && kept > 0) {
             double acc = 0.0;
             const float* col = a.rows + tid;
+            const float first = col[0];
             int j = 0;
             for (; j + 32 <= kept; j += 32) {
                 float v[32];
 #pragma unroll
                 for (int u = 0; u < 32; ++u) v[u] = col[(size_t)(j + u) * a.RS];
 #pragma unroll
-                for (int u = 0; u < 32; ++u) acc += (double)v[u];
+                for (int u = 0; u < 32; ++u) {
+                    acc += (double)v[u];
+                    differ |= __float_as_uint(v[u]) ^ __float_as_uint(first);
+                }
             }
-            for (; j < kept; ++j) acc += (double)col[(size_t)j * a.RS];
+            for (; j < kept; ++j) {
+                const float v = col[(size_t)j * a.RS];
+                acc += (double)v;
+                differ |= __float_as_uint(v) ^ __float_as_uint(first);
+            }
+            same = same && differ == 0;
             c = (float)(acc / (double)kept);
+            if (a.rows_sp && same) c = first;
         }
         a.centre[tid] = c;
+        if (tid < 128) s_same[tid] = same ? 1 : 0;
     }
     __syncthreads();
+    int sp = -1;
+    if (a.rows_sp)
+        for (int k = (a.Dt < 128 ? a.Dt : 128) - 1; k >= 0 && sp < 0; --k)
+            if (s_same[k]) sp = k;
     double mx = 0.0;
     for (int j = tid; j < kept; j += kPackThreads) {
         const float* r = a.rows + (size_t)j * a.RS;
         float* x = a.rows_xf + (size_t)j * a.RS;
+        float* y = sp >= 0 ? a.rows_sp + (size_t)j * a.RS : nullptr;
+        float v_last = 0.0f, v_pen = 0.0f;
         double ss = 0.0;
         for (int k = 0; k < a.D; ++k) {
             const float v = r[k] - a.centre[k];
             x[k] = v;
+            if (y) y[k] = v;
+            v_last = (k == a.Dt - 1) ? v : v_last;
+            v_pen = (k == a.Dt - 2) ? v : v_pen;
             ss += (double)v * (double)v;
         }
-        for (int k = a.D; k < a.RS; ++k) x[k] = r[k];
-        x[ss_off] = a.rq2 ? (float)(ss + (double)a.seed) : (float)ss;
+        for (int k = a.D; k < a.RS; ++k) {
+            const float v = r[k];
+            x[k] = v;
+            if (y) y[k] = v;
+        }
+        const float ssf = a.rq2 ? (float)(ss + (double)a.seed) : (float)ss;
+        x[ss_off] = ssf;
         mx = ss > mx ? ss : mx;
+        if (y) {
+            y[ss_off] = ssf;
+            y[sp] = v_last;
+            y[a.Dt - 1] = ssf;
+            y[a.Dt + 2] = (sp == a.Dt - 2) ? v_last : v_pen;
+            y[a.Dt + 3] = 1.0f;
+        }
     }
 #pragma unroll
     for (int o = 32; o > 0; o >>= 1) {
@@ -103,7 +139,7 @@
         double t = 0.0;
         for (int w = 0; w < kPackThreads / 64; ++w) t = s_max[w] > t ? s_max[w] : t;
         a.info[0] = kept;
-        a.info[1] = 0;
+        a.info[1] = sp + 1;
         reinterpret_cast<double*>(a.info)[1] = t;
     }
 }
diff --git a/diffco_amd/csrc/score_inst.hip b/diffco_amd/csrc/score_inst.hip
--- a/diffco_amd/csrc/score_inst.hip
+++ b/diffco_amd/csrc/score_inst.hip
@@ -37,6 +37,9 @@
     if constexpr (qt_applies(kD, CC, KF, MODE)) {
         if (a.qt) return launch(score_kernel<kD, KF, CC, MODE, kMaxT, false, true>);
     }
+    if constexpr (spare_applies(kD, CC, KF)) {
+        if (a.xf && a.spare > 0) return launch(score_kernel_sp<kD, KF, CC, MODE, kMaxT>);
+    }
     if constexpr (xf_applies(kD, CC, KF)) {
         if (a.xf) return launch(score_kernel<kD, KF, CC, MODE, kMaxT, true>);
     }
@@ -161,18 +164,24 @@
     }
     auto go_t = [&](auto kern) { return traj_go(kern, nw, lds, n_paths, a, st); };
     if (a.ys > 1) {
+        if constexpr (spare_applies(kD, 1, KF_POLY1)) {
+            if (kf == KF_POLY1 && a.sc.xf && a.sc.spare > 0) return go_t(traj_fused_kernel<kD, KF_POLY1, kMaxT, 2, true>);
+        }
         if constexpr (xf_applies(kD, 1, KF_POLY1)) {
-            if (kf == KF_POLY1 && a.sc.xf) return go_t(traj_fused_kernel<kD, KF_POLY1, kMaxT, true, true>);
+            if (kf == KF_POLY1 && a.sc.xf) return go_t(traj_fused_kernel<kD, KF_POLY1, kMaxT, 1, true>);
         }
         switch (kf) {
-        case KF_RQ2: return go_t(traj_fused_kernel<kD, KF_RQ2, kMaxT, false, true>);
-        case KF_POLY1: return go_t(traj_fused_kernel<kD, KF_POLY1, kMaxT, false, true>);
-        case KF_GEN: return go_t(traj_fused_kernel<kD, KF_GEN, kMaxT, false, true>);
+        case KF_RQ2: return go_t(traj_fused_kernel<kD, KF_RQ2, kMaxT, 0, true>);
+        case KF_POLY1: return go_t(traj_fused_kernel<kD, KF_POLY1, kMaxT, 0, true>);
+        case KF_GEN: return go_t(traj_fused_kernel<kD, KF_GEN, kMaxT, 0, true>);
         default: return hipErrorInvalidValue;
         }
     }
+    if constexpr (spare_applies(kD, 1, KF_POLY1)) {
+        if (kf == KF_POLY1 && a.sc.xf && a.sc.spare > 0) return go_t(traj_fused_kernel<kD, KF_POLY1, kMaxT, 2>);
+    }
     if constexpr (xf_applies(kD, 1, KF_POLY1)) {
-        if (kf == KF_POLY1 && a.sc.xf) return go_t(traj_fused_kernel<kD, KF_POLY1, kMaxT, true>);
+        if (kf == KF_POLY1 && a.sc.xf) return go_t(traj_fused_kernel<kD, KF_POLY1, kMaxT, 1>);
     }
     switch (kf) {
     case KF_RQ2: return go_t(traj_fused_kernel<kD, KF_RQ2, kMaxT>);
@@ -190,20 +199,20 @@
     auto go_t = [&](auto kern) { return traj_go(kern, nw, lds, n_paths, a, st); };
     if (a.ys > 1) {
         if constexpr (xf_applies(kD, CC, KF_POLY1)) {
-            if (kf == KF_POLY1 && a.sc.xf) return go_t(traj_fused_kernel<kD, KF_POLY1, kMaxT, true, true, CC>);
+            if (kf == KF_POLY1 && a.sc.xf) return go_t(traj_fused_kernel<kD, KF_POLY1, kMaxT, 1, true, CC>);
         }
         switch (kf) {
-        case KF_RQ2: return go_t(traj_fused_kernel<kD, KF_RQ2, kMaxT, false, true, CC>);
-        case KF_POLY1: return go_t(traj_fused_kernel<kD, KF_POLY1, kMaxT, false, true, CC>);
+        case KF_RQ2: return go_t(traj_fused_kernel<kD, KF_RQ2, kMaxT, 0, true, CC>);
+        case KF_POLY1: return go_t(traj_fused_kernel<kD, KF_POLY1, kMaxT, 0, true, CC>);
         default: return hipErrorNotSupported;
         }
     }
     if constexpr (xf_applies(kD, CC, KF_POLY1)) {
-        if (kf == KF_POLY1 && a.sc.xf) return go_t(traj_fused_kernel<kD, KF_POLY1, kMaxT, true, false, CC>);
-    }
-    switch (kf) {
-    case KF_RQ2: return go_t(traj_fused_kernel<kD, KF_RQ2, kMaxT, false, false, CC>);
-    case KF_POLY1: return go_t(traj_fused_kernel<kD, KF_POLY1, kMaxT, false, false, CC>);
+        if (kf == KF_POLY1 && a.sc.xf) return go_t(traj_fused_kernel<kD, KF_POLY1, kMaxT, 1, false, CC>);
+    }
+    switch (kf) {
+    case KF_RQ2: return go_t(traj_fused_kernel<kD, KF_RQ2, kMaxT, 0, false, CC>);
+    case KF_POLY1: return go_t(traj_fused_kernel<kD, KF_POLY1, kMaxT, 0, false, CC>);
     default: return hipErrorNotSupported;
     }
 }
diff --git a/diffco_amd/csrc/score_kernel.h b/diffco_amd/csrc/score_kernel.h
--- a/diffco_amd/csrc/score_kernel.h
+++ b/diffco_amd/csrc/score_kernel.h
@@ -47,6 +47,7 @@
 #endif
     float kp0, kp1;
     int32_t xf;
+    int32_t spare;
     int32_t fkk;
     int32_t fk_dwords;
     DhArgs dh;
@@ -284,26 +285,53 @@
     const int parts = (4 * used <= (CC > 1 ? DCX_P0_MAX_MULTI : DCX_P0_MAX_SINGLE)) ? 0 : (used + 37) / 38;
     return (KF == KF_POLY1 || KF == KF_RQ2) && used + 1 <= 38 && parts <= 1;
 }
+constexpr bool spare_applies(int D, int CC, int KF) {
+    return CC == 1 && (D % 4) == 0 && D >= 4 && D <= 12 && (KF == KF_POLY1 || KF == KF_RQ2) && D + 4 <= (D + 2 + 3) / 4 * 4;
+}
 constexpr bool p2_applies(int D, int CC, int KF) {
     return DCX_PAIR2 && DCX_PAIR2_LOADS && CC == 1 && (D % 2) == 0 && D <= DCX_PAIR2_MAX_D && 4 * (D + 1) <= DCX_P0_MAX_SINGLE &&
            (KF == KF_RQ2 || KF == KF_POLY1);
 }
 
-template <int D, int KF, int CC, int MODE, bool XF = false, int NACC = 0, bool NS = false>
-__device__ __forceinline__ void sweep_rows(const ScoreArgs& a, const float (&x)[D], const float (&up)[CC], int j0, int j1,
+template <int D, int KF, int CC, int MODE, bool XF = false, int NACC = 0, bool NS = false, bool SP = false>
+__device__ __forceinline__ void sweep_rows(const ScoreArgs& a, const float (&x_in)[D], const float (&up)[CC], int j0, int j1,
                                            float (&sc)[CC], float (&gx)[D]) {
     static_assert(!NS || (CC > 1 && MODE == MODE_GRAD_UP), "NS: the gradient sweep of a multi-class model");
+    static_assert(!SP || (XF && spare_applies(D, CC, KF) && xf_applies(D, CC, KF)), "the spare form: expanded, one class, D = 4, 8, 12");
+    float x[D];
+    float e_sp = 0.0f, tot_sp = 0.0f;
+    int col_sp = 0;
+    if constexpr (SP) {
+        const int c = a.spare - 1;
+        e_sp = x_in[D - 1];
+#pragma unroll
+        for (int k = 0; k + 1 < D; ++k) {
+            e_sp = (k == c) ? x_in[k] : e_sp;
+            x[k] = (k == c) ? x_in[D - 1] : x_in[k];
+        }
+        x[D - 1] = 0.0f;
+        col_sp = c;
+        asm volatile("" : "+v"(col_sp));
+    } else {
+#pragma unroll
+        for (int k = 0; k < D; ++k) x[k] = x_in[k];
+    }
     using L = RowLayout<D, CC>;
     constexpr bool GRAD = (MODE != MODE_SCORE);
     v2f gx2[D / 2 + 1];
 #pragma unroll
     for (int k = 0; k < D / 2 + 1; ++k) gx2[k] = v2f{0.0f, 0.0f};
     cfloat_ptr rows = (cfloat_ptr)(uintptr_t)a.rows;
+    if constexpr (SP) {
+        uint64_t rp = (uint64_t)(uintptr_t)a.rows;
+        asm volatile("" : "+s"(rp));
+        rows = (cfloat_ptr)(uintptr_t)rp;
+    }
     constexpr int USED_DIRECT = D + CC + (CC > 1 ? 1 : 0);
     constexpr bool XFA = XF && xf_applies(D, CC, KF);
-    constexpr int USED = USED_DIRECT + (XFA ? 1 : 0);
+    constexpr int USED = SP ? D + 4 : USED_DIRECT + (XFA ? 1 : 0);
     constexpr int RSTRIDE = L::RS;
-    constexpr int PARTS = (4 * USED <= (CC > 1 ? DCX_P0_MAX_MULTI : DCX_P0_MAX_SINGLE)) ? 0 : (USED + 37) / 38;
+    constexpr int PARTS = SP ? 0 : (4 * USED <= (CC > 1 ? DCX_P0_MAX_MULTI : DCX_P0_MAX_SINGLE)) ? 0 : (USED + 37) / 38;
     constexpr bool SC2 = (CC > 1 && PARTS == 1);
     v2f sc2[CC / 2 + 1];
 #pragma unroll
@@ -330,6 +358,7 @@
     if constexpr (XFA) {
 #pragma unroll
         for (int k = 0; k < D; ++k) xx = fmaf(x[k], x[k], xx);
+        if constexpr (SP) xx = fmaf(e_sp, e_sp, xx);
         thr = fmaxf(DCX_XF_TAU * xx, 1e-30f);
 #pragma unroll
         for (int k = 0; k + 1 < D; k += 2) {
@@ -337,11 +366,13 @@
             ga[k / 2] = v2f{0.0f, 0.0f};
         }
         if constexpr (D & 1) xm_tail = -2.0f * x[D - 1];
+        if constexpr (SP) xm[D / 2 - 1].y = 1.0f;
     }
     auto d2_x = [&](const auto& r) __attribute__((always_inline)) -> float {
         constexpr int NA = NACC > 0 ? NACC : DCX_D2_ACCS(D);
         v2f acc[NA];
-        acc[0] = v2f{xx + r[L::SS_OFF], 0.0f};
+        if constexpr (SP) acc[0] = v2f{xx, 0.0f};
+        else acc[0] = v2f{xx + r[L::SS_OFF], 0.0f};
 #pragma unroll
         for (int i = 1; i < NA; ++i) acc[i] = v2f{0.0f, 0.0f};
 #pragma unroll
@@ -384,11 +415,14 @@
             const v2f c2 = {coef, coef};
 #pragma unroll
             for (int k = 0; k + 1 < D; k += 2) {
-                const v2f rv = {r[k], r[k + 1]};
+                v2f rv = {r[k], r[k + 1]};
+                if constexpr (SP) {
+                    if (k == D - 2) rv = v2f{r[D + 2], r[D + 3]};
+                }
                 ga[k / 2] = __builtin_elementwise_fma(c2, rv, ga[k / 2]);
             }
             if constexpr (D & 1) ga_tail = fmaf(coef, r[D - 1], ga_tail);
-            asum += coef;
+            if constexpr (!SP) asum += coef;
         }
     };
     auto pair_x = [&](const auto& r) __attribute__((always_inline)) -> float {
@@ -404,7 +438,10 @@
 #pragma unroll
         for (int k = 0; k + 1 < D; k += 2) {
             const v2f rv = {r[k], r[k + 1]};
-            const v2f dk = xm[k / 2] * mh - rv;
+            v2f dk = xm[k / 2] * mh - rv;
+            if constexpr (SP) {
+                if (k == D - 2) dk.y = e_sp;
+            }
             dacc = __builtin_elementwise_fma(dk, dk, dacc);
         }
         float d2d = dacc.x + dacc.y;
@@ -425,7 +462,12 @@
 #pragma unroll
             for (int k = 0; k + 1 < D; k += 2) {
                 const v2f rv = {r[k], r[k + 1]};
-                ga[k / 2] = __builtin_elementwise_fma(cd2, xm[k / 2] * mh - rv, ga[k / 2]);
+                if (SP && k == D - 2) {
+                    ga[k / 2].x = fmaf(cd, fmaf(xm[k / 2].x, -0.5f, -rv.x), ga[k / 2].x);
+                    tot_sp -= cd;
+                } else {
+                    ga[k / 2] = __builtin_elementwise_fma(cd2, xm[k / 2] * mh - rv, ga[k / 2]);
+                }
             }
             if constexpr (D & 1) ga_tail = fmaf(cd, -0.5f * xm_tail - r[D - 1], ga_tail);
         }
@@ -452,10 +494,15 @@
     };
     auto flush_x = [&]() __attribute__((always_inline)) {
         if constexpr (XFA && GRAD) {
+            if constexpr (SP) asum = ga[D / 2 - 1].y;
             const v2f ah = {0.5f * asum, 0.5f * asum};
 #pragma unroll
             for (int k = 0; k + 1 < D; k += 2) ga[k / 2] = __builtin_elementwise_fma(xm[k / 2], ah, ga[k / 2]);
             if constexpr (D & 1) ga_tail = fmaf(xm_tail, 0.5f * asum, ga_tail);
+            if constexpr (SP) {
+                tot_sp += asum;
+                ga[D / 2 - 1].y = 0.0f;
+            }
             asum = 0.0f;
         }
     };
@@ -560,7 +607,10 @@
         --exp_real_loads;
 #endif
 #pragma unroll
-        for (int e = 0; e < NLOAD; ++e) dst[e] = r[e];
+        for (int e = 0; e < NLOAD; ++e) {
+            if (SP && e == D + 1) continue;
+            dst[e] = r[e];
+        }
     };
 
     static_assert(!XFA || PARTS <= 1, "expanded form: whole rows only");
@@ -810,12 +860,25 @@
 
     if constexpr (XFA && GRAD) {
         flush_x();
+        if constexpr (SP) {
+            const int c = __builtin_amdgcn_readfirstlane(col_sp);
+            const float gl = e_sp * tot_sp;
+            float gsw = gl;
+#pragma unroll
+            for (int k = 0; k + 1 < D; ++k) {
+                const float h = (k & 1) ? ga[k / 2].y : ga[k / 2].x;
+                gsw = (k == c) ? -h : gsw;
+                gx[k] += (k == c) ? gl : -h;
+            }
+            gx[D - 1] += gsw;
+        } else {
 #pragma unroll
         for (int k = 0; k + 1 < D; k += 2) {
             gx[k] -= ga[k / 2].x;
             gx[k + 1] -= ga[k / 2].y;
         }
         if constexpr (D & 1) gx[D - 1] -= ga_tail;
+        }
     } else {
 #pragma unroll
         for (int k = 0; k + 1 < D; k += 2) {
@@ -939,8 +1002,8 @@
 }
 
 
-template <int D, int KF, int CC, int MODE, int MAXT, bool XF = false, bool QT = false>
-__global__ __launch_bounds__(MAXT, sweep_min_waves(D, CC, KF, QT)) void score_kernel(const ScoreArgs a) {
+template <int D, int KF, int CC, int MODE, int MAXT, bool XF, bool QT, bool SP>
+__device__ __forceinline__ void score_body(const ScoreArgs& a) {
     extern __shared__ __attribute__((aligned(16))) float smem[];
     constexpr bool GRAD = (MODE != MODE_SCORE);
     constexpr int ACC = (GRAD ? D : 0) + CC;
@@ -1064,7 +1127,7 @@
         const float* slice = smem + a.qt_off + base + ((wave & 3) * kQtSlices + (lane >> 4)) * (per * RSQ + 4);
         sweep_rows_lds<D, KF, GRAD>(a, x, slice, per, sc[0], gx);
     } else {
-        sweep_rows<D, KF, CC, MODE, XF>(a, x, up, j0, j1, sc, gx);
+        sweep_rows<D, KF, CC, MODE, XF, 0, false, SP>(a, x, up, j0, j1, sc, gx);
     }
     DCX_TS(3);
     {
@@ -1417,6 +1480,16 @@
     }
 }
 
+template <int D, int KF, int CC, int MODE, int MAXT, bool XF = false, bool QT = false>
+__global__ __launch_bounds__(MAXT, sweep_min_waves(D, CC, KF, QT)) void score_kernel(const ScoreArgs a) {
+    score_body<D, KF, CC, MODE, MAXT, XF, QT, false>(a);
+}
+template <int D, int KF, int CC, int MODE, int MAXT>
+__global__ __launch_bounds__(MAXT, sweep_min_waves(D, CC, KF, false)) void score_kernel_sp(const ScoreArgs a) {
+    static_assert(spare_applies(D, CC, KF), "no spare form for this shape");
+    score_body<D, KF, CC, MODE, MAXT, true, false, true>(a);
+}
+
 struct FinishArgs {
     const float* partial;
     const FkProg* fk;
diff --git a/diffco_amd/csrc/traj_fused.h b/diffco_amd/csrc/traj_fused.h
--- a/diffco_amd/csrc/traj_fused.h
+++ b/diffco_amd/csrc/traj_fused.h
@@ -207,7 +207,7 @@
         if (lane == 0) { L.sR[0] = so; L.sR[16] = sm; }
 }
 
-template <int D, int KF, int MAXT, bool XF = false, bool CL = false, int CC = 1>
+template <int D, int KF, int MAXT, int XF = 0 , bool CL = false, int CC = 1>
 __global__ __launch_bounds__(MAXT, (MAXT / 256 > 0 ? MAXT / 256 : 1)) void traj_fused_kernel(const TrajFusedArgs a) {
     extern __shared__ __attribute__((aligned(16))) float smem[];
     constexpr int ACC = D + CC;
@@ -293,12 +293,13 @@
             } else {
                 wave_slice(wave, nw, b.sc.s_chunk, b.sc.s_skew, 0, b.sc.S, j0, j1);
             }
-            if constexpr (XF) {
+            if constexpr (XF != 0) {
                 cfloat_ptr cen = (cfloat_ptr)(uintptr_t)b.sc.centre;
 #pragma unroll
                 for (int k = 0; k < D; ++k) x[k] -= cen[k];
             }
             sa.rows = b.sc.rows;
+            sa.spare = b.sc.spare;
             sa.kind = b.sc.kind;
             sa.kp0 = b.sc.kp0;
             sa.kp1 = b.sc.kp1;
@@ -312,7 +313,7 @@
         for (int c = 0; c < CC; ++c) sc[c] = 0.0f;
         if constexpr (CC == 1) {
             const float up[1] = {1.0f};
-            sweep_rows<D, KF, 1, MODE_GRAD_ROW, XF, DCX_TRAJ_NACC>(sa, x, up, j0, j1, sc, gx);
+            sweep_rows<D, KF, 1, MODE_GRAD_ROW, XF != 0, DCX_TRAJ_NACC, false, XF == 2>(sa, x, up, j0, j1, sc, gx);
         } else {
             float up[CC];
             bool resweep = true;
@@ -331,7 +332,7 @@
             if (spec_full) {
 #pragma unroll
                 for (int c = 0; c < CC; ++c) up[c] = up_prev[c];
-                sweep_rows<D, KF, CC, MODE_GRAD_UP, XF, DCX_TRAJ_NACC>(sa, x, up, j0, j1, sc, gx);
+                sweep_rows<D, KF, CC, MODE_GRAD_UP, XF != 0, DCX_TRAJ_NACC>(sa, x, up, j0, j1, sc, gx);
                 const auto& b = reload_kernargs<TrajFusedArgs>();
                 const TrajLds L = traj_lds<D, CC>(smem, b, nw);
                 float* mine = L.sRed + (size_t)wave * ACC * 64 + lane;
@@ -358,7 +359,7 @@
             } else {
 #pragma unroll
                 for (int c = 0; c < CC; ++c) up[c] = 0.0f;
-                sweep_rows<D, KF, CC, MODE_SCORE, XF, DCX_TRAJ_NACC>(sa, x, up, j0, j1, sc, gx);
+                sweep_rows<D, KF, CC, MODE_SCORE, XF != 0, DCX_TRAJ_NACC>(sa, x, up, j0, j1, sc, gx);
                 const auto& b = reload_kernargs<TrajFusedArgs>();
                 const TrajLds L = traj_lds<D, CC>(smem, b, nw);
                 float* mine = L.sRed + (size_t)wave * ACC * 64 + lane;
@@ -390,7 +391,7 @@
                 for (int c = 0; c < CC; ++c) sc[c] = 0.0f;
 #pragma unroll
                 for (int k = 0; k < D; ++k) gx[k] = 0.0f;
-                sweep_rows<D, KF, CC, MODE_GRAD_UP, XF, DCX_TRAJ_NACC, true>(sa, x, up, j0, j1, sc, gx);
+                sweep_rows<D, KF, CC, MODE_GRAD_UP, XF != 0, DCX_TRAJ_NACC, true>(sa, x, up, j0, j1, sc, gx);
             }
             grad_folded = !resweep;
             regrad = spec_full && resweep;
```

Measured after the change: 797.6, median of 6. 1.02x the previous value.
